# zhm1205/Multimodal_TTA

Hardware: AMD Instinct MI355X
Metric: adapted volumes/sec (higher is better)
Workload: dtype bf16

## Files before the change

include/mmtta.h:

```cpp
#ifndef MMTTA_H
#define MMTTA_H

#include <stdint.h>

#ifdef __cplusplus
extern "C" {
#endif

#define MMTTA_ABI_VERSION 2

typedef enum {
  MMTTA_OK = 0,
  MMTTA_ERR_INVALID = -1,
  MMTTA_ERR_UNSUPPORTED = -2,
  MMTTA_ERR_LAUNCH = -3,
  MMTTA_ERR_WORKSPACE = -4
} mmtta_status;

typedef enum { MMTTA_F32 = 0, MMTTA_BF16 = 1 } mmtta_dtype;

typedef struct {
  void* ptr;
  int32_t n, c, d, h, w;
  int64_t sn, sc, sd, sh, sw;
  int32_t dtype;
  int32_t flags;
} mmtta_tensor;

#define MMTTA_TENSOR_OWNS_PAD 1

#define MMTTA_ACT_NONE 0
#define MMTTA_ACT_RELU 1
#define MMTTA_ACT_LEAKY_RELU 2
typedef struct {
  const float* mean;
  const float* rstd;
  const float* gamma;
  const float* beta;
  int32_t relu;
  int32_t per_item;
  const float* scale;
  const float* shift;
  float negative_slope;
  int32_t _pad2;
} mmtta_norm_on_load;

const char* mmtta_last_error(void);
int mmtta_abi_version(void);

#define MMTTA_OPT_PROFILE_MAIN_KERNEL_ONLY 1
#define MMTTA_OPT_SPLITK_BELOW 2
#define MMTTA_OPT_SPLITK_TARGET 3
#define MMTTA_OPT_WGRAD_WORKGROUPS 4
#define MMTTA_OPT_WGRAD_THIN_SLABS 5
#define MMTTA_OPT_IGEMM_PIPELINE 6
#define MMTTA_OPT_EPILOGUE_VEC16 9
#define MMTTA_OPT_IGEMM_LEAN 10
#define MMTTA_OPT_WGRAD_VECTOR_STAGING 11
#define MMTTA_OPT_CLASS_FUSED_MIN_WORKGROUPS 12
#define MMTTA_OPT_THIN_MFMA 13
#define MMTTA_OPT_IGEMM_FRAGMENT_REUSE 14
#define MMTTA_OPT_LAME_TILED 15
#define MMTTA_OPT_RAW_STAGING 16
#define MMTTA_OPT_HEAD_LOSS_PAIR 17
#define MMTTA_OPT_THIN_LEAN 18
#define MMTTA_OPT_WGRAD_EPILOGUE_UPDATE 19
#define MMTTA_OPT_CLS8_PIPELINE 20
#define MMTTA_OPT_CLS8_LEAN_EPILOGUE 21
int mmtta_set_option(int key, int value);

int mmtta_copy_strided(const mmtta_tensor* src, const mmtta_tensor* dst, void* stream);

typedef enum {
  MMTTA_CONV_FWD = 0,
  MMTTA_CONV_DGRAD = 1,
  MMTTA_CONVT_FWD = 2,
  MMTTA_CONVT_DGRAD = 3
} mmtta_conv_op;

typedef struct {
  int32_t op;
  int32_t ksize;
  int32_t stride;
  int32_t cin;
  int32_t cout;
  int32_t dtype;
} mmtta_conv_desc;

int64_t mmtta_conv_packed_bytes(const mmtta_conv_desc* desc);

int mmtta_conv_pack_weights(const mmtta_conv_desc* desc, const float* w_master, void* packed, void* stream);

typedef struct {
  mmtta_conv_desc desc;
  const float* w_master;
  void* packed;
} mmtta_pack_item;
int64_t mmtta_conv_pack_table_bytes(int count);
int mmtta_conv_pack_table_build(const mmtta_pack_item* items, int count, void* table_host, int64_t* total);
int mmtta_conv_pack_batched(const void* table_dev, int count, int64_t total, void* stream);

typedef struct {
  int32_t tiles;
  int32_t launches;
  int32_t ksplit;
  int32_t stats_rows;
  int32_t config;
  int32_t _pad;
  int64_t workspace_bytes;
} mmtta_conv_plan_t;

int mmtta_conv_plan(const mmtta_conv_desc* desc, const mmtta_tensor* x, const mmtta_tensor* y,
                    mmtta_conv_plan_t* plan);

typedef struct {
  const mmtta_tensor* add;
  mmtta_norm_on_load add_norm;
} mmtta_conv_epilogue;

int mmtta_conv_run(const mmtta_conv_desc* desc, const mmtta_tensor* x, const mmtta_norm_on_load* x_norm,
                   const void* packed, const float* bias, const mmtta_conv_epilogue* epi,
                   const mmtta_tensor* y, int accumulate, float* stats, void* workspace,
                   int64_t workspace_bytes, void* stream);

int mmtta_conv_route(const mmtta_conv_desc* desc, const mmtta_tensor* x, const mmtta_norm_on_load* x_norm,
                     const mmtta_conv_epilogue* epi, const mmtta_tensor* y, int accumulate, const float* stats);

int mmtta_conv_stages_raw(const mmtta_conv_desc* desc, const mmtta_tensor* x, const mmtta_norm_on_load* x_norm,
                          const mmtta_conv_epilogue* epi, const mmtta_tensor* y, int accumulate, const float* stats);

int mmtta_conv_cls8_pipelined(const mmtta_conv_desc* desc, const mmtta_tensor* x, const mmtta_norm_on_load* x_norm,
                              const mmtta_conv_epilogue* epi, const mmtta_tensor* y, int accumulate, const float* stats);

int mmtta_conv_cls8_lean_epilogue(const mmtta_conv_desc* desc, const mmtta_tensor* x, const mmtta_norm_on_load* x_norm,
                                  const mmtta_conv_epilogue* epi, const mmtta_tensor* y, int accumulate, const float* stats);

int mmtta_conv_thin_lean(const mmtta_conv_desc* desc, const mmtta_tensor* x, const mmtta_norm_on_load* x_norm,
                         const mmtta_conv_epilogue* epi, const mmtta_tensor* y, int accumulate, const float* stats);

int mmtta_conv_thin_kernel(const mmtta_conv_desc* desc, const mmtta_tensor* x, const mmtta_norm_on_load* x_norm,
                           const mmtta_conv_epilogue* epi, const mmtta_tensor* y, int accumulate, const float* stats);

typedef struct {
  int32_t items_per_set;
  int32_t inner;
  int64_t packed_outer, packed_inner;
  int64_t weight_outer, weight_inner;
  int64_t bias_outer, bias_inner;
} mmtta_param_sets;

int mmtta_conv_run_sets(const mmtta_conv_desc* desc, const mmtta_tensor* x, const mmtta_norm_on_load* x_norm,
                        const void* packed, const float* bias, const mmtta_conv_epilogue* epi,
                        const mmtta_tensor* y, int accumulate, float* stats, void* workspace,
                        int64_t workspace_bytes, const mmtta_param_sets* sets, void* stream);

int mmtta_conv_head_loss_eligible(const mmtta_conv_desc* desc, const mmtta_tensor* x, const mmtta_norm_on_load* x_norm,
                                  const mmtta_conv_epilogue* epi, const mmtta_tensor* y, const mmtta_tensor* dlogits,
                                  int softmax, int per_item);
int64_t mmtta_conv_head_loss_partials(const mmtta_conv_desc* desc, const mmtta_tensor* x, const mmtta_tensor* y);
int mmtta_conv_head_loss_run_sets(const mmtta_conv_desc* desc, const mmtta_tensor* x, const mmtta_norm_on_load* x_norm,
                                  const void* packed, const float* bias, const mmtta_conv_epilogue* epi,
                                  const mmtta_tensor* y, const mmtta_tensor* dlogits, int softmax, int per_item,
                                  double* partial, float* loss, const mmtta_param_sets* sets, void* stream);

int64_t mmtta_conv_wgrad_workspace_bytes(const mmtta_conv_desc* desc, const mmtta_tensor* x,
                                         const mmtta_tensor* dy);
int mmtta_conv_wgrad_kernel(const mmtta_conv_desc* desc, const mmtta_tensor* x, const mmtta_tensor* dy);
int mmtta_conv_wgrad_stages_raw(const mmtta_conv_desc* desc, const mmtta_tensor* x, const mmtta_norm_on_load* x_norm,
                                const mmtta_tensor* dy);
int mmtta_conv_wgrad(const mmtta_conv_desc* desc, const mmtta_tensor* x, const mmtta_norm_on_load* x_norm,
                     const mmtta_tensor* dy, float* dw, float* db, int accumulate, void* workspace,
                     int64_t workspace_bytes, void* stream);

int64_t mmtta_conv_wgrad_workspace_bytes_sets(const mmtta_conv_desc* desc, const mmtta_tensor* x, const mmtta_tensor* dy,
                                              const mmtta_param_sets* sets);
int mmtta_conv_wgrad_sets(const mmtta_conv_desc* desc, const mmtta_tensor* x, const mmtta_norm_on_load* x_norm,
                          const mmtta_tensor* dy, float* dw, float* db, int accumulate, void* workspace,
                          int64_t workspace_bytes, const mmtta_param_sets* sets, void* stream);
int mmtta_conv_wgrad_plan_sets(const mmtta_conv_desc* desc, const mmtta_tensor* x, const mmtta_tensor* dy,
                               const mmtta_param_sets* sets, int32_t plan[4]);

typedef struct {
  int32_t clip, zscore, masked, min_count;
  float lo, hi, mask_gt, eps;
  float mean, std;
  int32_t legacy, _pad;
} mmtta_intensity_rule;
int64_t mmtta_intensity_scratch_bytes(int channels);
int mmtta_intensity_normalize(const mmtta_tensor* x, const mmtta_intensity_rule* rules, const mmtta_tensor* y,
                              void* scratch, void* stream);

typedef enum {
  MMTTA_NORM_INSTANCE = 0,
  MMTTA_NORM_BATCH = 1,
  MMTTA_NORM_GROUP = 2
} mmtta_norm_kind;

int mmtta_norm_stats_finalize(int kind, int groups, const float* part, int rows_per_n, int n, int c,
                              int64_t count, float eps, int training, float* running_mean,
                              float* running_var, float momentum, float* mean, float* rstd,
                              const float* gamma, const float* beta, float* scale, float* shift,
                              double* scratch, void* stream);

typedef struct {
  int32_t items_per_set;
  int32_t _pad;
  int64_t affine_stride;
  int64_t stats_stride;
} mmtta_norm_sets;

int mmtta_norm_stats_finalize_sets(int kind, int groups, const float* part, int rows_per_n, int n, int c,
                                   int64_t count, float eps, int training, float* running_mean,
                                   float* running_var, float momentum, float* mean, float* rstd,
                                   const float* gamma, const float* beta, float* scale, float* shift,
                                   float* gamma_items, float* beta_items, double* scratch,
                                   const mmtta_norm_sets* sets, void* stream);

int mmtta_reduce_rows_per_n(const mmtta_tensor* t);

int mmtta_channel_stats(const mmtta_tensor* x, float* part, void* stream);

int mmtta_combine(const mmtta_tensor* a, const mmtta_norm_on_load* ta, const mmtta_tensor* b,
                  const mmtta_norm_on_load* tb, const mmtta_tensor* out, void* stream);

int mmtta_norm_bwd_reduce(const mmtta_tensor* dout, const mmtta_tensor* y, const mmtta_norm_on_load* t,
                          float* part, void* stream);

int mmtta_norm_bwd_finalize(int kind, int groups, const float* part, int rows_per_n, int n, int c, int64_t count,
                            const float* gamma, int training, float* m1, float* m2, float* dgamma,
                            float* dbeta, int accumulate, double* scratch , void* stream);

int mmtta_norm_bwd_finalize_sets(int kind, int groups, const float* part, int rows_per_n, int n, int c, int64_t count,
                                 const float* gamma, int training, float* m1, float* m2, float* dgamma,
                                 float* dbeta, int accumulate, double* scratch ,
                                 const mmtta_norm_sets* sets, void* stream);

int mmtta_norm_bwd_apply(const mmtta_tensor* dout, const mmtta_tensor* y, const mmtta_norm_on_load* t,
                         const float* m1, const float* m2, const mmtta_tensor* dy, void* stream);

int mmtta_norm_bwd_small_ok(const mmtta_tensor* dout, const mmtta_tensor* y, const mmtta_norm_on_load* t,
                            const mmtta_tensor* dy);
int mmtta_norm_bwd_small(const mmtta_tensor* dout, const mmtta_tensor* y, const mmtta_norm_on_load* t, int64_t count,
                         const mmtta_tensor* dy, void* stream);

int mmtta_upsample2x_fwd(const mmtta_tensor* x, const mmtta_tensor* y, void* stream);
int mmtta_upsample2x_bwd(const mmtta_tensor* dy, const mmtta_tensor* dx, int accumulate, void* stream);

int mmtta_lincomb(int count, const mmtta_tensor* const* in, const float* w, const mmtta_tensor* out,
                  int accumulate, void* stream);

#define MMTTA_PW_OP_CHANNEL_STATS 0
#define MMTTA_PW_OP_NORM_BWD_REDUCE 1
#define MMTTA_PW_OP_NORM_BWD_APPLY 2
#define MMTTA_PW_OP_NORM_BWD_SMALL 3
#define MMTTA_PW_OP_COMBINE 4
#define MMTTA_PW_OP_LINCOMB 5
#define MMTTA_PW_OP_UPSAMPLE_FWD 6
#define MMTTA_PW_OP_UPSAMPLE_BWD 7
#define MMTTA_PW_REDUCE 0
#define MMTTA_PW_REDUCE_STREAM 1
#define MMTTA_PW_ELEMENTWISE 2
#define MMTTA_PW_COMBINE8 3
#define MMTTA_PW_NORM_BWD_APPLY8 4
#define MMTTA_PW_NORM_BWD_SMALL 5
#define MMTTA_PW_LINCOMB 6
#define MMTTA_PW_UPSAMPLE_FWD 7
#define MMTTA_PW_UPSAMPLE_BWD 8
typedef struct {
  int64_t vox_per_row;
  int64_t work_items;
  int64_t grid_x;
  int32_t grid_y;
  int32_t family;
  int32_t mode;
  int32_t vec;
  int32_t it;
  int32_t count;
  int32_t bf16_a;
  int32_t bf16_b;
  int32_t bf16_o;
  int32_t has_b;
  int32_t rows_per_n;
  int32_t rows_per_block;
  int32_t cpl, nvl;
  int32_t trips;
  int32_t cb_passes;
  int32_t second_trip;
  int32_t leaky;
// ... 225 lines not shown
```

multimodal_tta_amd/_lib.py:

```python
from __future__ import annotations

import ctypes as C
import os
from typing import Optional, Sequence

import torch

_HERE = os.path.dirname(os.path.abspath(__file__))
LIB_PATH = os.path.join(_HERE, "csrc", "libmmtta.so")

F32, BF16 = 0, 1
CONV_FWD, CONV_DGRAD, CONVT_FWD, CONVT_DGRAD = 0, 1, 2, 3
NORM_INSTANCE, NORM_BATCH, NORM_GROUP = 0, 1, 2


class MmttaError(RuntimeError):
    pass


class Tensor(C.Structure):
    _fields_ = [
        ("ptr", C.c_void_p),
        ("n", C.c_int32), ("c", C.c_int32), ("d", C.c_int32), ("h", C.c_int32), ("w", C.c_int32),
        ("sn", C.c_int64), ("sc", C.c_int64), ("sd", C.c_int64), ("sh", C.c_int64), ("sw", C.c_int64),
        ("dtype", C.c_int32), ("flags", C.c_int32),
    ]


class NormOnLoad(C.Structure):
    _fields_ = [
        ("mean", C.c_void_p), ("rstd", C.c_void_p), ("gamma", C.c_void_p), ("beta", C.c_void_p),
        ("relu", C.c_int32), ("per_item", C.c_int32), ("scale", C.c_void_p), ("shift", C.c_void_p),
    ]


class NormOnLoadAct(NormOnLoad):
    _fields_ = [("negative_slope", C.c_float), ("_pad2", C.c_int32)]


class NormSets(C.Structure):
    _fields_ = [("items_per_set", C.c_int32), ("_pad", C.c_int32), ("affine_stride", C.c_int64), ("stats_stride", C.c_int64)]


class ConvDesc(C.Structure):
    _fields_ = [
        ("op", C.c_int32), ("ksize", C.c_int32), ("stride", C.c_int32), ("cin", C.c_int32), ("cout", C.c_int32),
        ("dtype", C.c_int32),
    ]


class PackItem(C.Structure):
    _fields_ = [("desc", ConvDesc), ("w_master", C.c_void_p), ("packed", C.c_void_p)]


class ParamSets(C.Structure):
    _fields_ = [("items_per_set", C.c_int32), ("inner", C.c_int32), ("packed_outer", C.c_int64), ("packed_inner", C.c_int64),
                ("weight_outer", C.c_int64), ("weight_inner", C.c_int64), ("bias_outer", C.c_int64), ("bias_inner", C.c_int64)]


class ConvPlan(C.Structure):
    _fields_ = [
        ("tiles", C.c_int32), ("launches", C.c_int32), ("ksplit", C.c_int32), ("stats_rows", C.c_int32),
        ("config", C.c_int32), ("_pad", C.c_int32), ("workspace_bytes", C.c_int64),
    ]


class PointwiseRoute(C.Structure):
    _fields_ = [("vox_per_row", C.c_int64), ("work_items", C.c_int64), ("grid_x", C.c_int64), ("grid_y", C.c_int32),
                ("family", C.c_int32), ("mode", C.c_int32), ("vec", C.c_int32), ("it", C.c_int32), ("count", C.c_int32),
                ("bf16_a", C.c_int32), ("bf16_b", C.c_int32), ("bf16_o", C.c_int32), ("has_b", C.c_int32),
                ("rows_per_n", C.c_int32), ("rows_per_block", C.c_int32), ("cpl", C.c_int32), ("nvl", C.c_int32),
                ("trips", C.c_int32), ("cb_passes", C.c_int32), ("second_trip", C.c_int32), ("leaky", C.c_int32)]


PW_OPS = ("channel_stats", "norm_bwd_reduce", "norm_bwd_apply", "norm_bwd_small", "combine", "lincomb", "upsample_fwd",
          "upsample_bwd")
PW_FAMILIES = ("reduce", "reduce_stream", "elementwise", "combine8", "norm_bwd_apply8", "norm_bwd_small", "lincomb",
               "upsample_fwd", "upsample_bwd")


class OptimDesc(C.Structure):
    _fields_ = [("kind", C.c_int32), ("lr", C.c_float), ("beta1", C.c_float), ("beta2", C.c_float), ("eps", C.c_float),
                ("weight_decay", C.c_float), ("momentum", C.c_float), ("dampening", C.c_float), ("nesterov", C.c_int32)]


class UpdateTarget(C.Structure):
    _fields_ = [("optim", OptimDesc), ("w_p", C.c_void_p), ("w_m", C.c_void_p), ("w_v", C.c_void_p), ("b_p", C.c_void_p),
                ("b_m", C.c_void_p), ("b_v", C.c_void_p), ("b_grad", C.c_void_p), ("image", C.c_void_p * 2),
                ("image_outer", C.c_int64 * 2), ("image_inner", C.c_int64 * 2), ("step", C.c_void_p),
                ("w_decay", C.c_int32), ("b_decay", C.c_int32)]


OPTIM_ADAM, OPTIM_ADAMW, OPTIM_SGD = 0, 1, 2


class ConvEpilogue(C.Structure):
    _fields_ = [("add", C.POINTER(Tensor)), ("add_norm", NormOnLoadAct)]


class IntensityRule(C.Structure):
    _fields_ = [("clip", C.c_int32), ("zscore", C.c_int32), ("masked", C.c_int32), ("min_count", C.c_int32),
                ("lo", C.c_float), ("hi", C.c_float), ("mask_gt", C.c_float), ("eps", C.c_float),
                ("mean", C.c_float), ("std", C.c_float), ("legacy", C.c_int32), ("_pad", C.c_int32)]


class InputNormBranch(C.Structure):
    _fields_ = [("dy", C.POINTER(Tensor)), ("weight", C.c_void_p), ("set_stride", C.c_int64), ("ksize", C.c_int32),
                ("stride", C.c_int32)]


class WindowGrid(C.Structure):
    _fields_ = [("extent", C.c_int32 * 3), ("count", C.c_int32 * 3)]


_P = C.POINTER
_SIGNATURES = {
    "mmtta_last_error": (C.c_char_p, []),
    "mmtta_abi_version": (C.c_int, []),
    "mmtta_set_option": (C.c_int, [C.c_int, C.c_int]),
    "mmtta_intensity_scratch_bytes": (C.c_int64, [C.c_int]),
    "mmtta_intensity_normalize": (C.c_int, [_P(Tensor), _P(IntensityRule), _P(Tensor), C.c_void_p, C.c_void_p]),
    "mmtta_copy_strided": (C.c_int, [_P(Tensor), _P(Tensor), C.c_void_p]),
    "mmtta_conv_packed_bytes": (C.c_int64, [_P(ConvDesc)]),
    "mmtta_conv_pack_weights": (C.c_int, [_P(ConvDesc), C.c_void_p, C.c_void_p, C.c_void_p]),
    "mmtta_conv_pack_table_bytes": (C.c_int64, [C.c_int]),
    "mmtta_conv_pack_table_build": (C.c_int, [_P(PackItem), C.c_int, C.c_void_p, _P(C.c_int64)]),
    "mmtta_conv_pack_batched": (C.c_int, [C.c_void_p, C.c_int, C.c_int64, C.c_void_p]),
    "mmtta_conv_plan": (C.c_int, [_P(ConvDesc), _P(Tensor), _P(Tensor), _P(ConvPlan)]),
    "mmtta_conv_run": (C.c_int, [_P(ConvDesc), _P(Tensor), _P(NormOnLoad), C.c_void_p, C.c_void_p, _P(ConvEpilogue),
                                 _P(Tensor), C.c_int, C.c_void_p, C.c_void_p, C.c_int64, C.c_void_p]),
    "mmtta_conv_run_sets": (C.c_int, [_P(ConvDesc), _P(Tensor), _P(NormOnLoad), C.c_void_p, C.c_void_p, _P(ConvEpilogue),
                                      _P(Tensor), C.c_int, C.c_void_p, C.c_void_p, C.c_int64, _P(ParamSets), C.c_void_p]),
    "mmtta_conv_route": (C.c_int, [_P(ConvDesc), _P(Tensor), _P(NormOnLoad), _P(ConvEpilogue), _P(Tensor), C.c_int, C.c_void_p]),
    "mmtta_conv_stages_raw": (C.c_int, [_P(ConvDesc), _P(Tensor), _P(NormOnLoad), _P(ConvEpilogue), _P(Tensor), C.c_int, C.c_void_p]),
    "mmtta_conv_cls8_pipelined": (C.c_int, [_P(ConvDesc), _P(Tensor), _P(NormOnLoad), _P(ConvEpilogue), _P(Tensor), C.c_int, C.c_void_p]),
    "mmtta_conv_cls8_lean_epilogue": (C.c_int, [_P(ConvDesc), _P(Tensor), _P(NormOnLoad), _P(ConvEpilogue), _P(Tensor), C.c_int, C.c_void_p]),
    "mmtta_conv_thin_lean": (C.c_int, [_P(ConvDesc), _P(Tensor), _P(NormOnLoad), _P(ConvEpilogue), _P(Tensor), C.c_int, C.c_void_p]),
    "mmtta_conv_thin_kernel": (C.c_int, [_P(ConvDesc), _P(Tensor), _P(NormOnLoad), _P(ConvEpilogue), _P(Tensor), C.c_int, C.c_void_p]),
    "mmtta_conv_head_loss_eligible": (C.c_int, [_P(ConvDesc), _P(Tensor), _P(NormOnLoad), _P(ConvEpilogue), _P(Tensor), _P(Tensor),
                                                C.c_int, C.c_int]),
    "mmtta_conv_head_loss_partials": (C.c_int64, [_P(ConvDesc), _P(Tensor), _P(Tensor)]),
    "mmtta_conv_head_loss_run_sets": (C.c_int, [_P(ConvDesc), _P(Tensor), _P(NormOnLoad), C.c_void_p, C.c_void_p, _P(ConvEpilogue),
                                                _P(Tensor), _P(Tensor), C.c_int, C.c_int, C.c_void_p, C.c_void_p, _P(ParamSets),
                                                C.c_void_p]),
    "mmtta_conv_wgrad_workspace_bytes": (C.c_int64, [_P(ConvDesc), _P(Tensor), _P(Tensor)]),
    "mmtta_conv_wgrad_workspace_bytes_sets": (C.c_int64, [_P(ConvDesc), _P(Tensor), _P(Tensor), _P(ParamSets)]),
    "mmtta_conv_wgrad_plan_sets": (C.c_int, [_P(ConvDesc), _P(Tensor), _P(Tensor), _P(ParamSets), _P(C.c_int32)]),
    "mmtta_conv_wgrad_sets": (C.c_int, [_P(ConvDesc), _P(Tensor), _P(NormOnLoad), _P(Tensor), C.c_void_p, C.c_void_p,
                                        C.c_int, C.c_void_p, C.c_int64, _P(ParamSets), C.c_void_p]),
    "mmtta_conv_wgrad_kernel": (C.c_int, [_P(ConvDesc), _P(Tensor), _P(Tensor)]),
    "mmtta_conv_wgrad_stages_raw": (C.c_int, [_P(ConvDesc), _P(Tensor), _P(NormOnLoad), _P(Tensor)]),
    "mmtta_conv_wgrad": (C.c_int, [_P(ConvDesc), _P(Tensor), _P(NormOnLoad), _P(Tensor), C.c_void_p, C.c_void_p,
                                   C.c_int, C.c_void_p, C.c_int64, C.c_void_p]),
    "mmtta_norm_stats_finalize": (C.c_int, [C.c_int, C.c_int, C.c_void_p, C.c_int, C.c_int, C.c_int, C.c_int64,
                                            C.c_float, C.c_int, C.c_void_p, C.c_void_p, C.c_float, C.c_void_p,
                                            C.c_void_p, C.c_void_p, C.c_void_p, C.c_void_p, C.c_void_p, C.c_void_p,
                                            C.c_void_p]),
    "mmtta_norm_stats_finalize_sets": (C.c_int, [C.c_int, C.c_int, C.c_void_p, C.c_int, C.c_int, C.c_int, C.c_int64,
                                                 C.c_float, C.c_int, C.c_void_p, C.c_void_p, C.c_float, C.c_void_p,
                                                 C.c_void_p, C.c_void_p, C.c_void_p, C.c_void_p, C.c_void_p, C.c_void_p,
                                                 C.c_void_p, C.c_void_p, _P(NormSets), C.c_void_p]),
    "mmtta_reduce_rows_per_n": (C.c_int, [_P(Tensor)]),
    "mmtta_channel_stats": (C.c_int, [_P(Tensor), C.c_void_p, C.c_void_p]),
    "mmtta_combine": (C.c_int, [_P(Tensor), _P(NormOnLoad), _P(Tensor), _P(NormOnLoad), _P(Tensor), C.c_void_p]),
    "mmtta_norm_bwd_reduce": (C.c_int, [_P(Tensor), _P(Tensor), _P(NormOnLoad), C.c_void_p, C.c_void_p]),
    "mmtta_norm_bwd_finalize": (C.c_int, [C.c_int, C.c_int, C.c_void_p, C.c_int, C.c_int, C.c_int, C.c_int64,
                                          C.c_void_p, C.c_int, C.c_void_p, C.c_void_p, C.c_void_p, C.c_void_p,
                                          C.c_int, C.c_void_p, C.c_void_p]),
    "mmtta_norm_bwd_finalize_sets": (C.c_int, [C.c_int, C.c_int, C.c_void_p, C.c_int, C.c_int, C.c_int, C.c_int64,
                                               C.c_void_p, C.c_int, C.c_void_p, C.c_void_p, C.c_void_p, C.c_void_p,
                                               C.c_int, C.c_void_p, _P(NormSets), C.c_void_p]),
    "mmtta_norm_bwd_apply": (C.c_int, [_P(Tensor), _P(Tensor), _P(NormOnLoad), C.c_void_p, C.c_void_p, _P(Tensor),
                                       C.c_void_p]),
    "mmtta_norm_bwd_small_ok": (C.c_int, [_P(Tensor), _P(Tensor), _P(NormOnLoad), _P(Tensor)]),
    "mmtta_norm_bwd_small": (C.c_int, [_P(Tensor), _P(Tensor), _P(NormOnLoad), C.c_int64, _P(Tensor), C.c_void_p]),
    "mmtta_upsample2x_fwd": (C.c_int, [_P(Tensor), _P(Tensor), C.c_void_p]),
    "mmtta_upsample2x_bwd": (C.c_int, [_P(Tensor), _P(Tensor), C.c_int, C.c_void_p]),
    "mmtta_lincomb": (C.c_int, [C.c_int, _P(_P(Tensor)), _P(C.c_float), _P(Tensor), C.c_int, C.c_void_p]),
    "mmtta_pointwise_route": (C.c_int, [C.c_int, _P(_P(Tensor)), C.c_int, _P(NormOnLoad), _P(NormOnLoad), C.c_void_p, C.c_void_p,
                                        _P(PointwiseRoute)]),
    "mmtta_entropy_partials": (C.c_int64, [_P(Tensor)]),
    "mmtta_entropy_loss": (C.c_int, [_P(Tensor), C.c_int, _P(Tensor), C.c_void_p, C.c_void_p, C.c_void_p]),
    "mmtta_entropy_partials_items": (C.c_int64, [_P(Tensor)]),
    "mmtta_entropy_loss_items": (C.c_int, [_P(Tensor), C.c_int, _P(Tensor), C.c_void_p, C.c_void_p, C.c_void_p]),
    "mmtta_entropy_filtered_partials": (C.c_int64, [_P(Tensor)]),
    "mmtta_entropy_filtered_items": (C.c_int, [_P(Tensor), C.c_int, C.c_float, C.c_void_p, C.c_void_p, _P(Tensor), C.c_void_p,
                                               C.c_void_p, C.c_void_p, C.c_void_p]),
    "mmtta_mirror_views": (C.c_int, [_P(Tensor), _P(Tensor), C.c_int, _P(C.c_int32), C.c_void_p]),
    "mmtta_memo_partials": (C.c_int64, [_P(Tensor), C.c_int]),
    "mmtta_memo_loss_items": (C.c_int, [_P(Tensor), C.c_int, C.c_int, _P(C.c_int32), _P(Tensor), C.c_void_p, C.c_void_p,
                                        C.c_void_p]),
    "mmtta_memo_ensemble": (C.c_int, [_P(Tensor), C.c_int, C.c_int, _P(C.c_int32), _P(Tensor), C.c_void_p]),
    "mmtta_affine_views": (C.c_int, [_P(Tensor), _P(Tensor), C.c_int, C.c_int, C.c_int, C.c_void_p, C.c_void_p, C.c_void_p]),
    "mmtta_affine_ensemble": (C.c_int, [_P(Tensor), C.c_int, C.c_int, _P(C.c_int32), C.c_int, C.c_int, C.c_void_p, C.c_void_p,
                                        _P(Tensor), C.c_void_p]),
    "mmtta_consistency_partials": (C.c_int64, [_P(Tensor)]),
    "mmtta_consistency_loss_items": (C.c_int, [_P(Tensor), _P(Tensor), C.c_int, _P(Tensor), C.c_void_p, C.c_void_p, C.c_void_p]),
    "mmtta_cotta_update_partials": (C.c_int64, [C.c_int64, C.c_int]),
    "mmtta_cotta_update_sets": (C.c_int, [C.c_void_p, C.c_void_p, C.c_void_p, C.c_int64, C.c_int, C.c_int64, C.c_int64,
                                          C.c_double, C.c_float, C.c_uint64, C.c_void_p, C.c_void_p, C.c_void_p, C.c_void_p,
                                          C.c_void_p]),
    "mmtta_magnitude_select_class": (C.c_int, [C.c_int64]),
    "mmtta_magnitude_select_chunks": (C.c_int64, [C.c_int64]),
    "mmtta_magnitude_select_scratch_bytes": (C.c_int64, [C.c_int, C.c_int]),
    "mmtta_magnitude_select_sets": (C.c_int, [C.c_void_p, C.c_void_p, C.c_void_p, C.c_int, C.c_int, C.c_int64, C.c_void_p,
                                              C.c_void_p, C.c_void_p]),
    "mmtta_petal_update_partials": (C.c_int64, [C.c_int64, C.c_int]),
    "mmtta_petal_update_sets": (C.c_int, [C.c_void_p, C.c_void_p, C.c_void_p, C.c_void_p, C.c_void_p, C.c_void_p, C.c_void_p,
                                          C.c_int, C.c_int64, C.c_int, C.c_int64, C.c_int64, C.c_int64, C.c_double, C.c_void_p,
                                          C.c_void_p, C.c_void_p]),
    "mmtta_intensity_range_partials": (C.c_int64, [_P(Tensor)]),
    "mmtta_intensity_range": (C.c_int, [_P(Tensor), C.c_void_p, C.c_void_p, C.c_void_p]),
    "mmtta_augment_views": (C.c_int, [_P(Tensor), _P(Tensor), C.c_int, _P(C.c_int32), C.c_void_p, C.c_void_p, C.c_void_p,
                                      C.c_uint64, C.c_void_p, C.c_void_p]),
    "mmtta_entropy_weighted_partials": (C.c_int64, [_P(Tensor)]),
    "mmtta_entropy_weighted_items": (C.c_int, [_P(Tensor), C.c_int, C.c_float, C.c_void_p, _P(Tensor), C.c_void_p, C.c_void_p,
                                               C.c_void_p, C.c_void_p]),
    "mmtta_pseudo_label_partials": (C.c_int64, [_P(Tensor)]),
    "mmtta_pseudo_label_loss_items": (C.c_int, [_P(Tensor), C.c_int, _P(Tensor), C.c_void_p, C.c_void_p, C.c_void_p]),
    "mmtta_fisher_accumulate_sets": (C.c_int, [C.c_void_p, C.c_void_p, C.c_int64, C.c_int, C.c_int64, C.c_void_p]),
    "mmtta_fisher_scale": (C.c_int, [C.c_void_p, C.c_int64, C.c_float, C.c_void_p]),
    "mmtta_fisher_penalty_partials": (C.c_int64, [C.c_int64, C.c_int]),
    "mmtta_fisher_penalty_sets": (C.c_int, [C.c_void_p, C.c_void_p, C.c_void_p, C.c_void_p, C.c_int64, C.c_int, C.c_int,
                                            C.c_int64, C.c_float, C.c_void_p, C.c_void_p, C.c_void_p]),
    "mmtta_patch_shuffle": (C.c_int, [_P(Tensor), _P(Tensor), _P(C.c_int32), C.c_void_p, C.c_void_p]),
    "mmtta_deyo_partials": (C.c_int64, [_P(Tensor)]),
    "mmtta_deyo_loss_items": (C.c_int, [_P(Tensor), _P(Tensor), _P(C.c_int32), C.c_void_p, C.c_int, C.c_float, C.c_float,
                                        C.c_float, C.c_void_p, _P(Tensor), C.c_void_p, C.c_void_p, C.c_void_p, C.c_void_p,
                                        C.c_void_p]),
    "mmtta_lame_refine": (C.c_int, [_P(Tensor), _P(Tensor), C.c_uint32, C.c_int, C.c_int, C.c_float, C.c_float, C.c_int,
                                    _P(Tensor), _P(Tensor), C.c_void_p, C.c_void_p]),
    "mmtta_crf_partials": (C.c_int64, [_P(Tensor)]),
    "mmtta_crf_entropy_items": (C.c_int, [_P(Tensor), _P(Tensor), C.c_uint32, C.c_int, C.c_int, C.c_int, C.c_float, C.c_float,
                                          _P(Tensor), C.c_void_p, C.c_void_p, C.c_void_p, C.c_void_p, C.c_void_p]),
    "mmtta_nuclear_scratch": (C.c_int64, [_P(Tensor), C.c_int, C.c_int, C.c_int, C.c_int]),
    "mmtta_nuclear_entropy_items": (C.c_int, [_P(Tensor), C.c_int, C.c_int, C.c_int, C.c_int, C.c_float, C.c_float, C.c_float,
                                              _P(Tensor), C.c_void_p, C.c_void_p, C.c_void_p, C.c_void_p, C.c_void_p]),
    "mmtta_input_norm_apply": (C.c_int, [_P(Tensor), _P(Tensor), C.c_void_p, C.c_void_p, C.c_uint32, C.c_int, C.c_void_p]),
    "mmtta_input_norm_grad_partials": (C.c_int64, [_P(Tensor)]),
    "mmtta_input_norm_grad": (C.c_int, [_P(Tensor), _P(InputNormBranch), C.c_int, C.c_void_p, C.c_void_p, C.c_uint32, C.c_int,
                                        C.c_void_p, C.c_void_p, C.c_void_p, C.c_void_p, C.c_void_p, C.c_double, C.c_double,
                                        C.c_double, C.c_double, C.c_void_p]),
    "mmtta_bias_field_apply": (C.c_int, [_P(Tensor), _P(Tensor), C.c_void_p, C.c_void_p, C.c_void_p, C.c_void_p, C.c_void_p, C.c_int,
                                         C.c_int, C.c_uint32, C.c_void_p]),
    "mmtta_bias_field_grad_partials": (C.c_int64, [_P(Tensor), C.c_int]),
    "mmtta_bias_field_grad": (C.c_int, [_P(Tensor), _P(InputNormBranch), C.c_int, C.c_void_p, C.c_void_p, C.c_void_p, C.c_void_p,
                                        C.c_void_p, C.c_int, C.c_int, C.c_uint32, C.c_void_p, C.c_void_p, C.c_void_p, C.c_void_p,
                                        C.c_void_p, C.c_double, C.c_double, C.c_double, C.c_double, C.c_void_p]),
    "mmtta_modality_views": (C.c_int, [_P(Tensor), _P(Tensor), C.c_int, _P(C.c_uint32), C.c_void_p]),
    "mmtta_modcons_partials": (C.c_int64, [_P(Tensor), C.c_int]),
    "mmtta_modcons_loss_items": (C.c_int, [_P(Tensor), C.c_int, C.c_int, C.c_float, C.c_float, C.c_int, _P(Tensor), C.c_void_p,
                                           C.c_void_p, C.c_void_p, C.c_void_p, C.c_void_p, C.c_void_p, C.c_void_p]),
    "mmtta_window_views": (C.c_int, [_P(Tensor), _P(Tensor), _P(WindowGrid), _P(C.c_int32), C.c_void_p, C.c_float, C.c_void_p]),
    "mmtta_window_partials": (C.c_int64, [_P(Tensor)]),
    "mmtta_window_entropy_items": (C.c_int, [_P(Tensor), C.c_int, _P(WindowGrid), C.c_void_p, _P(Tensor), C.c_void_p, C.c_void_p,
                                             C.c_void_p]),
    "mmtta_window_blend": (C.c_int, [_P(Tensor), _P(Tensor), _P(WindowGrid), C.c_void_p, C.c_void_p, C.c_void_p]),
    "mmtta_adam_step": (C.c_int, [C.c_void_p, C.c_void_p, C.c_void_p, C.c_void_p, C.c_int64, C.c_int64, C.c_float,
                                  C.c_float, C.c_float, C.c_float, C.c_float, C.c_void_p, C.c_void_p]),
    "mmtta_optim_step": (C.c_int, [_P(OptimDesc), C.c_void_p, C.c_void_p, C.c_void_p, C.c_void_p, C.c_int64, C.c_int64,
                                   C.c_void_p, C.c_void_p]),
    "mmtta_optim_step_sets": (C.c_int, [_P(OptimDesc), C.c_void_p, C.c_void_p, C.c_void_p, C.c_void_p, C.c_int64, C.c_int64,
                                        C.c_int, C.c_int64, C.c_void_p, C.c_void_p]),
    "mmtta_optim_step_segments": (C.c_int, [_P(OptimDesc), C.c_void_p, C.c_void_p, C.c_void_p, C.c_void_p, C.c_void_p, C.c_int,
                                            C.c_int64, C.c_int, C.c_int64, C.c_void_p, C.c_void_p]),
    "mmtta_fused_update_enabled": (C.c_int, []),
    "mmtta_conv_wgrad_update_sets": (C.c_int, [_P(ConvDesc), _P(Tensor), _P(NormOnLoad), _P(Tensor), _P(UpdateTarget),
                                               C.c_void_p, C.c_int64, _P(ParamSets), C.c_void_p]),
    "mmtta_conv_wgrad_updates_in_epilogue": (C.c_int, [_P(ConvDesc), _P(Tensor), _P(NormOnLoad), _P(Tensor), _P(ParamSets)]),
    "mmtta_sam_ascent_partials": (C.c_int64, [C.c_int64, C.c_int]),
    "mmtta_sam_ascent_sets": (C.c_int, [C.c_void_p, C.c_void_p, C.c_void_p, C.c_int64, C.c_void_p, C.c_int64, C.c_int, C.c_int,
                                        C.c_int64, C.c_float, C.c_void_p]),
    "mmtta_mask_dice_counts": (C.c_int, [_P(Tensor), _P(Tensor), C.c_float, C.c_void_p, C.c_void_p, C.c_void_p]),
    "mmtta_dice_ce_scratch_bytes": (C.c_int64, [_P(Tensor)]),
    "mmtta_dice_ce_sums": (C.c_int, [_P(Tensor), _P(Tensor), C.c_void_p, C.c_int, C.c_int, C.c_void_p, C.c_void_p, C.c_void_p]),
    "mmtta_dice_ce_grad": (C.c_int, [_P(Tensor), _P(Tensor), C.c_void_p, C.c_int, C.c_int, C.c_int, C.c_int, C.c_float, C.c_float,
                                     C.c_float, C.c_float, C.c_void_p, _P(Tensor), C.c_void_p]),
    "mmtta_calibration_scratch_bytes": (C.c_int64, [_P(Tensor), C.c_int]),
    "mmtta_calibration_bins": (C.c_int, [_P(Tensor), _P(Tensor), C.c_int, C.c_int, C.c_int, C.c_void_p, C.c_void_p, C.c_void_p]),
    "mmtta_components_scratch_bytes": (C.c_int64, [C.c_int64, C.c_int64, C.c_int64, C.c_int64]),
    "mmtta_components_filter": (C.c_int, [C.c_void_p, C.c_void_p, _P(Tensor), C.c_int, C.c_int, C.c_int, C.c_int, C.c_int, C.c_int,
                                          _P(C.c_int64), _P(C.c_int32), C.c_void_p, C.c_void_p, C.c_void_p, C.c_void_p, C.c_void_p]),
    "mmtta_lesionwise_scratch_bytes": (C.c_int64, [C.c_int64, C.c_int64, C.c_int64, C.c_int64]),
    "mmtta_lesionwise_scores": (C.c_int, [C.c_void_p, _P(Tensor), C.c_int, C.c_int, C.c_int, C.c_int, C.c_int, C.c_int, C.c_int,
                                          _P(C.c_int64), C.c_void_p, C.c_void_p, C.c_void_p, C.c_void_p]),
    "mmtta_lesionwise_hd95_scratch_bytes": (C.c_int64, [C.c_int64, C.c_int64, C.c_int64, C.c_int64]),
    "mmtta_lesionwise_hd95": (C.c_int, [C.c_void_p, _P(Tensor), C.c_int, C.c_int, C.c_int, C.c_int, C.c_int, _P(C.c_double), C.c_double,
                                        _P(C.c_int64), C.c_void_p, C.c_void_p, C.c_void_p, C.c_void_p, C.c_void_p]),
    "mmtta_mask_fill_nest_scratch_bytes": (C.c_int64, [C.c_int64, C.c_int64, C.c_int64, C.c_int64]),
    "mmtta_mask_fill_nest": (C.c_int, [C.c_void_p, _P(Tensor), C.c_int, C.c_int, C.c_int, C.c_int, C.c_int, C.c_int, _P(C.c_int32),
                                       _P(C.c_int64), _P(C.c_int32), C.c_int, C.c_int, C.c_void_p, C.c_void_p, C.c_void_p, C.c_void_p]),
    "mmtta_surface_scratch_bytes": (C.c_int64, [C.c_int64, C.c_int64, C.c_int64, C.c_int64]),
    "mmtta_surface_distances": (C.c_int, [C.c_void_p, _P(Tensor), _P(C.c_double), C.c_double, C.c_int, C.c_void_p,
                                          C.c_void_p, C.c_void_p, C.c_void_p]),
    "mmtta_surface_dice_scratch_bytes": (C.c_int64, [C.c_int64, C.c_int64, C.c_int64, C.c_int64]),
    "mmtta_surface_dice": (C.c_int, [C.c_void_p, _P(Tensor), _P(C.c_double), _P(C.c_double), C.c_int, C.c_void_p, C.c_void_p,
                                     C.c_void_p]),
    "mmtta_lesionwise_nsd_list_slots": (C.c_int, []),
    "mmtta_lesionwise_nsd_scratch_bytes": (C.c_int64, [C.c_int64, C.c_int64, C.c_int64, C.c_int64]),
    "mmtta_lesionwise_nsd": (C.c_int, [C.c_void_p, C.c_int, C.c_int, C.c_int, C.c_int, C.c_int, _P(C.c_double), _P(C.c_double),
                                       C.c_int, _P(C.c_int64), C.c_void_p, C.c_void_p, C.c_void_p, C.c_void_p, C.c_void_p]),
}

_lib = None


def load() -> C.CDLL:
    global _lib
    if _lib is not None:
        return _lib
    if not os.path.exists(LIB_PATH):
        raise MmttaError(
            f"{LIB_PATH} is missing: build it with `python -m multimodal_tta_amd.build` (hipcc, gfx950). "
            "There is no CPU or PyTorch fallback for the adaptation path."
        )
    lib = C.CDLL(LIB_PATH)
    for name, (res, args) in _SIGNATURES.items():
        fn = getattr(lib, name)
        fn.restype = res
        fn.argtypes = args
    if lib.mmtta_abi_version() != 2:
        raise MmttaError("libmmtta.so ABI version mismatch")
    if os.environ.get("MMTTA_NO_PIPE", "0") == "1":
        lib.mmtta_set_option(6, 0)
    if os.environ.get("MMTTA_NO_EPIVEC", "0") == "1":
        lib.mmtta_set_option(9, 0)
    if "MMTTA_WGVEC" in os.environ:
        lib.mmtta_set_option(11, int(os.environ["MMTTA_WGVEC"]))
    if "MMTTA_THINMFMA" in os.environ:
        lib.mmtta_set_option(13, int(os.environ["MMTTA_THINMFMA"]))
    if "MMTTA_CLSFUSE" in os.environ:
        lib.mmtta_set_option(12, int(os.environ["MMTTA_CLSFUSE"]))
    if "MMTTA_LEAN" in os.environ:
        lib.mmtta_set_option(10, int(os.environ["MMTTA_LEAN"]))
    if "MMTTA_RAWSTAGE" in os.environ:
        lib.mmtta_set_option(16, int(os.environ["MMTTA_RAWSTAGE"]))
    if "MMTTA_HEADLOSS" in os.environ:
        lib.mmtta_set_option(17, int(os.environ["MMTTA_HEADLOSS"]))
    if "MMTTA_THINLEAN" in os.environ:
        lib.mmtta_set_option(18, int(os.environ["MMTTA_THINLEAN"]))
    if "MMTTA_EPIUPDATE" in os.environ:
        lib.mmtta_set_option(19, int(os.environ["MMTTA_EPIUPDATE"]))
    if "MMTTA_CLS8PIPE" in os.environ:
        lib.mmtta_set_option(20, int(os.environ["MMTTA_CLS8PIPE"]))
    if "MMTTA_CLS8LEAN" in os.environ:
        lib.mmtta_set_option(21, int(os.environ["MMTTA_CLS8LEAN"]))
    _lib = lib
    return lib


def exported_names() -> Sequence[str]:
    return list(_SIGNATURES)


def check(status: int, what: str = "") -> None:
    if status != 0:
        msg = load().mmtta_last_error().decode("utf-8", "replace")
        raise MmttaError(f"{what or 'libmmtta'} failed with status {status}: {msg}")


def stream_ptr() -> int:
    return int(torch.cuda.current_stream().cuda_stream)


def ptr(t: Optional[torch.Tensor]) -> Optional[int]:
    return None if t is None else int(t.data_ptr())


TENSOR_OWNS_PAD = 1


def desc_cl(t: torch.Tensor) -> Tensor:
    if t.dim() != 5 or t.dtype not in (torch.float32, torch.bfloat16) or not t.is_cuda:
        raise MmttaError(f"expected a CUDA float32 / bfloat16 [N,D,H,W,C] view, got {tuple(t.shape)} {t.dtype} {t.device}")
    n, d, h, w, c = t.shape
    sn, sd, sh, sw, sc = t.stride()
    if sc != 1 and c != 1:
        raise MmttaError("activation views must have unit stride along C")
    flags = TENSOR_OWNS_PAD if getattr(t, "_mmtta_owns_pad", False) else 0
    return Tensor(t.data_ptr(), n, c, d, h, w, sn, 1, sd, sh, sw, BF16 if t.dtype == torch.bfloat16 else F32, flags)


def desc_ncdhw(t: torch.Tensor) -> Tensor:
    if t.dim() != 5 or t.dtype != torch.float32 or not t.is_cuda:
        raise MmttaError(f"expected a CUDA float32 [N,C,D,H,W] tensor, got {tuple(t.shape)} {t.dtype} {t.device}")
    n, c, d, h, w = t.shape
    sn, sc, sd, sh, sw = t.stride()
    return Tensor(t.data_ptr(), n, c, d, h, w, sn, sc, sd, sh, sw, F32, 0)


ACT_NONE, ACT_RELU, ACT_LEAKY_RELU = 0, 1, 2


def norm_on_load(mean=None, rstd=None, gamma=None, beta=None, relu=False, scale=None, shift=None,
                 per_item=False, act=None, negative_slope=0.0) -> NormOnLoadAct:
    code = (ACT_RELU if relu else ACT_NONE) if act is None else int(act)
    return NormOnLoadAct(ptr(mean), ptr(rstd), ptr(gamma), ptr(beta), code, 1 if per_item else 0, ptr(scale),
                      ptr(shift), float(negative_slope) if code == ACT_LEAKY_RELU else 0.0, 0)
```

multimodal_tta_amd/csrc/api.hip:

```cpp
#include "common.h"
#include <string.h>

namespace mmtta {
static thread_local char g_err[512] = "";
void set_error(const char* fmt, ...) {
  va_list ap;
  va_start(ap, fmt);
  vsnprintf(g_err, sizeof(g_err), fmt, ap);
  va_end(ap);
}
int g_profile_main_only = 0;
int g_igemm_pipeline = 1;
int g_epilogue_vec = 1;
int g_igemm_lean = 1;
int g_igemm_reuse = 1;
int g_cls_fused_min = 128;
int g_thin_mfma = 2;
int g_wgrad_vec = 1;
int g_lame_tiled = 1;
int g_raw_staging = 3;
int g_head_loss_pair = 3;
int g_thin_lean = 3;
int g_wgrad_epilogue_update = 1;
int g_cls8_pipeline = 1;
int g_cls8_lean_epilogue = 1;
int g_tune[4] = {96, 128, 128, 256};
}

extern "C" int mmtta_set_option(int key, int value) {
  if (key == MMTTA_OPT_PROFILE_MAIN_KERNEL_ONLY) {
    const int prev = mmtta::g_profile_main_only;
    mmtta::g_profile_main_only = value;
    return prev;
  }
  if (key == MMTTA_OPT_WGRAD_VECTOR_STAGING) {
    const int prev = mmtta::g_wgrad_vec;
    mmtta::g_wgrad_vec = value ? 1 : 0;
    return prev;
  }
  if (key == MMTTA_OPT_THIN_MFMA) {
    const int prev = mmtta::g_thin_mfma;
    mmtta::g_thin_mfma = value < 0 ? 0 : (value > 3 ? 3 : value);
    return prev;
  }
  if (key == MMTTA_OPT_CLASS_FUSED_MIN_WORKGROUPS) {
    const int prev = mmtta::g_cls_fused_min;
    mmtta::g_cls_fused_min = value < 0 ? 0 : value;
    return prev;
  }
  if (key == MMTTA_OPT_IGEMM_LEAN) {
    const int prev = mmtta::g_igemm_lean;
    mmtta::g_igemm_lean = value ? 1 : 0;
    return prev;
  }
  if (key == MMTTA_OPT_IGEMM_FRAGMENT_REUSE) {
    const int prev = mmtta::g_igemm_reuse;
    mmtta::g_igemm_reuse = value ? 1 : 0;
    return prev;
  }
  if (key == MMTTA_OPT_EPILOGUE_VEC16) {
    const int prev = mmtta::g_epilogue_vec;
    mmtta::g_epilogue_vec = value ? 1 : 0;
    return prev;
  }
  if (key == MMTTA_OPT_LAME_TILED) {
    const int prev = mmtta::g_lame_tiled;
    mmtta::g_lame_tiled = value ? 1 : 0;
    return prev;
  }
  if (key == MMTTA_OPT_RAW_STAGING) {
    const int prev = mmtta::g_raw_staging;
    mmtta::g_raw_staging = value & 3;
    return prev;
  }
  if (key == MMTTA_OPT_HEAD_LOSS_PAIR) {
    const int prev = mmtta::g_head_loss_pair;
    mmtta::g_head_loss_pair = value & 3;
    return prev;
  }
  if (key == MMTTA_OPT_THIN_LEAN) {
    const int prev = mmtta::g_thin_lean;
    mmtta::g_thin_lean = value & 3;
    return prev;
  }
  if (key == MMTTA_OPT_WGRAD_EPILOGUE_UPDATE) {
    const int prev = mmtta::g_wgrad_epilogue_update;
    mmtta::g_wgrad_epilogue_update = value ? 1 : 0;
    return prev;
  }
  if (key == MMTTA_OPT_CLS8_PIPELINE) {
    const int prev = mmtta::g_cls8_pipeline;
    mmtta::g_cls8_pipeline = value ? 1 : 0;
    return prev;
  }
  if (key == MMTTA_OPT_CLS8_LEAN_EPILOGUE) {
    const int prev = mmtta::g_cls8_lean_epilogue;
    mmtta::g_cls8_lean_epilogue = value & 1;
    return prev;
  }
  if (key == MMTTA_OPT_IGEMM_PIPELINE) {
    const int prev = mmtta::g_igemm_pipeline;
    mmtta::g_igemm_pipeline = value ? 1 : 0;
    return prev;
  }
  if (key >= MMTTA_OPT_SPLITK_BELOW && key <= MMTTA_OPT_WGRAD_THIN_SLABS) {
    if (value < 1) return MMTTA_ERR_INVALID;
    const int prev = mmtta::g_tune[key - MMTTA_OPT_SPLITK_BELOW];
    mmtta::g_tune[key - MMTTA_OPT_SPLITK_BELOW] = value;
    return prev;
  }
  return MMTTA_ERR_INVALID;
}

extern "C" const char* mmtta_last_error(void) { return mmtta::g_err; }
extern "C" int mmtta_abi_version(void) { return MMTTA_ABI_VERSION; }
```

multimodal_tta_amd/csrc/common.h:

```cpp
#pragma once
#include <hip/hip_runtime.h>
#include <type_traits>
#include <stdint.h>
#include <stdio.h>
#include <stdarg.h>
#include "../../include/mmtta.h"

namespace mmtta {

constexpr int WAVE = 64;

void set_error(const char* fmt, ...);

#define MMTTA_CHECK(cond, code, ...)      \
  do {                                    \
    if (!(cond)) {                        \
      ::mmtta::set_error(__VA_ARGS__);    \
      return (code);                      \
    }                                     \
  } while (0)

inline int launch_status(const char* what) {
  hipError_t e = hipGetLastError();
  if (e != hipSuccess) {
    set_error("%s: %s", what, hipGetErrorString(e));
    return MMTTA_ERR_LAUNCH;
  }
  return MMTTA_OK;
}

extern int g_profile_main_only;
extern int g_igemm_pipeline;
extern int g_wgrad_vec;
extern int g_igemm_lean;
extern int g_igemm_reuse;
extern int g_cls_fused_min;
extern int g_lame_tiled;
extern int g_thin_mfma;
extern int g_epilogue_vec;
extern int g_raw_staging;
extern int g_head_loss_pair;
extern int g_thin_lean;
extern int g_wgrad_epilogue_update;
extern int g_cls8_pipeline;
extern int g_cls8_lean_epilogue;
extern int g_tune[4];

inline bool nl_leaky(const mmtta_norm_on_load* t) { return t != nullptr && t->relu == MMTTA_ACT_LEAKY_RELU; }
inline int nl_act_check(const mmtta_norm_on_load* t, const char* what) {
  MMTTA_CHECK(t == nullptr || (t->relu >= MMTTA_ACT_NONE && t->relu <= MMTTA_ACT_LEAKY_RELU), MMTTA_ERR_INVALID,
              "%s: activation code %d (MMTTA_ACT_NONE, _RELU or _LEAKY_RELU)", what, t ? t->relu : 0);
  MMTTA_CHECK(t == nullptr || t->relu != MMTTA_ACT_LEAKY_RELU || __builtin_isfinite(t->negative_slope), MMTTA_ERR_INVALID,
              "%s: LeakyReLU negative_slope must be finite", what);
  return MMTTA_OK;
}

struct PackImageGeo {
  int A, B, T, Kp, Np, kn_is_ba, plain_bf16;
};
int pack_image_geometry(const mmtta_conv_desc* d, PackImageGeo& g);

#define MMTTA_ACT_BODIES                                                                                                    \
  int conv_run_body(const mmtta_conv_desc* d, const mmtta_tensor* x, const mmtta_norm_on_load* x_norm, const void* packed,  \
                    const float* bias, const mmtta_conv_epilogue* epi, const mmtta_tensor* y, int accumulate, float* stats, \
                    void* workspace, int64_t workspace_bytes, const mmtta_param_sets* sets, void* stream);                \
  int conv_wgrad_body(const mmtta_conv_desc* d, const mmtta_tensor* x, const mmtta_norm_on_load* x_norm,                    \
                      const mmtta_tensor* dy, float* dw, float* db, int accumulate, void* workspace,                        \
                      int64_t workspace_bytes, const mmtta_param_sets* sets, void* stream,                                  \
                      const mmtta_update_target* upd);                                                                      \
  int combine_body(const mmtta_tensor* a, const mmtta_norm_on_load* ta, const mmtta_tensor* b,                              \
                   const mmtta_norm_on_load* tb, const mmtta_tensor* out, void* stream);                                    \
  int norm_bwd_reduce_body(const mmtta_tensor* dout, const mmtta_tensor* y, const mmtta_norm_on_load* t, float* part,      \
                           void* stream);                                                                                   \
  int norm_bwd_apply_body(const mmtta_tensor* dout, const mmtta_tensor* y, const mmtta_norm_on_load* t, const float* m1,   \
                          const float* m2, const mmtta_tensor* dy, void* stream);                                           \
  int norm_bwd_small_body(const mmtta_tensor* dout, const mmtta_tensor* y, const mmtta_norm_on_load* t, int64_t count,     \
                          const mmtta_tensor* dy, void* stream);
namespace leaky { MMTTA_ACT_BODIES }

#ifdef MMTTA_ACT_LEAKY_TU
#define MMTTA_ACT_NS_OPEN namespace leaky {
#define MMTTA_ACT_NS_CLOSE }
#else
#define MMTTA_ACT_NS_OPEN
#define MMTTA_ACT_NS_CLOSE
#endif

MMTTA_ACT_NS_OPEN
MMTTA_ACT_BODIES

inline bool is_cl(const mmtta_tensor* t) { return t->sc == 1 || t->c == 1; }

inline bool is_f32(const mmtta_tensor* t) { return t->dtype == MMTTA_F32; }
inline bool is_bf16(const mmtta_tensor* t) { return t->dtype == MMTTA_BF16; }

inline bool quad_aligned(const mmtta_tensor* t, int base_bytes, int elems = 4) {
  return ((uintptr_t)t->ptr) % base_bytes == 0 && t->sw % elems == 0 && t->sh % elems == 0 && t->sd % elems == 0 &&
         t->sn % elems == 0;
}
inline int quad_bytes(const mmtta_tensor* t) { return is_bf16(t) ? 8 : 16; }
inline bool item_fits_31(const mmtta_tensor* t, int64_t pad) {
  const int64_t last = (int64_t)(t->d - 1) * t->sd + (int64_t)(t->h - 1) * t->sh + (int64_t)(t->w - 1) * t->sw + pad;
  return last < ((int64_t)1 << 31);
}
inline bool strides_fit_24(const mmtta_tensor* t) { return t->sw < (1 << 24) && t->sh < (1 << 24) && t->sd < (1 << 24); }
inline bool voxel_dense(const mmtta_tensor* t) { return t->sc == 1 && t->sh == (int64_t)t->w * t->sw && t->sd == (int64_t)t->h * t->sh; }
inline bool dense_rows16(const mmtta_tensor* t) {
  const int q = is_bf16(t) ? 8 : 4;
  return voxel_dense(t) && ((uintptr_t)t->ptr) % 16 == 0 && t->sw % q == 0 && t->sn % q == 0 &&
         (int64_t)t->d * t->h * t->w * t->sw < ((int64_t)1 << 31);
}
inline bool same_shape(const mmtta_tensor* a, const mmtta_tensor* b) {
  return a->n == b->n && a->c == b->c && a->d == b->d && a->h == b->h && a->w == b->w;
}

__device__ __forceinline__ float bf16_bits_to_f32(unsigned int h) { return __uint_as_float(h << 16); }
__device__ __forceinline__ unsigned int f32x2_to_bf16x2(float lo, float hi) {
  typedef __bf16 bf2 __attribute__((ext_vector_type(2)));
  bf2 v;
  v[0] = (__bf16)lo;
  v[1] = (__bf16)hi;
  return __builtin_bit_cast(unsigned int, v);
}
__device__ __forceinline__ unsigned short f32_to_bf16_bits(float v) { return __builtin_bit_cast(unsigned short, (__bf16)v); }
__device__ __forceinline__ uint4 bf16x8_pack(const unsigned short* h) {
  uint4 q;
  q.x = h[0] | ((unsigned)h[1] << 16); q.y = h[2] | ((unsigned)h[3] << 16);
  q.z = h[4] | ((unsigned)h[5] << 16); q.w = h[6] | ((unsigned)h[7] << 16);
  return q;
}
__device__ __forceinline__ float4 ld4_any(const float* base, long long eoff, int bf) {
  if (bf) {
    const uint2 u = *reinterpret_cast<const uint2*>(reinterpret_cast<const unsigned short*>(base) + eoff);
    return make_float4(bf16_bits_to_f32(u.x & 0xffffu), bf16_bits_to_f32(u.x >> 16), bf16_bits_to_f32(u.y & 0xffffu),
                       bf16_bits_to_f32(u.y >> 16));
  }
  return *reinterpret_cast<const float4*>(base + eoff);
}
__device__ __forceinline__ void st4_any(float* base, long long eoff, float4 v, int bf) {
  if (bf) {
    uint2 u;
    u.x = f32x2_to_bf16x2(v.x, v.y);
    u.y = f32x2_to_bf16x2(v.z, v.w);
    *reinterpret_cast<uint2*>(reinterpret_cast<unsigned short*>(base) + eoff) = u;
  } else {
    *reinterpret_cast<float4*>(base + eoff) = v;
  }
}
__device__ __forceinline__ float ld1_any(const float* base, long long eoff, int bf) {
  if (bf) return bf16_bits_to_f32(reinterpret_cast<const unsigned short*>(base)[eoff]);
  return base[eoff];
}
__device__ __forceinline__ void st1_any(float* base, long long eoff, float v, int bf) {
  if (bf) reinterpret_cast<unsigned short*>(base)[eoff] = (unsigned short)(f32x2_to_bf16x2(v, 0.f) & 0xffffu);
  else base[eoff] = v;
}
__device__ __forceinline__ void ld8_any(const float* base, long long eoff, int bf, float4& lo, float4& hi) {
  if (bf) {
    const uint4 u = *reinterpret_cast<const uint4*>(reinterpret_cast<const unsigned short*>(base) + eoff);
    lo = make_float4(bf16_bits_to_f32(u.x & 0xffffu), bf16_bits_to_f32(u.x >> 16), bf16_bits_to_f32(u.y & 0xffffu),
                     bf16_bits_to_f32(u.y >> 16));
    hi = make_float4(bf16_bits_to_f32(u.z & 0xffffu), bf16_bits_to_f32(u.z >> 16), bf16_bits_to_f32(u.w & 0xffffu),
                     bf16_bits_to_f32(u.w >> 16));
  } else {
    lo = *reinterpret_cast<const float4*>(base + eoff);
    hi = *reinterpret_cast<const float4*>(base + eoff + 4);
  }
}

template <bool BF> struct Oct8 { float4 lo, hi; };
template <> struct Oct8<true> { uint4 q; };
template <bool BF>
__device__ __forceinline__ Oct8<BF> oct8_ld(const float* base, unsigned eoff_lo, unsigned eoff_hi) {
  Oct8<BF> o;
  if constexpr (BF) {
    o.q = *reinterpret_cast<const uint4*>(reinterpret_cast<const unsigned short*>(base) + eoff_lo);
  } else {
    o.lo = *reinterpret_cast<const float4*>(base + eoff_lo);
    o.hi = *reinterpret_cast<const float4*>(base + eoff_hi);
  }
  return o;
}
__device__ __forceinline__ void oct8_f8(const Oct8<false>& o, float (&v)[8]) {
  v[0] = o.lo.x; v[1] = o.lo.y; v[2] = o.lo.z; v[3] = o.lo.w; v[4] = o.hi.x; v[5] = o.hi.y; v[6] = o.hi.z; v[7] = o.hi.w;
}
__device__ __forceinline__ void oct8_f8(const Oct8<true>& o, float (&v)[8]) {
  v[0] = bf16_bits_to_f32(o.q.x & 0xffffu); v[1] = __uint_as_float(o.q.x & 0xffff0000u);
  v[2] = bf16_bits_to_f32(o.q.y & 0xffffu); v[3] = __uint_as_float(o.q.y & 0xffff0000u);
  v[4] = bf16_bits_to_f32(o.q.z & 0xffffu); v[5] = __uint_as_float(o.q.z & 0xffff0000u);
  v[6] = bf16_bits_to_f32(o.q.w & 0xffffu); v[7] = __uint_as_float(o.q.w & 0xffff0000u);
}


template <bool BF>
__device__ __forceinline__ void oct8_st(float* base, unsigned eoff, const float (&v)[8]) {
  if constexpr (BF) {
    uint4 q;
    q.x = f32x2_to_bf16x2(v[0], v[1]); q.y = f32x2_to_bf16x2(v[2], v[3]);
// ... 348 lines not shown
```

multimodal_tta_amd/csrc/conv_igemm.hip:

```cpp
#include "common.h"

namespace mmtta {
MMTTA_ACT_NS_OPEN

typedef float f32x16 __attribute__((ext_vector_type(16)));
typedef __bf16 bf16x8 __attribute__((ext_vector_type(8)));
typedef __bf16 bf16x2 __attribute__((ext_vector_type(2)));

__device__ __forceinline__ unsigned int pack_bf16x2(float lo, float hi) {
  bf16x2 v;
  v[0] = (__bf16)lo;
  v[1] = (__bf16)hi;
  return __builtin_bit_cast(unsigned int, v);
}

struct Taps {
  int n;
  int slab[27];
  signed char dz[27], dy[27], dx[27];
  int zmin, ymin, xmin;
  int zext, yext, xext;
};

struct ClassInfo {
  int tap0, ntaps;
  int oz, oy, ox;
  int zmin, ymin, xmin;
  int zext, yext, xext;
  int Dg, Hg, Wg;
  int BX, BXY;
  unsigned mBX, mBXY;
};

struct GArgs {
  const float* in; long long isn, isd, ish, isw; int Ci, Di, Hi, Wi;
  NL tin;
  float* out; long long osn, osd, osh, osw; int Co, Do, Ho, Wo;
  int so;
  int si;
  const float* wp; int Kp, Np;
  const float* bias;
  PSets ps;
  const float* add; long long asn, asd, ash, asw; NL tadd;
  int accumulate;
  float* stats; int stats_rows_per_n;
  float* ws; int ksplit, stages_per_split, nstages;
  int tz, ty, tx;
  int in_bf, out_bf, add_bf;
  int vec4;
  int ovec;
  int coef_off;
  int rowload;
  int flip27;
  int ncls;
  ClassInfo cls[8];
  int toff[27];
  int slab[27];
};

__device__ __forceinline__ void class_of_tile(const GArgs& a, int tile, int& cidx, int& t) {
  if (a.ncls == 8) { cidx = 7 - (tile & 7); t = tile >> 3; }
  else { cidx = 0; t = tile; }
}

template <int TZ, int TY, int TX, bool PERM>
__device__ __forceinline__ void row_to_local(int v, int& zl, int& yl, int& xl) {
  if (PERM) {
    static_assert(TX == 8 && TY % 4 == 0, "the permutation assumes 4 x 8 row blocks");
    const int r = v & 31, q = r >> 2;
    const int y = (0xEB14 >> (2 * q)) & 3;
    const int xh = (q >> 1) & 1;
    v = (v & ~31) + y * 8 + xh * 4 + (r & 3);
  }
  xl = v % TX;
  yl = (v / TX) % TY;
  zl = v / (TX * TY);
}

constexpr int LDS_PITCH_BF16 = 12;

__host__ __device__ constexpr int tap27_off(int t, int rby) { return ((t / 9) * rby + (t / 3) % 3) * LDS_PITCH_BF16 + t % 3; }

__host__ __device__ constexpr int reuse_xslot(int bx) { return (bx & 1) * 5 + (bx >> 1); }
__host__ __device__ constexpr int reuse_row(int i, int b) {
  const int yl = i >> 2, x = 2 * (i & 3) + b, xh = x >> 2;
  int q = 0;
  for (int c = 0; c < 8; ++c)
    if (((0xEB14 >> (2 * c)) & 3) == yl && ((c >> 1) & 1) == xh) q = c;
  return q * 4 + (x & 3);
}

template <int TZ, int TY, int TX, int MB, bool PERM, bool ABF, bool XPAR = false>
__device__ __forceinline__ void epilogue_vec16(const GArgs& a, const float* biasp, const ClassInfo& ci, f32x16 (&acc)[MB], float* tr,
                                               int lane, int rowblock0, int colbase, bool colact, int n, int gz0, int gy0, int gx0,
                                               float (&ssum)[4], float (&ssq)[4]) {
  int osd = (int)a.osd, osh = (int)a.osh, osw = (int)a.osw, asd = (int)a.asd, ash_ = (int)a.ash, asw = (int)a.asw;
  int so = a.so, Do = a.Do, Ho = a.Ho, Wo = a.Wo, coz = ci.oz, coy = ci.oy, cox = ci.ox, cDg = ci.Dg, cHg = ci.Hg, cWg = ci.Wg;
  asm volatile("" : "+s"(osd), "+s"(osh), "+s"(osw), "+s"(asd), "+s"(ash_), "+s"(asw), "+s"(so), "+s"(Do), "+s"(Ho), "+s"(Wo));
  asm volatile("" : "+s"(coz), "+s"(coy), "+s"(cox), "+s"(cDg), "+s"(cHg), "+s"(cWg));
  const int h = lane >> 5, r = lane & 31;
  const int rsub = lane >> 3, c4 = (lane & 7) * 4;
  const int colv = colbase + c4;
  const bool cvok = colact && colv < a.Co;
  const int colc = min(colv, a.Co - 4);
  float4 bias4 = make_float4(0.f, 0.f, 0.f, 0.f);
  float asc[4] = {1.f, 1.f, 1.f, 1.f}, ash[4] = {0.f, 0.f, 0.f, 0.f};
  if (biasp) bias4 = *reinterpret_cast<const float4*>(biasp + colc);
  if (a.add) nl_coeff_vec<4>(a.tadd, n, a.Co, colc, asc, ash);
#pragma unroll
  for (int j = 0; j < 4; ++j) { ssum[j] = 0.f; ssq[j] = 0.f; }
  const float* addb = a.add;
  float* outb = a.out;
  const long long abase = (long long)n * a.asn + colc, obase = (long long)n * a.osn + colc;
  auto finish = [&](const float4& val, const float4& addq, const float4& oldq, bool okk, int oo) {
    float v[4] = {val.x + bias4.x, val.y + bias4.y, val.z + bias4.z, val.w + bias4.w};
    if (a.add) {
      const float av[4] = {addq.x, addq.y, addq.z, addq.w};
#pragma unroll
      for (int j = 0; j < 4; ++j) v[j] += nl_apply(av[j], asc[j], ash[j], a.tadd.relu);
    }
    if (a.accumulate) { v[0] += oldq.x; v[1] += oldq.y; v[2] += oldq.z; v[3] += oldq.w; }
    if (okk) {
      st4_t<ABF>(outb, obase + oo, make_float4(v[0], v[1], v[2], v[3]));
#pragma unroll
      for (int j = 0; j < 4; ++j) { ssum[j] += v[j]; ssq[j] += v[j] * v[j]; }
    }
  };
  if constexpr (XPAR) {
    static_assert(MB == 2, "two parity blocks");
#pragma unroll
    for (int b = 0; b < 2; ++b)
#pragma unroll
      for (int i = 0; i < 16; ++i) tr[(reuse_row(i, b) + 32 * h) * 36 + r] = acc[b][i];
  }
  const bool interior = PERM && so == 1 && coz == 0 && coy == 0 && cox == 0 && gz0 + TZ <= min(cDg, Do) && gy0 + TY <= min(cHg, Ho) &&
                        gx0 + TX <= min(cWg, Wo);
  if (interior) {
    const bool lb = (rsub >> 2) != 0;
    const int lxo = (rsub & 3) * osw, lxa = (rsub & 3) * asw;
    constexpr int T = 0xEB14;
    auto row_off = [&](int mb, int k, int sd_, int sh_, int sw_, int lx) {
      const int rb = rowblock0 + mb;
      const int zl = TY == 4 ? rb : (rb >> 1), yb = TY == 4 ? 0 : (rb & 1) * 4;
      const int u = (gz0 + zl) * sd_ + (gy0 + yb) * sh_ + (gx0 + 4 * (k & 1)) * sw_;
      const int y0 = (T >> (2 * (2 * k))) & 3, y1 = (T >> (2 * (2 * k + 1))) & 3;
      return (lb ? u + y1 * sh_ : u + y0 * sh_) + lx;
    };
    const bool one_operand = (a.add != nullptr) != (a.accumulate != 0);
    float4 pre[MB][4];
    if (one_operand) {
#pragma unroll
      for (int mb = 0; mb < MB; ++mb)
#pragma unroll
        for (int k = 0; k < 4; ++k)
          pre[mb][k] = a.add ? ld4_t<ABF>(addb, abase + row_off(mb, k, asd, ash_, asw, lxa))
                             : ld4_t<ABF>(outb, obase + row_off(mb, k, osd, osh, osw, lxo));
    }
#pragma unroll
    for (int mb = 0; mb < MB; ++mb) {
      if constexpr (!XPAR) {
#pragma unroll
        for (int i = 0; i < 16; ++i) tr[((i & 3) + 8 * (i >> 2) + 4 * h) * 36 + r] = acc[mb][i];
      }
      const float* trb = tr + (XPAR ? mb * 32 * 36 : 0);
      float4 val[4], addv[4], oldv[4];
#pragma unroll
      for (int k = 0; k < 4; ++k) val[k] = *reinterpret_cast<const float4*>(trb + (rsub + 8 * k) * 36 + c4);
      if (!one_operand) {
        if (a.add) {
#pragma unroll
          for (int k = 0; k < 4; ++k) addv[k] = ld4_t<ABF>(addb, abase + row_off(mb, k, asd, ash_, asw, lxa));
        }
        if (a.accumulate) {
#pragma unroll
          for (int k = 0; k < 4; ++k) oldv[k] = ld4_t<ABF>(outb, obase + row_off(mb, k, osd, osh, osw, lxo));
        }
      }
#pragma unroll
      for (int k = 0; k < 4; ++k) {
        const int oo = row_off(mb, k, osd, osh, osw, lxo);
        if (one_operand) finish(val[k], pre[mb][k], pre[mb][k], cvok, oo);
        else finish(val[k], addv[k], oldv[k], cvok, oo);
      }
    }
  } else {
#pragma unroll
  for (int mb = 0; mb < MB; ++mb) {
    if constexpr (!XPAR) {
#pragma unroll
      for (int i = 0; i < 16; ++i) tr[((i & 3) + 8 * (i >> 2) + 4 * h) * 36 + r] = acc[mb][i];
    }
    const float* trb = tr + (XPAR ? mb * 32 * 36 : 0);
    int ooff[4], aoff[4];
    bool ok[4];
    float4 val[4];
#pragma unroll
    for (int k = 0; k < 4; ++k) {
      const int row = rsub + 8 * k;
      val[k] = *reinterpret_cast<const float4*>(trb + row * 36 + c4);
      int zl, yl, xl;
      row_to_local<TZ, TY, TX, PERM>((rowblock0 + mb) * 32 + row, zl, yl, xl);
      const int gz = gz0 + zl, gy = gy0 + yl, gx = gx0 + xl;
      const int oz = gz * so + coz, oy = gy * so + coy, ox = gx * so + cox;
      ok[k] = cvok && gz < cDg && gy < cHg && gx < cWg && oz < Do && oy < Ho && ox < Wo;
      const int cz = min(oz, Do - 1), cy = min(oy, Ho - 1), cx = min(ox, Wo - 1);
      ooff[k] = cz * osd + cy * osh + cx * osw;
      aoff[k] = cz * asd + cy * ash_ + cx * asw;
    }
    float4 addv[4], oldv[4];
    if (a.add) {
#pragma unroll
      for (int k = 0; k < 4; ++k) addv[k] = ld4_t<ABF>(addb, abase + aoff[k]);
    }
    if (a.accumulate) {
#pragma unroll
      for (int k = 0; k < 4; ++k) oldv[k] = ld4_t<ABF>(outb, obase + ooff[k]);
    }
#pragma unroll
    for (int k = 0; k < 4; ++k) finish(val[k], addv[k], oldv[k], ok[k], ooff[k]);
  }
  }
#pragma unroll
  for (int j = 0; j < 4; ++j) {
#pragma unroll
    for (int o = 8; o < 64; o <<= 1) { ssum[j] += __shfl_xor(ssum[j], o, 64); ssq[j] += __shfl_xor(ssq[j], o, 64); }
  }
}

constexpr int EPI_TILE_FLOATS = 32 * 36;

template <int NB, int MB, int TZ, int TY, int TX, int KCI, bool BF, int OCC = 2, bool ABF = false>
__global__ __launch_bounds__(256, OCC) void igemm_kernel(GArgs a) {
  constexpr bool REUSE = false, RAW = false;
#include "conv_igemm_body.h"
}

template <bool ABF>
__global__ __launch_bounds__(256, 3) void igemm_reuse_kernel(GArgs a) {
  constexpr int NB = 1, MB = 2, TZ = 4, TY = 8, TX = 8, KCI = 16, OCC = 3;
  constexpr bool BF = true, REUSE = true, RAW = false;
#include "conv_igemm_body.h"
}

template <int NB, int MB, int TZ, int TY, int TX, int KCI, int OCC>
__global__ __launch_bounds__(256, OCC) void igemm_raw_kernel(GArgs a) {
  constexpr bool BF = true, ABF = true, REUSE = false, RAW = true;
#include "conv_igemm_body.h"
}

template <bool ABF>
__global__ __launch_bounds__(256, 3) void igemm_reuse_raw_kernel(GArgs a) {
  constexpr int NB = 1, MB = 2, TZ = 4, TY = 8, TX = 8, KCI = 16, OCC = 3;
  constexpr bool BF = true, REUSE = true, RAW = true;
#include "conv_igemm_body.h"
}

struct ClsTap { int cls, d, slab; };
__host__ __device__ constexpr ClsTap cls_tap(int f) {
  int idx = 0;
  for (int cls = 0; cls < 8; ++cls) {
    const int pz = (cls >> 2) & 1, py = (cls >> 1) & 1, px = cls & 1;
    for (int a = 0; a <= pz; ++a)
      for (int b = 0; b <= py; ++b)
        for (int c = 0; c <= px; ++c) {
          const int kz = pz ? (a == 0 ? 0 : 2) : 1, dz = pz ? (a == 0 ? 1 : 0) : 0;
          const int ky = py ? (b == 0 ? 0 : 2) : 1, dy = py ? (b == 0 ? 1 : 0) : 0;
          const int kx = px ? (c == 0 ? 0 : 2) : 1, dx = px ? (c == 0 ? 1 : 0) : 0;
          if (idx == f) return ClsTap{cls, (dz * 2 + dy) * 2 + dx, (kz * 3 + ky) * 3 + kx};
          ++idx;
        }
  }
  return ClsTap{0, 0, 0};
}

typedef unsigned cls8_u32x4 __attribute__((ext_vector_type(4)));
template <bool TYPED>
__device__ __forceinline__ uint4 cls8_lds_q(const void* p) {
  if constexpr (TYPED) {
    const cls8_u32x4 v = *reinterpret_cast<const cls8_u32x4*>(p);
    return make_uint4(v.x, v.y, v.z, v.w);
  } else {
    return *reinterpret_cast<const uint4*>(p);
  }
}

template <bool ADD, bool ACC>
__device__ __forceinline__ void epilogue_cls8_lean_t(const GArgs& a, const float* biasp, f32x16 (&acc)[8], float* tr, int lane, int wave,
                                                     int colbase, bool colact, int n, int gz0, int gy0, int gx0, float (&tsum)[4],
                                                     float (&tsq)[4]) {
  constexpr int AHEAD = (ADD && ACC) ? 1 : 3;
  const int osd = (int)a.osd, osh = (int)a.osh, osw = (int)a.osw, asd = (int)a.asd, ash_ = (int)a.ash, asw = (int)a.asw;
  const int h = lane >> 5, r = lane & 31;
  const int rsub = lane >> 3, c4 = (lane & 7) * 4;
  const int colv = colbase + c4;
  const bool cvok = colact && colv < a.Co;
  const int colc = min(colv, a.Co - 4);
  float4 bias4 = make_float4(0.f, 0.f, 0.f, 0.f);
  float asc[4] = {1.f, 1.f, 1.f, 1.f}, ash[4] = {0.f, 0.f, 0.f, 0.f};
  if (biasp) bias4 = *reinterpret_cast<const float4*>(biasp + colc);
  if constexpr (ADD) nl_coeff_vec<4>(a.tadd, n, a.Co, colc, asc, ash);
  const bool lb = (rsub >> 2) != 0, odd = (lane & 1) != 0;
  constexpr int T = 0xEB14;
  unsigned lo[4], la[4];
#pragma unroll
  for (int k = 0; k < 4; ++k) {
    const int y0 = (T >> (2 * (2 * k))) & 3, y1 = (T >> (2 * (2 * k + 1))) & 3, x2 = 2 * (4 * (k & 1) + (rsub & 3));
    lo[k] = (unsigned)((lb ? 2 * y1 : 2 * y0) * osh + x2 * osw + colc) * 2u;
    la[k] = (unsigned)((lb ? 2 * y1 : 2 * y0) * ash_ + x2 * asw + colc) * 2u;
  }
  const unsigned lst[2] = {odd ? lo[1] - 8u : lo[0], odd ? lo[3] - 8u : lo[2]};
  char* const outh = reinterpret_cast<char*>(reinterpret_cast<unsigned short*>(a.out) + ((long long)n * a.osn + (long long)(2 * (gz0 + wave)) * osd +
                                                                               (long long)(2 * gy0) * osh + (long long)(2 * gx0) * osw));
  const char* const addh = reinterpret_cast<const char*>(reinterpret_cast<const unsigned short*>(a.add) + ((long long)n * a.asn + (long long)(2 * (gz0 + wave)) * asd +
                                                                                           (long long)(2 * gy0) * ash_ + (long long)(2 * gx0) * asw));
  uint2 qa[AHEAD + 1][4], qo[AHEAD + 1][4];
  auto request = [&](auto cc) {
    constexpr int c = decltype(cc)::value, s = c % (AHEAD + 1), pz = (c >> 2) & 1, py = (c >> 1) & 1, px = c & 1;
    if constexpr (ADD) {
      const char* const p = addh + 2 * (pz * asd + py * ash_ + px * asw);
#pragma unroll
      for (int k = 0; k < 4; ++k) qa[s][k] = *reinterpret_cast<const uint2*>(p + la[k]);
    }
    if constexpr (ACC) {
      const char* const p = outh + 2 * (pz * osd + py * osh + px * osw);
#pragma unroll
      for (int k = 0; k < 4; ++k) qo[s][k] = *reinterpret_cast<const uint2*>(p + lo[k]);
    }
  };
  static_for<0, AHEAD>([&](auto cc) { request(cc); });
  static_for<0, 8>([&](auto cc) {
    constexpr int c = decltype(cc)::value, s = c % (AHEAD + 1), pz = (c >> 2) & 1, py = (c >> 1) & 1, px = c & 1;
    if constexpr (c + AHEAD < 8) request(std::integral_constant<int, c + AHEAD>{});
#pragma unroll
    for (int i = 0; i < 16; ++i) tr[((i & 3) + 8 * (i >> 2) + 4 * h) * 36 + r] = acc[c][i];
    float v[4][4];
#pragma unroll
    for (int k = 0; k < 4; ++k) {
      const float4 val = *reinterpret_cast<const float4*>(tr + (rsub + 8 * k) * 36 + c4);
      v[k][0] = val.x + bias4.x; v[k][1] = val.y + bias4.y; v[k][2] = val.z + bias4.z; v[k][3] = val.w + bias4.w;
    }
    unsigned pk[4][2];
#pragma unroll
    for (int k = 0; k < 4; ++k) {
      if constexpr (ADD) {
        const uint2 u = qa[s][k];
        const float av[4] = {bf16_bits_to_f32(u.x & 0xffffu), bf16_bits_to_f32(u.x >> 16), bf16_bits_to_f32(u.y & 0xffffu),
                             bf16_bits_to_f32(u.y >> 16)};
#pragma unroll
        for (int j = 0; j < 4; ++j) v[k][j] += nl_apply(av[j], asc[j], ash[j], a.tadd.relu);
      }
      if constexpr (ACC) {
        const uint2 u = qo[s][k];
        v[k][0] += bf16_bits_to_f32(u.x & 0xffffu); v[k][1] += bf16_bits_to_f32(u.x >> 16);
        v[k][2] += bf16_bits_to_f32(u.y & 0xffffu); v[k][3] += bf16_bits_to_f32(u.y >> 16);
      }
      pk[k][0] = f32x2_to_bf16x2(v[k][0], v[k][1]);
      pk[k][1] = f32x2_to_bf16x2(v[k][2], v[k][3]);
    }
    char* const po = outh + 2 * (pz * osd + py * osh + px * osw);
    uint4 q[2];
#pragma unroll
    for (int p = 0; p < 2; ++p) {
      const unsigned s0 = odd ? pk[2 * p][0] : pk[2 * p + 1][0], s1 = odd ? pk[2 * p][1] : pk[2 * p + 1][1];
      const unsigned n0 = (unsigned)__builtin_amdgcn_update_dpp(0, (int)s0, 0xb1, 0xf, 0xf, true);
      const unsigned n1 = (unsigned)__builtin_amdgcn_update_dpp(0, (int)s1, 0xb1, 0xf, 0xf, true);
      q[p] = odd ? make_uint4(n0, n1, pk[2 * p + 1][0], pk[2 * p + 1][1]) : make_uint4(pk[2 * p][0], pk[2 * p][1], n0, n1);
    }
    if (cvok) {
      *reinterpret_cast<uint4*>(po + lst[0]) = q[0];
      *reinterpret_cast<uint4*>(po + lst[1]) = q[1];
    }
    if (a.stats != nullptr) {
#pragma clang fp contract(off)
      float ssum[4] = {0.f, 0.f, 0.f, 0.f}, ssq[4] = {0.f, 0.f, 0.f, 0.f};
      if (cvok) {
#pragma unroll
        for (int k = 0; k < 4; ++k)
#pragma unroll
          for (int j = 0; j < 4; ++j) { ssum[j] += v[k][j]; ssq[j] = fmaf(v[k][j], v[k][j], ssq[j]); }
      }
#pragma unroll
      for (int j = 0; j < 4; ++j) {
#pragma unroll
        for (int o = 8; o < 64; o <<= 1) { ssum[j] += __shfl_xor(ssum[j], o, 64); ssq[j] += __shfl_xor(ssq[j], o, 64); }
      }
#pragma unroll
      for (int j = 0; j < 4; ++j) { tsum[j] += ssum[j]; tsq[j] += ssq[j]; }
    }
  });
}

template <bool ABF>
__device__ __forceinline__ void epilogue_cls8_lean(const GArgs& a, const float* biasp, f32x16 (&acc)[8], float* tr, int lane, int wave,
                                                   int colbase, bool colact, int n, int gz0, int gy0, int gx0, float (&tsum)[4],
                                                   float (&tsq)[4]) {
  static_assert(ABF, "bf16 rows: a lane pair holds 16 bytes of one");
  if (a.add != nullptr) {
    if (a.accumulate) epilogue_cls8_lean_t<true, true>(a, biasp, acc, tr, lane, wave, colbase, colact, n, gz0, gy0, gx0, tsum, tsq);
    else epilogue_cls8_lean_t<true, false>(a, biasp, acc, tr, lane, wave, colbase, colact, n, gz0, gy0, gx0, tsum, tsq);
  } else {
    if (a.accumulate) epilogue_cls8_lean_t<false, true>(a, biasp, acc, tr, lane, wave, colbase, colact, n, gz0, gy0, gx0, tsum, tsq);
    else epilogue_cls8_lean_t<false, false>(a, biasp, acc, tr, lane, wave, colbase, colact, n, gz0, gy0, gx0, tsum, tsq);
  }
}

template <int KCI, bool ABF>
// ... 469 lines not shown
    __builtin_amdgcn_fence(__ATOMIC_RELEASE, "wavefront");
    __builtin_amdgcn_wave_barrier();
  }
}

template <int KB, bool BF>
static void launch_pointwise_mfma_nb(const PWArgs& a, int nb, dim3 grid, hipStream_t s) {
  if (nb == 1) hipLaunchKernelGGL((pointwise_mfma_kernel<KB, 1, BF>), grid, dim3(256), 0, s, a);
  else hipLaunchKernelGGL((pointwise_mfma_kernel<KB, 2, BF>), grid, dim3(256), 0, s, a);
}
template <bool BF>
static void launch_pointwise_mfma(const PWArgs& a, int kb, int nb, dim3 grid, hipStream_t s) {
  switch (kb) {
    case 1: launch_pointwise_mfma_nb<1, BF>(a, nb, grid, s); break;
    case 2: launch_pointwise_mfma_nb<2, BF>(a, nb, grid, s); break;
    case 3: launch_pointwise_mfma_nb<3, BF>(a, nb, grid, s); break;
    case 4: launch_pointwise_mfma_nb<4, BF>(a, nb, grid, s); break;
    case 6: launch_pointwise_mfma_nb<6, BF>(a, nb, grid, s); break;
    default: launch_pointwise_mfma_nb<8, BF>(a, nb, grid, s); break;
  }
}

struct Config { int NB, MB, TZ, TY, TX, KCI; bool bf; };

static inline int roundup(int v, int m) { return (v + m - 1) / m * m; }

static void op_dims(const mmtta_conv_desc* d, int& K, int& N, int& si, bool& classes) {
  switch (d->op) {
    case MMTTA_CONV_FWD: K = d->cin; N = d->cout; si = d->stride; classes = false; break;
    case MMTTA_CONV_DGRAD: K = d->cout; N = d->cin; si = 1; classes = d->stride == 2; break;
    case MMTTA_CONVT_FWD: K = d->cin; N = d->cout; si = 1; classes = true; break;
    default: K = d->cout; N = d->cin; si = 2; classes = false; break;
  }
}

static Config pick_config(int Np, int si, long long voxels, int K, bool bf) {
  if (si == 1) {
    if (Np == 32 && bf && g_igemm_lean) return {1, 2, 4, 8, 8, 16, bf};
    if (Np == 32) return {1, 4, 8, 8, 8, bf ? 16 : 8, bf};
    if (Np == 64) return {2, 4, 4, 8, 8, bf ? 32 : 16, bf};
    const long long tiles = (voxels + 127) / 128, colgroups = (Np + 127) / 128;
    if (tiles * colgroups * ((K + 31) / 32) < 384) return {4, 4, 4, 4, 8, bf ? 16 : 8, bf};
    return {4, 4, 4, 4, 8, 32, bf};
  }
  if (Np == 32) return {1, 1, 4, 4, 8, bf ? 16 : 8, bf};
  if (Np == 64) return {2, 2, 4, 4, 8, bf ? 16 : 8, bf};
  return {4, 4, 4, 4, 8, bf ? 16 : 8, bf};
}

static bool use_bf16(const mmtta_conv_desc* d, int K) {
  return d->dtype == MMTTA_BF16 && K >= 16 && !direct_applicable(d);
}

static int validate_desc(const mmtta_conv_desc* d) {
  MMTTA_CHECK(d != nullptr, MMTTA_ERR_INVALID, "conv: null desc");
  MMTTA_CHECK(d->op >= 0 && d->op <= 3, MMTTA_ERR_INVALID, "conv: bad op %d", d->op);
  MMTTA_CHECK(d->ksize == 1 || d->ksize == 3, MMTTA_ERR_UNSUPPORTED, "conv: ksize %d (1 or 3)", d->ksize);
  MMTTA_CHECK(d->stride == 1 || d->stride == 2, MMTTA_ERR_UNSUPPORTED, "conv: stride %d (1 or 2)", d->stride);
  MMTTA_CHECK(!(d->ksize == 1 && d->stride != 1), MMTTA_ERR_UNSUPPORTED, "conv: 1x1x1 with stride 2");
  MMTTA_CHECK(d->cin > 0 && d->cout > 0, MMTTA_ERR_INVALID, "conv: channels must be positive");
  MMTTA_CHECK(d->dtype == MMTTA_F32 || d->dtype == MMTTA_BF16, MMTTA_ERR_UNSUPPORTED, "conv: dtype %d", d->dtype);
  if (d->op == MMTTA_CONVT_FWD || d->op == MMTTA_CONVT_DGRAD)
    MMTTA_CHECK(d->ksize == 3 && d->stride == 2, MMTTA_ERR_UNSUPPORTED,
                "conv_transpose: only k3 s2 p1 op1 (the monai UNet up layer)");
  return MMTTA_OK;
}

static int config_id(const Config& c) {
  int id;
  if (c.bf && c.NB == 1 && c.MB == 2) return 14;
  if (c.NB == 1) id = c.MB == 4 ? 0 : 3;
  else if (c.NB == 2) id = c.MB == 4 ? 1 : 4;
  else id = c.KCI == 32 ? 2 : 5;
  return c.bf ? id + 7 : id;
}

enum CRoute : int {
  C_DIRECT = 6,
  C_THIN = 13,
  C_CLS_FUSED = 15,
  C_PW_SMALL = 16,
  C_PW_MFMA = 17,
  C_IGEMM_REUSE = 18,
};

struct RunFacts {
  const float* stats; const mmtta_tensor* add; const mmtta_norm_on_load* x_norm;
  int accumulate;
  const float* bias;
};

#ifdef MMTTA_ACT_LEAKY_TU
constexpr bool RAW_KERNELS = false;
#else
constexpr bool RAW_KERNELS = true;
#endif
static bool raw_operand(const mmtta_tensor* x, const mmtta_norm_on_load* x_norm) {
  return is_bf16(x) && x->c % 8 == 0 && quad_aligned(x, 16, 8) &&
         (x_norm == nullptr || (x_norm->mean == nullptr && x_norm->scale == nullptr && x_norm->relu == MMTTA_ACT_NONE));
}
static bool raw_staging(int route, bool bf_tile, const mmtta_tensor* x, const mmtta_norm_on_load* x_norm, const mmtta_tensor* y,
                        const mmtta_tensor* add) {
  const bool igemm = route != 6 && route != 13 && route != 16 && route != 17;
  return RAW_KERNELS && (g_raw_staging & 1) && igemm && bf_tile && raw_operand(x, x_norm) && is_bf16(y) && (add == nullptr || is_bf16(add));
}

static bool cls8_pipelined(int route, bool bf_tile, const mmtta_tensor* x, const mmtta_norm_on_load* x_norm, const mmtta_tensor* y,
                           const mmtta_tensor* add) {
  return g_cls8_pipeline && route == 15  && raw_staging(route, bf_tile, x, x_norm, y, add);
}

static bool cls8_lean(int route, bool bf_tile, const mmtta_tensor* x, const mmtta_norm_on_load* x_norm, const mmtta_tensor* y,
                      const mmtta_tensor* add) {
  return (g_cls8_lean_epilogue & 1) && cls8_pipelined(route, bf_tile, x, x_norm, y, add) && y->c % 8 == 0 &&
         (add == nullptr || add->c % 8 == 0);
}

struct Geometry {
  int route;
  int K, N, Kp, Np, si;
  bool classes;
  Config cfg;
  int tz, ty, tx, tiles_per_n, tiles, ncls;
  int nstages, ksplit, sps;
  int stats_rows;
  int64_t workspace_bytes;
};

static int expected_out_dim(const mmtta_conv_desc* d, int in) {
  switch (d->op) {
    case MMTTA_CONV_FWD: return d->stride == 1 ? in : (in + 1) / 2;
    case MMTTA_CONVT_FWD: return in * 2;
    case MMTTA_CONVT_DGRAD: return in / 2;
    default: return -1;
  }
}

static bool pointwise_mfma_applicable(const mmtta_conv_desc* d, const mmtta_tensor* x, const mmtta_tensor* y, const Geometry& g,
                                      const RunFacts& rt) {
  static const bool pw_on = !(getenv("MMTTA_POINTWISE_MFMA") && atoi(getenv("MMTTA_POINTWISE_MFMA")) == 0);
  const int kb = (g.K + 15) / 16;
  auto rows_ok = [&](const mmtta_tensor* t) { return dense_rows16(t) && is_bf16(t) == is_bf16(x); };
  return pw_on && d->ksize == 1 && (d->op == MMTTA_CONV_FWD || d->op == MMTTA_CONV_DGRAD) && use_bf16(d, g.K) &&
         (kb <= 4 || kb == 6 || kb == 8) && g.Np <= 64 && rt.stats == nullptr && !(rt.x_norm && (rt.x_norm->mean || rt.x_norm->scale)) &&
         (long long)y->d * y->h * y->w >= 4096 && rows_ok(x) && rows_ok(y) && (rt.add == nullptr || (rows_ok(rt.add) && same_shape(rt.add, y)));
}

static bool rowload_operand(const mmtta_tensor* x) {
  const int64_t lim24 = (int64_t)1 << 24;
  return quad_aligned(x, 16, is_bf16(x) ? 8 : 4) && strides_fit_24(x) && x->d < lim24 && x->h < lim24 && x->w < lim24 &&
         item_fits_31(x, x->c + 16);
}

static bool igemm_reuse_applicable(const mmtta_conv_desc* d, const mmtta_tensor* x, const mmtta_tensor* y, const Geometry& g,
                                   const RunFacts& rt) {
  const mmtta_tensor* ad = rt.add;
  return g_igemm_reuse && g_igemm_pipeline && g_epilogue_vec && g.route == 14 && !g.classes && d->ksize == 3 && g.si == 1 &&
         g.K == 32 && g.N == 32 && g.ksplit == 1 && rowload_operand(x) && quad_aligned(y, quad_bytes(y)) && (!ad || quad_aligned(ad, quad_bytes(ad))) &&
         is_bf16(x) == is_bf16(y) && (!ad || is_bf16(ad) == is_bf16(y)) && ((uintptr_t)rt.bias) % 16 == 0;
}

static bool cls_fused_operand(const mmtta_tensor* t) {
  return quad_aligned(t, 16, is_bf16(t) ? 8 : 4) && strides_fit_24(t) && item_fits_31(t, t->c + 16);
}

static int stats_rows_per_tile(const Geometry& g) {
  if (g.route == C_CLS_FUSED) return 1;
  return g.ksplit > 1 ? g.cfg.TZ * g.cfg.TY * g.cfg.TX / 32 : 1;
}

static int geometry(const mmtta_conv_desc* d, const mmtta_tensor* x, const mmtta_tensor* y, const RunFacts* rt, Geometry& g) {
  int st = validate_desc(d);
  if (st) return st;
  MMTTA_CHECK(x && y && x->ptr && y->ptr, MMTTA_ERR_INVALID, "conv: null tensor");
  MMTTA_CHECK(is_cl(x) && is_cl(y), MMTTA_ERR_UNSUPPORTED, "conv: tensors must be channels-last (sc == 1)");
  op_dims(d, g.K, g.N, g.si, g.classes);
  MMTTA_CHECK(x->c == g.K && y->c == g.N, MMTTA_ERR_INVALID, "conv: channel mismatch (x.c=%d want %d, y.c=%d want %d)",
              x->c, g.K, y->c, g.N);
  MMTTA_CHECK(x->n == y->n, MMTTA_ERR_INVALID, "conv: batch mismatch");
  const int xd[3] = {x->d, x->h, x->w}, yd[3] = {y->d, y->h, y->w};
  for (int i = 0; i < 3; ++i) {
    int e = expected_out_dim(d, xd[i]);
    if (e >= 0) {
      MMTTA_CHECK(yd[i] == e, MMTTA_ERR_INVALID, "conv: spatial mismatch axis %d: in %d -> out %d, expected %d", i, xd[i],
                  yd[i], e);
      if (d->op == MMTTA_CONVT_DGRAD)
        MMTTA_CHECK(xd[i] % 2 == 0, MMTTA_ERR_INVALID, "conv_transpose dgrad: dy extent must be even");
    } else {
      int want = d->stride == 1 ? yd[i] : (yd[i] + 1) / 2;
      MMTTA_CHECK(xd[i] == want, MMTTA_ERR_INVALID, "conv dgrad: dy extent %d does not match dx extent %d", xd[i], yd[i]);
    }
  }
  g.Kp = roundup(g.K, 32);
  g.Np = roundup(g.N, 32);
  int Dg = y->d, Hg = y->h, Wg = y->w;
  if (g.classes) { Dg = (y->d + 1) / 2; Hg = (y->h + 1) / 2; Wg = (y->w + 1) / 2; }
  g.cfg = pick_config(g.Np, g.si, (long long)Dg * Hg * Wg * (g.classes ? 8 : 1), g.K, use_bf16(d, g.K));
  g.tz = (Dg + g.cfg.TZ - 1) / g.cfg.TZ;
  g.ty = (Hg + g.cfg.TY - 1) / g.cfg.TY;
  g.tx = (Wg + g.cfg.TX - 1) / g.cfg.TX;
  g.tiles_per_n = g.tz * g.ty * g.tx;
  g.ncls = g.classes ? 8 : 1;
  g.tiles = g.tiles_per_n * x->n * g.ncls;
  g.nstages = (g.K + g.cfg.KCI - 1) / g.cfg.KCI;
  const int ncolgroups = (g.Np + 32 * g.cfg.NB - 1) / (32 * g.cfg.NB);
  const int wgs = g.tiles_per_n * g.ncls * ncolgroups;
  g.ksplit = 1;
  g.sps = g.nstages;
  if (wgs < g_tune[0] && g.nstages > 1) {
    int want = (g_tune[1] + wgs - 1) / wgs;
    if (want > g.nstages) want = g.nstages;
    g.sps = (g.nstages + want - 1) / want;
    g.ksplit = (g.nstages + g.sps - 1) / g.sps;
  }
  g.route = config_id(g.cfg);
  if (g.classes && g.cfg.bf && g_cls_fused_min > 0) {
    const int ftz = (Dg + 3) / 4, fty = (Hg + 3) / 4, ftx = (Wg + 7) / 8;
    const long long fw = (long long)ftz * fty * ftx * (g.Np / 32);
    if (fw >= g_cls_fused_min && cls_fused_operand(x) && cls_fused_operand(y) && y->c % 4 == 0 && is_bf16(x) == is_bf16(y) &&
        g_epilogue_vec) {
      g.route = C_CLS_FUSED;
      g.tz = ftz; g.ty = fty; g.tx = ftx;
      g.tiles_per_n = ftz * fty * ftx;
      g.ncls = 1;
      g.tiles = g.tiles_per_n * x->n;
      g.nstages = (g.K + 15) / 16;
      g.ksplit = 1; g.sps = g.nstages;
    }
  }
  const bool f32_operands = !use_bf16(d, g.K);
  if (direct_applicable(d)) {
    g.route = C_DIRECT; g.ksplit = 1;
    g.tiles = direct_blocks_per_n(d, x, y) * y->n;
  } else if (rt && f32_operands && is_f32(x) && pointwise_small_applicable(d, x, y, rt->stats, rt->add, rt->x_norm)) {
    g.route = C_PW_SMALL;
  } else if (f32_operands && chan_applicable(d, x, y)) {
    g.route = C_THIN; g.ksplit = 1;
    g.tiles = chan_tiles_per_n(y) * y->n;
  } else if (rt && pointwise_mfma_applicable(d, x, y, g, *rt)) {
    g.route = C_PW_MFMA;
  } else if (rt && igemm_reuse_applicable(d, x, y, g, *rt)) {
    g.route = C_IGEMM_REUSE;
  }
  g.stats_rows = g.tiles * stats_rows_per_tile(g);
  g.workspace_bytes = g.ksplit > 1 ? (int64_t)g.ksplit * g.tiles * g.cfg.TZ * g.cfg.TY * g.cfg.TX * g.Np * (int64_t)sizeof(float) : 0;
  return MMTTA_OK;
}

static void build_taps(const mmtta_conv_desc* d, int pz, int py, int px, Taps& t) {
  int n = 0;
  const bool classes = (d->op == MMTTA_CONVT_FWD) || (d->op == MMTTA_CONV_DGRAD && d->stride == 2);
  if (d->ksize == 1) {
    t.dz[0] = t.dy[0] = t.dx[0] = 0; t.slab[0] = 0; n = 1;
  } else if (!classes) {
    const int sgn = (d->op == MMTTA_CONV_DGRAD) ? -1 : 1;
    for (int m = 0; m < 27; ++m) {
      const int q = sgn < 0 ? 26 - m : m, kz = q / 9, ky = q / 3 % 3, kx = q % 3;
      t.dz[n] = (signed char)(sgn * (kz - 1)); t.dy[n] = (signed char)(sgn * (ky - 1));
      t.dx[n] = (signed char)(sgn * (kx - 1)); t.slab[n] = q; ++n;
    }
  } else {
    int kzs[2], dzs[2], nz, kys[2], dys[2], ny, kxs[2], dxs[2], nx;
    auto axis = [](int p, int* ks, int* ds) { if (p == 0) { ks[0] = 1; ds[0] = 0; return 1; }
                                              ks[0] = 0; ds[0] = 1; ks[1] = 2; ds[1] = 0; return 2; };
    nz = axis(pz, kzs, dzs); ny = axis(py, kys, dys); nx = axis(px, kxs, dxs);
    for (int a = 0; a < nz; ++a) for (int b = 0; b < ny; ++b) for (int c = 0; c < nx; ++c) {
      t.dz[n] = (signed char)dzs[a]; t.dy[n] = (signed char)dys[b]; t.dx[n] = (signed char)dxs[c];
      t.slab[n] = (kzs[a] * 3 + kys[b]) * 3 + kxs[c]; ++n;
    }
  }
  t.n = n;
  int zmn = 9, zmx = -9, ymn = 9, ymx = -9, xmn = 9, xmx = -9;
  for (int i = 0; i < n; ++i) {
    zmn = t.dz[i] < zmn ? t.dz[i] : zmn; zmx = t.dz[i] > zmx ? t.dz[i] : zmx;
    ymn = t.dy[i] < ymn ? t.dy[i] : ymn; ymx = t.dy[i] > ymx ? t.dy[i] : ymx;
    xmn = t.dx[i] < xmn ? t.dx[i] : xmn; xmx = t.dx[i] > xmx ? t.dx[i] : xmx;
  }
  t.zmin = zmn; t.ymin = ymn; t.xmin = xmn;
  t.zext = zmx - zmn; t.yext = ymx - ymn; t.xext = xmx - xmn;
}

template <int NB, int MB, int TZ, int TY, int TX, int KCI, bool BF, int OCC, bool ABF, bool REUSE = false, bool RAW = false>
static int launch_cfg_t(const GArgs& a_in, const Taps* ht, int tiles, hipStream_t s) {
  GArgs a = a_in;
  size_t lds = 0;
  for (int c = 0; c < a.ncls; ++c) {
    const Taps& tp = ht[c];
    const int BZ = (TZ - 1) * a.si + tp.zext + 1, BY = (TY - 1) * a.si + tp.yext + 1, BX = (TX - 1) * a.si + tp.xext + 1;
    const int LP = (BF && a.si == 1) ? LDS_PITCH_BF16 : BX;
    for (int t = 0; t < tp.n; ++t) {
      a.toff[a.cls[c].tap0 + t] = ((tp.dz[t] - tp.zmin) * BY + (tp.dy[t] - tp.ymin)) * LP + (tp.dx[t] - tp.xmin);
      a.slab[a.cls[c].tap0 + t] = tp.slab[t];
    }
    a.cls[c].BX = BX; a.cls[c].BXY = BX * BY;
    a.cls[c].mBX = (unsigned)(((1ULL << 32) + BX - 1) / BX);
    a.cls[c].mBXY = (unsigned)(((1ULL << 32) + (unsigned long long)BX * BY - 1) / ((unsigned long long)BX * BY));
    const size_t need = BF ? (size_t)BZ * BY * LP * (KCI + 8) * 2 : (size_t)BZ * BY * BX * (KCI + 1) * sizeof(float);
    if (need > lds) lds = need;
  }
  if (BF && a.rowload && a.si == 1 && a.ncls == 1 && a.cls[0].ntaps == 27) {
    a.flip27 = a.slab[0] == 26 ? 1 : 0;
    for (int t = 0; t < 27; ++t)
      if (a.toff[t] != tap27_off(t, TY + 2) || a.slab[t] != (a.flip27 ? 26 - t : t)) a.rowload = 0;
  }
  constexpr size_t epi = (4 * (REUSE ? 2 : 1) * EPI_TILE_FLOATS + 4 * 2 * 32) * sizeof(float);
  if (lds < epi) lds = epi;
  if constexpr (REUSE) {
    if (!(a.rowload && a.ovec && a.ksplit == 1 && a.Ci == KCI * a.nstages))
      return launch_cfg_t<NB, MB, TZ, TY, TX, KCI, BF, OCC, ABF, false, RAW>(a_in, ht, tiles, s);
  }
  lds = (lds + 15) / 16 * 16;
  a.coef_off = (int)(lds / sizeof(float));
  if (BF && !RAW) lds += (size_t)2 * a.stages_per_split * KCI * sizeof(float);
  MMTTA_CHECK(lds <= 160 * 1024, MMTTA_ERR_UNSUPPORTED, "conv: LDS box of %zu bytes exceeds 160 KiB", lds);
  int st;
  void (*kern)(GArgs);
  if constexpr (RAW) {
    static_assert(BF && ABF, "raw staging copies bf16-stored items");
    if constexpr (REUSE) kern = igemm_reuse_raw_kernel<ABF>;
    else kern = igemm_raw_kernel<NB, MB, TZ, TY, TX, KCI, OCC>;
  } else if constexpr (REUSE) {
    kern = igemm_reuse_kernel<ABF>;
  } else {
    kern = igemm_kernel<NB, MB, TZ, TY, TX, KCI, BF, OCC, ABF>;
  }
  static bool attr_set = false;
  if (!attr_set) {
    (void)hipFuncSetAttribute((const void*)kern, hipFuncAttributeMaxDynamicSharedMemorySize, 160 * 1024);
    attr_set = true;
  }
  dim3 grid(tiles, (a.Np + 32 * NB - 1) / (32 * NB), a.ksplit);
  hipLaunchKernelGGL(kern, grid, dim3(256), lds, s, a);
  st = launch_status("conv igemm");
  if (st) return st;
  if (a.ksplit > 1 && !g_profile_main_only) {
    dim3 g2(tiles * (TZ * TY * TX / 32), (a.Np + 31) / 32);
    hipLaunchKernelGGL((splitk_finalize_kernel<TZ, TY, TX, BF, ABF>), g2, dim3(256), 0, s, a, tiles);
    st = launch_status("conv split-K finalize");
  }
  return st;
}

template <int NB, int MB, int TZ, int TY, int TX, int KCI, bool BF, int OCC = 2, bool REUSE = false>
static int launch_cfg(const GArgs& a, const Taps* ht, int tiles, bool raw, hipStream_t s) {
  if constexpr (BF) {
    if (a.in_bf || a.out_bf || a.add_bf) {
      MMTTA_CHECK(a.in_bf && a.out_bf && (a.add == nullptr || a.add_bf), MMTTA_ERR_UNSUPPORTED,
                  "conv: input, output and fused add must share one storage type (in %d out %d add %d)", a.in_bf, a.out_bf,
                  a.add_bf);
      if constexpr (RAW_KERNELS) {
        if (raw) return launch_cfg_t<NB, MB, TZ, TY, TX, KCI, BF, OCC, true, REUSE, true>(a, ht, tiles, s);
      }
      return launch_cfg_t<NB, MB, TZ, TY, TX, KCI, BF, OCC, true, REUSE>(a, ht, tiles, s);
    }
  }
  return launch_cfg_t<NB, MB, TZ, TY, TX, KCI, BF, OCC, false, REUSE>(a, ht, tiles, s);
}

static int launch_any(int route, const GArgs& a, const Taps* ht, int tiles, bool raw, hipStream_t s) {
  switch (route) {
    case 0: return launch_cfg<1, 4, 8, 8, 8, 8, false>(a, ht, tiles, raw, s);
    case 1: return launch_cfg<2, 4, 4, 8, 8, 16, false>(a, ht, tiles, raw, s);
    case 2: return launch_cfg<4, 4, 4, 4, 8, 32, false>(a, ht, tiles, raw, s);
    case 3: return launch_cfg<1, 1, 4, 4, 8, 8, false>(a, ht, tiles, raw, s);
    case 4: return launch_cfg<2, 2, 4, 4, 8, 8, false>(a, ht, tiles, raw, s);
    case 5: return launch_cfg<4, 4, 4, 4, 8, 8, false>(a, ht, tiles, raw, s);
    case 14: return launch_cfg<1, 2, 4, 8, 8, 16, true, 3>(a, ht, tiles, raw, s);
    case C_IGEMM_REUSE: return launch_cfg<1, 2, 4, 8, 8, 16, true, 3, true>(a, ht, tiles, raw, s);
    case 7: return launch_cfg<1, 4, 8, 8, 8, 16, true>(a, ht, tiles, raw, s);
    case 8: return launch_cfg<2, 4, 4, 8, 8, 32, true>(a, ht, tiles, raw, s);
    case 9: return launch_cfg<4, 4, 4, 4, 8, 32, true>(a, ht, tiles, raw, s);
    case 10: return launch_cfg<1, 1, 4, 4, 8, 16, true>(a, ht, tiles, raw, s);
    case 11: return launch_cfg<2, 2, 4, 4, 8, 16, true>(a, ht, tiles, raw, s);
    default: return launch_cfg<4, 4, 4, 4, 8, 16, true>(a, ht, tiles, raw, s);
  }
}

struct ConvCall {
  const mmtta_conv_desc* d; const mmtta_tensor* x; const mmtta_norm_on_load* x_norm; const void* packed; const float* bias;
  const mmtta_conv_epilogue* epi; const mmtta_tensor* y; int accumulate; float* stats; void* workspace; int64_t workspace_bytes;
  PSets ps; hipStream_t stream;
};

static int fill_gargs(const ConvCall& c, const Geometry& g, GArgs& a, Taps* ht) {
  const mmtta_tensor *x = c.x, *y = c.y, *ad = (c.epi && c.epi->add) ? c.epi->add : nullptr;
  a.in = (const float*)x->ptr; a.isn = x->sn; a.isd = x->sd; a.ish = x->sh; a.isw = x->sw;
  a.Ci = x->c; a.Di = x->d; a.Hi = x->h; a.Wi = x->w; a.tin = nl(c.x_norm);
  a.out = (float*)y->ptr; a.osn = y->sn; a.osd = y->sd; a.osh = y->sh; a.osw = y->sw;
  a.Co = y->c; a.Do = y->d; a.Ho = y->h; a.Wo = y->w;
  a.si = g.si; a.bias = c.bias; a.ps = c.ps; a.accumulate = c.accumulate;
  a.wp = (const float*)c.packed; a.Kp = g.Kp; a.Np = g.Np;
  const int st = epilogue_add(c.epi, y, a);
  if (st) return st;
  a.in_bf = is_bf16(x) ? 1 : 0; a.out_bf = is_bf16(y) ? 1 : 0; a.add_bf = (ad && is_bf16(ad)) ? 1 : 0;
  const bool oal = quad_aligned(y, quad_bytes(y)) && y->c % 4 == 0 &&
                   (!ad || quad_aligned(ad, quad_bytes(ad))) && (c.bias == nullptr || ((uintptr_t)c.bias) % 16 == 0);
  a.ovec = (oal && g_epilogue_vec) ? 1 : 0;
  a.stats = c.stats; a.stats_rows_per_n = g.ncls * g.tiles_per_n * stats_rows_per_tile(g);
  a.ws = (float*)c.workspace; a.ksplit = g.ksplit; a.stages_per_split = g.sps; a.nstages = g.nstages;
  a.tz = g.tz; a.ty = g.ty; a.tx = g.tx;
  MMTTA_CHECK(g.cfg.bf || (!a.in_bf && !a.out_bf && !a.add_bf), MMTTA_ERR_UNSUPPORTED,
              "conv: bf16-stored tensors need a bf16-operand layer (K >= 16 in bf16 precision)");
  const bool al = quad_aligned(x, 16, a.in_bf ? 8 : 4);
  a.vec4 = al ? 1 : 0; a.flip27 = 0;
  a.rowload = (rowload_operand(x) && g_igemm_pipeline) ? 1 : 0;
  a.ncls = g.classes ? 8 : 1; a.so = g.classes ? 2 : 1;
  int tap0 = 0;
  for (int cls = 0; cls < a.ncls; ++cls) {
    const int pz = (cls >> 2) & 1, py = (cls >> 1) & 1, px = cls & 1;
    build_taps(c.d, pz, py, px, ht[cls]);
    ClassInfo& ci = a.cls[cls];
    ci.tap0 = tap0; ci.ntaps = ht[cls].n; tap0 += ht[cls].n;
    ci.zmin = ht[cls].zmin; ci.ymin = ht[cls].ymin; ci.xmin = ht[cls].xmin;
    ci.zext = ht[cls].zext; ci.yext = ht[cls].yext; ci.xext = ht[cls].xext;
    if (g.classes) {
      ci.oz = pz; ci.oy = py; ci.ox = px;
      ci.Dg = (y->d - pz + 1) / 2; ci.Hg = (y->h - py + 1) / 2; ci.Wg = (y->w - px + 1) / 2;
    } else {
      ci.oz = ci.oy = ci.ox = 0;
      ci.Dg = y->d; ci.Hg = y->h; ci.Wg = y->w;
    }
  }
  return MMTTA_OK;
}

static int igemm_run(const ConvCall& c, const Geometry& g) {
  MMTTA_CHECK(g.workspace_bytes == 0 || (c.workspace != nullptr && c.workspace_bytes >= g.workspace_bytes), MMTTA_ERR_WORKSPACE,
              "conv: workspace %lld bytes, need %lld", (long long)c.workspace_bytes, (long long)g.workspace_bytes);
  GArgs a; Taps ht[8];
  const int st = fill_gargs(c, g, a, ht);
  if (st) return st;
  const bool raw = raw_staging(g.route, g.cfg.bf, c.x, c.x_norm, c.y, (c.epi && c.epi->add) ? c.epi->add : nullptr);
  return launch_any(g.route, a, ht, g.tiles, raw, c.stream);
}

static int cls_fused_run(const ConvCall& c, const Geometry& g) {
  GArgs a; Taps ht[8];
  const int st = fill_gargs(c, g, a, ht);
  if (st) return st;
  MMTTA_CHECK(a.ovec && a.vec4, MMTTA_ERR_UNSUPPORTED,
              "conv (class-fused stride-2 form): the epilogue operands must admit 16-byte accesses");
  MMTTA_CHECK(a.in_bf == a.out_bf && (a.add == nullptr || a.add_bf == a.out_bf), MMTTA_ERR_UNSUPPORTED,
              "conv: input, output and fused add must share one storage type (in %d out %d add %d)", a.in_bf, a.out_bf, a.add_bf);
  if constexpr (RAW_KERNELS) {
    const mmtta_tensor* ad = (c.epi && c.epi->add) ? c.epi->add : nullptr;
    if (cls8_lean(g.route, g.cfg.bf, c.x, c.x_norm, c.y, ad)) return launch_cls8_t<16, true, true, true, true>(a, g.tiles, c.stream);
    if (cls8_pipelined(g.route, g.cfg.bf, c.x, c.x_norm, c.y, ad)) return launch_cls8_t<16, true, true, true>(a, g.tiles, c.stream);
    if (raw_staging(g.route, g.cfg.bf, c.x, c.x_norm, c.y, ad)) return launch_cls8_t<16, true, true>(a, g.tiles, c.stream);
  }
  return a.in_bf ? launch_cls8_t<16, true>(a, g.tiles, c.stream) : launch_cls8_t<16, false>(a, g.tiles, c.stream);
}

static int pointwise_mfma_run(const ConvCall& c, const Geometry& g) {
  const mmtta_tensor *x = c.x, *y = c.y, *ad = (c.epi && c.epi->add) ? c.epi->add : nullptr;
  PWArgs q;
  q.in = (const float*)x->ptr; q.isn = x->sn; q.isw = (unsigned)x->sw; q.Ci = x->c;
  q.out = (float*)y->ptr; q.osn = y->sn; q.osw = (unsigned)y->sw; q.Co = y->c;
  q.add = ad ? (const float*)ad->ptr : nullptr; q.asn = ad ? ad->sn : 0; q.asw = ad ? (unsigned)ad->sw : 0u;
  q.tadd = ad ? nl(&c.epi->add_norm) : nl(nullptr);
  q.wp = (const float*)c.packed; q.bias = c.bias; q.Np = g.Np; q.ps = c.ps; q.accumulate = c.accumulate;
  q.dhw = (long long)y->d * y->h * y->w;
  long long blocks = (q.dhw + 127) / 128;
  if (blocks > 2048) blocks = 2048;
  const dim3 grid((unsigned)blocks, y->n);
  if (is_bf16(x)) launch_pointwise_mfma<true>(q, (g.K + 15) / 16, g.Np / 32, grid, c.stream);
  else launch_pointwise_mfma<false>(q, (g.K + 15) / 16, g.Np / 32, grid, c.stream);
  return launch_status("1x1 conv (streaming MFMA)");
}

static int plan_run(const mmtta_conv_desc* d, const mmtta_tensor* x, const mmtta_norm_on_load* x_norm, const mmtta_conv_epilogue* epi,
                    const mmtta_tensor* y, int accumulate, const float* stats, const float* bias, Geometry& g) {
  const RunFacts rt{stats, epi ? epi->add : nullptr, x_norm, accumulate, bias};
  return geometry(d, x, y, &rt, g);
}

int conv_run_body(const mmtta_conv_desc* d, const mmtta_tensor* x, const mmtta_norm_on_load* x_norm, const void* packed,
                  const float* bias, const mmtta_conv_epilogue* epi, const mmtta_tensor* y, int accumulate, float* stats,
                  void* workspace, int64_t workspace_bytes, const mmtta_param_sets* sets, void* stream) {
  Geometry g;
  int st = plan_run(d, x, x_norm, epi, y, accumulate, stats, bias, g);
  if (st) return st;
  MMTTA_CHECK(packed != nullptr, MMTTA_ERR_INVALID, "conv: null packed weights");
  st = psets_validate(sets, x->n);
  if (st) return st;
  const ConvCall c{d, x, x_norm, packed, bias, epi, y, accumulate, stats, workspace, workspace_bytes, psets(sets), (hipStream_t)stream};
  switch (g.route) {
    case C_DIRECT: return direct_conv_run(d, x, x_norm, packed, bias, epi, y, accumulate, stats, c.ps, c.stream);
    case C_PW_SMALL: return pointwise_small_run(x, packed, g.Kp, g.Np, bias, y, accumulate, c.ps, c.stream);
    case C_THIN: return chan_conv_run(d, x, x_norm, packed, g.Kp, g.Np, bias, epi, y, accumulate, stats, c.ps, c.stream);
    case C_PW_MFMA: return pointwise_mfma_run(c, g);
    case C_CLS_FUSED: return cls_fused_run(c, g);
    default: return igemm_run(c, g);
  }
}

MMTTA_ACT_NS_CLOSE
}

#ifndef MMTTA_ACT_LEAKY_TU
using namespace mmtta;

static int pack_entry_geometry(const mmtta_conv_desc* d, PackEntry& e, bool& up8, bool& chfr) {
  int st = validate_desc(d);
  if (st) return st;
  int K, N, si; bool cl;
  op_dims(d, K, N, si, cl);
  const bool convt = d->op == MMTTA_CONVT_FWD || d->op == MMTTA_CONVT_DGRAD;
  const bool direct = direct_applicable(d);
  e.w = nullptr; e.p = nullptr; e.up8 = nullptr; e.chfr = nullptr;
  e.A = convt ? d->cin : d->cout; e.B = convt ? d->cout : d->cin;
  e.T = d->ksize * d->ksize * d->ksize;
  e.Kp = direct ? K : roundup(K, 32); e.Np = direct ? 4 : roundup(N, 32);
  e.kn_is_ba = (d->op == MMTTA_CONV_FWD || d->op == MMTTA_CONVT_DGRAD) ? 1 : 0;
  e.bf16 = use_bf16(d, K) ? 1 : 0; e.direct = direct ? 1 : 0;
  up8 = direct && upconv8_image_bytes(d) > 0;
  chfr = !direct && chan_frag_bytes(d) > 0;
  e.KI = K; e.NO = N;
  MMTTA_CHECK(e.T == 1 || e.T == 27, MMTTA_ERR_UNSUPPORTED, "pack: ksize %d", d->ksize);
  e.start = 0;
  return MMTTA_OK;
}

static int fill_pack_entry(const mmtta_conv_desc* d, const float* w, void* packed, PackEntry& e) {
  bool up8, chfr;
  int st = pack_entry_geometry(d, e, up8, chfr);
  if (st) return st;
  MMTTA_CHECK(w && packed, MMTTA_ERR_INVALID, "pack: null pointer");
  e.w = w; e.p = packed;
  e.up8 = up8 ? (unsigned short*)((char*)packed + (size_t)e.T * e.Kp * e.Np * 4) : nullptr;
  e.chfr = chfr ? (uint4*)((char*)packed + (size_t)e.T * e.Kp * e.Np * 4) : nullptr;
  return MMTTA_OK;
}

extern "C" int64_t mmtta_conv_packed_bytes(const mmtta_conv_desc* d) {
  PackEntry e;
  bool up8, chfr;
  if (pack_entry_geometry(d, e, up8, chfr)) return -1;
  return (int64_t)e.T * e.Kp * e.Np * (int64_t)(e.bf16 ? 2 : sizeof(float)) + (e.direct ? upconv8_image_bytes(d) : chan_frag_bytes(d));
}

extern "C" int mmtta_conv_pack_weights(const mmtta_conv_desc* d, const float* w, void* packed, void* stream) {
  PackEntry e;
  int st = fill_pack_entry(d, w, packed, e);
  if (st) return st;
  const long long total = (long long)e.T * e.Kp * e.Np;
  int blocks = (int)((total + 255) / 256);
  if (blocks > 4096) blocks = 4096;
  if (e.bf16)
    hipLaunchKernelGGL(pack_weights_bf16_kernel, dim3(blocks), dim3(256), 0, (hipStream_t)stream, w, (unsigned short*)packed,
                       e.A, e.B, e.T, e.Kp, e.Np, e.kn_is_ba);
  else
    hipLaunchKernelGGL(pack_weights_kernel, dim3(blocks), dim3(256), 0, (hipStream_t)stream, w, (float*)packed, e.A, e.B, e.T,
                       e.Kp, e.Np, e.kn_is_ba);
  if (e.up8)
    hipLaunchKernelGGL(pack_upconv8_kernel, dim3((e.KI * 4 + 255) / 256), dim3(256), 0, (hipStream_t)stream, w, e.up8, e.KI, e.NO);
  if (e.chfr)
    hipLaunchKernelGGL(pack_chan_frags_kernel, dim3(1), dim3(256), 0, (hipStream_t)stream, (const float*)packed, e.chfr, e.Kp,
                       e.Np, e.KI, e.NO);
  return launch_status("pack weights");
}

namespace mmtta {
int pack_image_geometry(const mmtta_conv_desc* d, PackImageGeo& g) {
  PackEntry e;
  bool up8, chfr;
  const int st = pack_entry_geometry(d, e, up8, chfr);
  if (st) return st;
  g.A = e.A; g.B = e.B; g.T = e.T; g.Kp = e.Kp; g.Np = e.Np; g.kn_is_ba = e.kn_is_ba;
  g.plain_bf16 = (e.bf16 && !e.direct && !up8 && !chfr) ? 1 : 0;
  return MMTTA_OK;
}
}

extern "C" int64_t mmtta_conv_pack_table_bytes(int count) { return count < 0 ? -1 : (int64_t)count * (int64_t)sizeof(PackEntry); }

extern "C" int mmtta_conv_pack_table_build(const mmtta_pack_item* items, int count, void* table_host, int64_t* total) {
  MMTTA_CHECK(items && table_host && total && count > 0, MMTTA_ERR_INVALID, "pack table: bad argument");
  PackEntry* tab = (PackEntry*)table_host;
  long long run = 0;
  for (int i = 0; i < count; ++i) {
    int st = fill_pack_entry(&items[i].desc, items[i].w_master, items[i].packed, tab[i]);
    if (st) return st;
    tab[i].start = run;
    run += tab[i].direct ? ((long long)tab[i].Kp * tab[i].Np + 255) / 256
                         : (long long)(tab[i].Kp / PK) * (tab[i].Np / PN);
  }
  *total = run;
  return MMTTA_OK;
}

extern "C" int mmtta_conv_pack_batched(const void* table_dev, int count, int64_t total, void* stream) {
  MMTTA_CHECK(table_dev && count > 0 && total > 0, MMTTA_ERR_INVALID, "pack batched: bad argument");
  MMTTA_CHECK(total < (1LL << 31), MMTTA_ERR_UNSUPPORTED, "pack batched: %lld workgroups", (long long)total);
  hipLaunchKernelGGL(pack_batched_kernel, dim3((unsigned)total), dim3(256), 0, (hipStream_t)stream, (const PackEntry*)table_dev,
                     count);
  int st = launch_status("pack batched");
  if (st) return st;
  hipLaunchKernelGGL(pack_chan_frags_batched_kernel, dim3((unsigned)count), dim3(256), 0, (hipStream_t)stream, (const PackEntry*)table_dev);
  return launch_status("pack batched (thin-K fragments)");
}

extern "C" int mmtta_conv_plan(const mmtta_conv_desc* d, const mmtta_tensor* x, const mmtta_tensor* y,
                               mmtta_conv_plan_t* plan) {
  MMTTA_CHECK(plan != nullptr, MMTTA_ERR_INVALID, "conv plan: null plan");
  Geometry g;
  int st = geometry(d, x, y, nullptr, g);
  if (st) return st;
  *plan = mmtta_conv_plan_t{g.tiles,  1, g.ksplit, g.stats_rows, g.route, 0, g.workspace_bytes};
  return MMTTA_OK;
}

extern "C" int mmtta_conv_route(const mmtta_conv_desc* d, const mmtta_tensor* x, const mmtta_norm_on_load* x_norm,
                                const mmtta_conv_epilogue* epi, const mmtta_tensor* y, int accumulate, const float* stats) {
  Geometry g;
  const int st = plan_run(d, x, x_norm, epi, y, accumulate, stats, nullptr, g);
  if (st) return st < 0 ? st : -st;
  return g.route;
}

extern "C" int mmtta_conv_stages_raw(const mmtta_conv_desc* d, const mmtta_tensor* x, const mmtta_norm_on_load* x_norm,
                                     const mmtta_conv_epilogue* epi, const mmtta_tensor* y, int accumulate, const float* stats) {
  Geometry g;
  const int st = plan_run(d, x, x_norm, epi, y, accumulate, stats, nullptr, g);
  if (st) return st < 0 ? st : -st;
  const mmtta_tensor* add = (epi && epi->add) ? epi->add : nullptr;
  return (raw_staging(g.route, g.cfg.bf, x, x_norm, y, add) && !(add && nl_leaky(&epi->add_norm))) ? 1 : 0;
}

extern "C" int mmtta_conv_cls8_pipelined(const mmtta_conv_desc* d, const mmtta_tensor* x, const mmtta_norm_on_load* x_norm,
                                         const mmtta_conv_epilogue* epi, const mmtta_tensor* y, int accumulate, const float* stats) {
  Geometry g;
  const int st = plan_run(d, x, x_norm, epi, y, accumulate, stats, nullptr, g);
  if (st) return st < 0 ? st : -st;
  const mmtta_tensor* add = (epi && epi->add) ? epi->add : nullptr;
  return (cls8_pipelined(g.route, g.cfg.bf, x, x_norm, y, add) && !(add && nl_leaky(&epi->add_norm))) ? 1 : 0;
}

extern "C" int mmtta_conv_cls8_lean_epilogue(const mmtta_conv_desc* d, const mmtta_tensor* x, const mmtta_norm_on_load* x_norm,
                                             const mmtta_conv_epilogue* epi, const mmtta_tensor* y, int accumulate, const float* stats) {
  Geometry g;
  const int st = plan_run(d, x, x_norm, epi, y, accumulate, stats, nullptr, g);
  if (st) return st < 0 ? st : -st;
  const mmtta_tensor* add = (epi && epi->add) ? epi->add : nullptr;
  return (cls8_lean(g.route, g.cfg.bf, x, x_norm, y, add) && !(add && nl_leaky(&epi->add_norm))) ? 1 : 0;
}

extern "C" int mmtta_conv_thin_lean(const mmtta_conv_desc* d, const mmtta_tensor* x, const mmtta_norm_on_load* x_norm,
                                    const mmtta_conv_epilogue* epi, const mmtta_tensor* y, int accumulate, const float* stats) {
  Geometry g;
  const int st = plan_run(d, x, x_norm, epi, y, accumulate, stats, nullptr, g);
  if (st) return st < 0 ? st : -st;
  if (g.route == C_THIN) return chan_lean_applicable(d, x, x_norm, epi, y, accumulate) ? 1 : 0;
  if (g.route == C_DIRECT) return direct_upconv8_lean(d, x, x_norm, epi, y) ? 2 : 0;
  return 0;
}

extern "C" int mmtta_conv_thin_kernel(const mmtta_conv_desc* d, const mmtta_tensor* x, const mmtta_norm_on_load* x_norm,
                                      const mmtta_conv_epilogue* epi, const mmtta_tensor* y, int accumulate, const float* stats) {
  Geometry g;
  const int st = plan_run(d, x, x_norm, epi, y, accumulate, stats, nullptr, g);
  if (st) return st < 0 ? st : -st;
  if (g.route == C_THIN) return chan_kernel(d, x, x_norm, epi, y, accumulate);
  if (g.route == C_DIRECT) return direct_kernel(d, x, x_norm, epi, y, accumulate, stats);
  return 0;
}

static int head_loss_plan(const mmtta_conv_desc* d, const mmtta_tensor* x, const mmtta_norm_on_load* x_norm,
                          const mmtta_conv_epilogue* epi, const mmtta_tensor* y, const mmtta_tensor* dz, int softmax, int per_item,
                          bool& eligible) {
  Geometry g;
  const int st = plan_run(d, x, x_norm, epi, y, 0, nullptr, nullptr, g);
  if (st) return st;
  eligible = g.route == C_DIRECT && direct_head_loss_eligible(d, x, x_norm, epi, y, dz, softmax, per_item);
  return MMTTA_OK;
}

extern "C" int mmtta_conv_head_loss_eligible(const mmtta_conv_desc* d, const mmtta_tensor* x, const mmtta_norm_on_load* x_norm,
                                             const mmtta_conv_epilogue* epi, const mmtta_tensor* y, const mmtta_tensor* dlogits,
                                             int softmax, int per_item) {
  bool ok = false;
  const int st = head_loss_plan(d, x, x_norm, epi, y, dlogits, softmax, per_item, ok);
  if (st) return st < 0 ? st : -st;
  return ok ? 1 : 0;
}

extern "C" int64_t mmtta_conv_head_loss_partials(const mmtta_conv_desc* d, const mmtta_tensor* x, const mmtta_tensor* y) {
  Geometry g;
  if (geometry(d, x, y, nullptr, g) || g.route != C_DIRECT) return -1;
  return (int64_t)direct_blocks_per_n(d, x, y) * y->n;
}

extern "C" int mmtta_conv_head_loss_run_sets(const mmtta_conv_desc* d, const mmtta_tensor* x, const mmtta_norm_on_load* x_norm,
                                             const void* packed, const float* bias, const mmtta_conv_epilogue* epi,
                                             const mmtta_tensor* y, const mmtta_tensor* dlogits, int softmax, int per_item,
                                             double* partial, float* loss, const mmtta_param_sets* sets, void* stream) {
  int st = nl_act_check(x_norm, "conv_head_loss_run (x_norm)");
  if (st) return st;
  st = nl_act_check((epi && epi->add) ? &epi->add_norm : nullptr, "conv_head_loss_run (epilogue add_norm)");
  if (st) return st;
  st = nl_per_item_check(x_norm, "conv_head_loss_run (x_norm)");
  if (st) return st;
  st = nl_per_item_check(epi ? &epi->add_norm : nullptr, "conv_head_loss_run (epilogue add_norm)");
  if (st) return st;
  bool ok = false;
  st = head_loss_plan(d, x, x_norm, epi, y, dlogits, softmax, per_item, ok);
  if (st) return st;
  MMTTA_CHECK(ok, MMTTA_ERR_UNSUPPORTED,
              "conv_head_loss_run: not a sigmoid head on the 4x4x4 matrix tiles with a dense 4-lane `dlogits` (ask "
              "mmtta_conv_head_loss_eligible; run mmtta_conv_run and mmtta_entropy_loss_items instead)");
  MMTTA_CHECK(packed != nullptr && partial != nullptr && loss != nullptr, MMTTA_ERR_INVALID, "conv_head_loss_run: null argument");
  st = psets_validate(sets, x->n);
  if (st) return st;
  return direct_head_loss_run(d, x, x_norm, packed, bias, epi, y, dlogits, partial, loss, psets(sets), (hipStream_t)stream);
}

extern "C" int mmtta_conv_run(const mmtta_conv_desc* d, const mmtta_tensor* x, const mmtta_norm_on_load* x_norm,
                              const void* packed, const float* bias, const mmtta_conv_epilogue* epi,
                              const mmtta_tensor* y, int accumulate, float* stats, void* workspace,
                              int64_t workspace_bytes, void* stream) {
  return mmtta_conv_run_sets(d, x, x_norm, packed, bias, epi, y, accumulate, stats, workspace, workspace_bytes, nullptr, stream);
}

extern "C" int mmtta_conv_run_sets(const mmtta_conv_desc* d, const mmtta_tensor* x, const mmtta_norm_on_load* x_norm,
                                   const void* packed, const float* bias, const mmtta_conv_epilogue* epi,
                                   const mmtta_tensor* y, int accumulate, float* stats, void* workspace,
                                   int64_t workspace_bytes, const mmtta_param_sets* sets, void* stream) {
  const mmtta_norm_on_load* add_norm = (epi && epi->add) ? &epi->add_norm : nullptr;
  {
    int st = nl_act_check(x_norm, "conv_run (x_norm)");
    if (st) return st;
    st = nl_act_check(add_norm, "conv_run (epilogue add_norm)");
    if (st) return st;
    st = nl_per_item_check(x_norm, "conv_run (x_norm)");
    if (st) return st;
    st = nl_per_item_check(epi ? &epi->add_norm : nullptr, "conv_run (epilogue add_norm)");
    if (st) return st;
  }
  if (nl_leaky(x_norm) || nl_leaky(add_norm))
    return leaky::conv_run_body(d, x, x_norm, packed, bias, epi, y, accumulate, stats, workspace, workspace_bytes, sets, stream);
  return conv_run_body(d, x, x_norm, packed, bias, epi, y, accumulate, stats, workspace, workspace_bytes, sets, stream);
}
#endif
```

multimodal_tta_amd/csrc/conv_igemm_body.h:

```cpp
  extern __shared__ float lds[];
  static_assert(!REUSE || (NB == 1 && MB == 2 && TZ == 4 && TY == 8 && TX == 8 && KCI == 16 && BF && OCC > 2),
                "fragment reuse is built for the lean tile");
  static_assert(!RAW || (BF && ABF), "raw staging copies bf16-stored items");
  constexpr int VS = BF ? (KCI + 8) : (KCI + 1);
  static_assert(!BF || KCI % 16 == 0, "bf16 stages are multiples of the MFMA K=16");
  constexpr int MT = TZ * TY * TX;
  constexpr int MG = 4 / NB;
  static_assert(MT == 32 * MB * MG, "tile rows must equal 32*MB*(4/NB)");

  const int tid = threadIdx.x, lane = tid & 63, wave = tid >> 6;
  const int cb = wave % NB, mg = wave / NB;
  const int h = lane >> 5, r = lane & 31;

  const unsigned lflat = xcd_contiguous_id(blockIdx.x + gridDim.x * (blockIdx.y + gridDim.y * blockIdx.z),
                                           gridDim.x * gridDim.y * gridDim.z);
  const int bx = (int)(lflat % gridDim.x);
  const int lby = (int)((lflat / gridDim.x) % gridDim.y), lbz = (int)(lflat / (gridDim.x * gridDim.y));
  int cidx, t;
  class_of_tile(a, bx, cidx, t);
  const ClassInfo ci = a.cls[cidx];
  const int tile_in_n = t % (a.tz * a.ty * a.tx);
  const int txi = t % a.tx; t /= a.tx;
  const int tyi = t % a.ty; t /= a.ty;
  const int tzi = t % a.tz;
  const int n = t / a.tz;
  const float* wpn = pset_packed(a.ps, a.wp, n);
  const float* biasn = pset_bias(a.ps, a.bias, n);
  const int gz0 = tzi * TZ, gy0 = tyi * TY, gx0 = txi * TX;
  const int BZ = (TZ - 1) * a.si + ci.zext + 1;
  const int BY = (TY - 1) * a.si + ci.yext + 1;
  const int BX = (TX - 1) * a.si + ci.xext + 1;
  const int boxvox = BZ * BY * BX;
  const int LP = (BF && a.si == 1) ? LDS_PITCH_BF16 : BX;
  const int iz0 = gz0 * a.si + ci.zmin, iy0 = gy0 * a.si + ci.ymin, ix0 = gx0 * a.si + ci.xmin;

  const int colbase = (lby * NB + cb) * 32;
  const bool colact = REUSE || colbase < a.Np;

  int rowaddr[MB];
#pragma unroll
  for (int mb = 0; mb < MB; ++mb) {
    int zl, yl, xl;
    row_to_local<TZ, TY, TX, BF>((mg * MB + mb) * 32 + r, zl, yl, xl);
    rowaddr[mb] = (((zl * a.si) * BY + yl * a.si) * LP + xl * a.si) * VS + (BF ? 8 * h : h);
    if constexpr (REUSE) rowaddr[mb] = ((mg * (TY + 2) + (r >> 3) + 4 * ((r >> 2) & 1)) * LDS_PITCH_BF16 + (r & 3)) * VS + 8 * h;
  }

  f32x16 acc[MB];
#pragma unroll
  for (int mb = 0; mb < MB; ++mb)
#pragma unroll
    for (int i = 0; i < 16; ++i) acc[mb][i] = 0.f;

  const int ks0 = lbz * a.stages_per_split;
  const int ks1 = min(a.nstages, ks0 + a.stages_per_split);
  const float* inb = a.in;
  const long long inoff = (long long)n * a.isn;

  constexpr int RCV8 = BF ? KCI / 8 : 1;
  constexpr int RBY = TY + 2, RBZ = TZ + 2, RBX = TX + 2;
  constexpr int RIPR = RBX * RCV8;
  constexpr int RRPP = 256 / RIPR;
  constexpr int RNROW = RBZ * RBY;
  constexpr int RGP = (RNROW + RRPP - 1) / RRPP;
  constexpr int RPG = !BF ? 0 : (OCC > 2 ? 0 : (KCI == 16 ? (ABF ? 4 : 2) : 0));
  constexpr int RGPA = BF ? RGP : 1;
  const bool fast = REUSE || (BF && a.rowload && ci.ntaps == 27 && a.si == 1);
  const bool pipe = fast && RPG > 0;
  Oct8<ABF> gv[RGPA];
  unsigned voff[RGPA];
  unsigned pok = 0u;
  constexpr bool RHOIST = KCI == 16;
  const int rrsub = min(tid / RIPR, RRPP - 1), rrem = tid % RIPR, rbx = rrem / RCV8, rcv = rrem % RCV8;
  auto geometry = [&]() {
    int rs = rrsub;
    if constexpr (!RHOIST) asm volatile("" : "+v"(rs));
    const int ix = ix0 + rbx;
    const bool xok = (unsigned)ix < (unsigned)a.Wi;
    const unsigned xoff = __umul24((unsigned)min(max(ix, 0), a.Wi - 1), (unsigned)a.isw) + rcv * 8;
    pok = 0u;
    static_for<0, RGP>([&](auto pc) {
      constexpr int P = decltype(pc)::value;
      const int row = min(RRPP * P + rs, RNROW - 1);
      const int bz = row / RBY, by = row - bz * RBY;
      const int iz = iz0 + bz, iy = iy0 + by;
      const bool ok = xok && (unsigned)iz < (unsigned)a.Di && (unsigned)iy < (unsigned)a.Hi;
      pok |= (ok ? 1u : 0u) << P;
      voff[P] = __umul24((unsigned)min(max(iz, 0), a.Di - 1), (unsigned)a.isd) + __umul24((unsigned)min(max(iy, 0), a.Hi - 1), (unsigned)a.ish) + xoff;
    });
  };
  unsigned short* lh0 = reinterpret_cast<unsigned short*>(lds);
  unsigned short* rst = lh0 + (rrsub * LDS_PITCH_BF16 + (REUSE ? reuse_xslot(rbx) : rbx)) * VS + rcv * 8;
  float* coef = lds + a.coef_off;
  const int cbase = ks0 * KCI, nch = (ks1 - ks0) * KCI;
  if (fast) {
    if constexpr (!RAW) {
      for (int cch = tid; cch < nch; cch += 256) {
        float sc1 = 0.f, sh1 = 0.f;
        if (cbase + cch < a.Ci) nl_coeff(a.tin, n, a.Ci, cbase + cch, sc1, sh1);
        coef[cch] = sc1;
        coef[nch + cch] = sh1;
      }
    }
    if constexpr (RHOIST) geometry();
  }
  auto stage_base = [&](int ks) {
    return reinterpret_cast<const float*>(reinterpret_cast<const char*>(a.in) + ((long long)n * a.isn + (long long)ks * KCI) * (ABF ? 2 : 4));
  };
  const int cmax8 = ABF ? ((a.Ci - 1) & ~7) : ((a.Ci - 1) & ~3);
  auto load_item = [&](auto pc, const float* sb, int c0) {
    constexpr int P = decltype(pc)::value;
    const int over = max(c0 + rcv * 8 - cmax8, 0), over_hi = max(c0 + rcv * 8 + 4 - cmax8, 0);
    gv[P] = oct8_ld<ABF>(sb, voff[P] - over, voff[P] + 4 - over_hi);
  };
  auto issue = [&](int ks) {
    const float* sb = stage_base(ks);
    static_for<0, RPG>([&](auto pc) { load_item(pc, sb, ks * KCI); });
  };
  if (fast && ks0 < ks1) {
    if (pipe) issue(ks0);
    if constexpr (!RAW) __syncthreads();
  }

  constexpr bool CANON_CFG = BF && OCC > 2;
  const long long wslab16 = (long long)(a.Kp / 8) * a.Np * 16;
  const char* const wuni = reinterpret_cast<const char*>(wpn) + (a.flip27 ? 26 * wslab16 : 0);
  const long long wstep16 = a.flip27 ? -wslab16 : wslab16;
  const unsigned wlane16 = (unsigned)(h * a.Np + colbase + r) * 16u;
  auto wfrag27 = [&](int c0, int t, int k2) {
    const char* ub = wuni + ((long long)(c0 / 8) * a.Np + (long long)k2 * 2 * a.Np) * 16 + t * wstep16;
    return *reinterpret_cast<const uint4*>(ub + wlane16);
  };

  for (int ks = ks0; ks < ks1; ++ks) {
    const int stage = ks;
    const int c0 = ks * KCI;
    constexpr int WG0 = BF ? (OCC > 2 ? 3 : (KCI == 16 ? 9 : 5)) : 1;
    constexpr int WKS = BF ? KCI / 16 : 1;
    uint4 wfirst[WG0][WKS];
    bool wfirst_ok = false;
    if constexpr (BF) {
      if (REUSE || (colact && ci.ntaps == 27 && ((min(KCI, a.Ci - c0) + 15) >> 4) == WKS)) {
        wfirst_ok = true;
        const long long slabsz8 = (long long)(a.Kp / 8) * a.Np;
        if (CANON_CFG && fast) {
#pragma unroll
          for (int t = 0; t < WG0; ++t)
#pragma unroll
            for (int k2 = 0; k2 < WKS; ++k2) wfirst[t][k2] = wfrag27(c0, t, k2);
        } else {
          const uint4* wq0 = reinterpret_cast<const uint4*>(wpn) + (long long)(c0 / 8 + h) * a.Np + colbase + r;
#pragma unroll
          for (int t = 0; t < WG0; ++t)
#pragma unroll
            for (int k2 = 0; k2 < WKS; ++k2) wfirst[t][k2] = wq0[(a.slab + ci.tap0)[t] * slabsz8 + k2 * 2 * a.Np];
        }
      }
    }
    if constexpr (BF) {
      unsigned short* lh = reinterpret_cast<unsigned short*>(lds);
      if (fast) {
        const float* sb = stage_base(ks);
        constexpr int RB = ABF ? 6 : 4;
        constexpr int R1 = RPG + RB < RGP ? RPG + RB : RGP;
        if constexpr (!RHOIST) geometry();
        static_for<RPG, R1>([&](auto pc) { load_item(pc, sb, c0); });
        float sc[8], sh[8];
        if constexpr (!RAW) {
          const float4* cq = reinterpret_cast<const float4*>(coef + (c0 - cbase) + rcv * 8);
          const float4* hq = reinterpret_cast<const float4*>(coef + nch + (c0 - cbase) + rcv * 8);
          const float4 s0 = cq[0], s1 = cq[1], h0 = hq[0], h1 = hq[1];
          sc[0] = s0.x; sc[1] = s0.y; sc[2] = s0.z; sc[3] = s0.w; sc[4] = s1.x; sc[5] = s1.y; sc[6] = s1.z; sc[7] = s1.w;
          sh[0] = h0.x; sh[1] = h0.y; sh[2] = h0.z; sh[3] = h0.w; sh[4] = h1.x; sh[5] = h1.y; sh[6] = h1.z; sh[7] = h1.w;
        }
        const float relu_lo = act_lo(a.tin.relu);
        auto commit_item = [&](auto pc) {
          constexpr int P = decltype(pc)::value;
          uint4 pk;
          if constexpr (RAW) {
            const unsigned okm = (((pok >> P) & 1u) && (REUSE || c0 + rcv * 8 < a.Ci)) ? 0xffffffffu : 0u;
            pk = gv[P].q;
            pk.x &= okm; pk.y &= okm; pk.z &= okm; pk.w &= okm;
          } else {
          float v[8];
          oct8_f8(gv[P], v);
#pragma unroll
          for (int j = 0; j < 8; ++j) v[j] = act_max(fmaf(v[j], sc[j], sh[j]), relu_lo);
          const unsigned okm = ((pok >> P) & 1u) ? 0xffffffffu : 0u;
          pk.x = pack_bf16x2(v[0], v[1]) & okm; pk.y = pack_bf16x2(v[2], v[3]) & okm;
          pk.z = pack_bf16x2(v[4], v[5]) & okm; pk.w = pack_bf16x2(v[6], v[7]) & okm;
          }
          if (RNROW % RRPP == 0 || P + 1 < RGP || RRPP * P + rrsub < RNROW)
            *reinterpret_cast<uint4*>(rst + P * (RRPP * LDS_PITCH_BF16 * VS)) = pk;
        };
        static_for<0, R1>(commit_item);
        static_for_step<R1, RGP, RB>([&](auto r0) {
          constexpr int A = decltype(r0)::value, B = A + RB < RGP ? A + RB : RGP;
          static_for<A, B>([&](auto pc) { load_item(pc, sb, c0); });
          static_for<A, B>(commit_item);
        });
      } else if (RAW || a.vec4) {
        constexpr int CV8 = KCI / 8;
        const int cv = tid % CV8;
        const int c = c0 + cv * 8;
        float sc[8], sh[8];
        constexpr int STEP = 256 / CV8;
        const int first_item = 0;
        if constexpr (!RAW) nl_coeff_vec<8>(a.tin, n, a.Ci, c, sc, sh);
        constexpr int U = OCC > 2 ? 2 : 4;
        const bool tail = (a.Ci & 7) != 0;
        for (int bv0 = tid / CV8 + first_item * STEP; bv0 < boxvox; bv0 += U * STEP) {
          float4 x0[U], x1[U];
          uint4 xq[U];
          bool ok[U];
#pragma unroll
          for (int u = 0; u < U; ++u) {
            const int bv = bv0 + u * STEP;
            const int bz = (int)__umulhi((unsigned)bv, ci.mBXY), brem = bv - bz * ci.BXY;
            const int by = (int)__umulhi((unsigned)brem, ci.mBX), bx = brem - by * ci.BX;
            const int iz = iz0 + bz, iy = iy0 + by, ix = ix0 + bx;
            ok[u] = bv < boxvox && (unsigned)iz < (unsigned)a.Di && (unsigned)iy < (unsigned)a.Hi &&
                    (unsigned)ix < (unsigned)a.Wi && c < a.Ci;
            x0[u] = make_float4(0.f, 0.f, 0.f, 0.f);
            x1[u] = make_float4(0.f, 0.f, 0.f, 0.f);
            if constexpr (RAW) xq[u] = make_uint4(0u, 0u, 0u, 0u);
            if (ok[u]) {
              const long long so = inoff + (long long)iz * a.isd + (long long)iy * a.ish + (long long)ix * a.isw + c;
              if constexpr (RAW) xq[u] = *reinterpret_cast<const uint4*>(reinterpret_cast<const unsigned short*>(inb) + so);
              else if constexpr (ABF) ld8_t<true>(inb, so, x0[u], x1[u]);
              else {
                x0[u] = *reinterpret_cast<const float4*>(inb + so);
                if (c + 4 < a.Ci) x1[u] = *reinterpret_cast<const float4*>(inb + so + 4);
              }
            }
          }
#pragma unroll
          for (int u = 0; u < U; ++u) {
            const int bv = bv0 + u * STEP;
            if (bv < boxvox) {
              uint4 pk = make_uint4(0u, 0u, 0u, 0u);
              if constexpr (RAW) pk = xq[u];
              else if (ok[u]) {
                const float xs[8] = {x0[u].x, x0[u].y, x0[u].z, x0[u].w, x1[u].x, x1[u].y, x1[u].z, x1[u].w};
                float v[8];
#pragma unroll
                for (int j = 0; j < 8; ++j) {
                  v[j] = nl_apply(xs[j], sc[j], sh[j], a.tin.relu);
                  if (tail && c + j >= a.Ci) v[j] = 0.f;
                }
                pk.x = pack_bf16x2(v[0], v[1]); pk.y = pack_bf16x2(v[2], v[3]);
                pk.z = pack_bf16x2(v[4], v[5]); pk.w = pack_bf16x2(v[6], v[7]);
              }
              const int bz = (int)__umulhi((unsigned)bv, ci.mBXY), brem = bv - bz * ci.BXY;
              const int by = (int)__umulhi((unsigned)brem, ci.mBX), bx = brem - by * ci.BX;
              *reinterpret_cast<uint4*>(lh + ((bz * BY + by) * LP + bx) * VS + cv * 8) = pk;
            }
          }
        }
      } else {
        const int cc = tid % KCI;
        const int c = c0 + cc;
        float sc, sh;
        nl_coeff_vec<1>(a.tin, n, a.Ci, c, &sc, &sh);
        for (int bv = tid / KCI; bv < boxvox; bv += 256 / KCI) {
          const int bz = (int)__umulhi((unsigned)bv, ci.mBXY), brem = bv - bz * ci.BXY;
          const int by = (int)__umulhi((unsigned)brem, ci.mBX), bx = brem - by * ci.BX;
          const int iz = iz0 + bz, iy = iy0 + by, ix = ix0 + bx;
          float v = 0.f;
          if ((unsigned)iz < (unsigned)a.Di && (unsigned)iy < (unsigned)a.Hi && (unsigned)ix < (unsigned)a.Wi &&
              c < a.Ci)
            v = nl_apply(ld1_t<ABF>(inb, inoff + (long long)iz * a.isd + (long long)iy * a.ish + (long long)ix * a.isw + c), sc, sh,
                         a.tin.relu);
          lh[((bz * BY + by) * LP + bx) * VS + cc] = __builtin_bit_cast(unsigned short, (__bf16)v);
        }
      }
    } else {
    if (a.vec4) {
      constexpr int CV = KCI / 4;
      const int cv = tid % CV;
      const int c = c0 + cv * 4;
      float sc[4], sh[4];
      nl_coeff_vec<4>(a.tin, n, a.Ci, c, sc, sh);
      constexpr int U = 4, STEP = 256 / CV;
      for (int bv0 = tid / CV; bv0 < boxvox; bv0 += U * STEP) {
        float4 xin[U];
        bool ok[U];
#pragma unroll
        for (int u = 0; u < U; ++u) {
          const int bv = bv0 + u * STEP;
          const int bz = (int)__umulhi((unsigned)bv, ci.mBXY), brem = bv - bz * ci.BXY;
          const int by = (int)__umulhi((unsigned)brem, ci.mBX), bx = brem - by * ci.BX;
          const int iz = iz0 + bz, iy = iy0 + by, ix = ix0 + bx;
          ok[u] = bv < boxvox && (unsigned)iz < (unsigned)a.Di && (unsigned)iy < (unsigned)a.Hi &&
                  (unsigned)ix < (unsigned)a.Wi && c < a.Ci;
          xin[u] = make_float4(0.f, 0.f, 0.f, 0.f);
          if (ok[u]) xin[u] = *reinterpret_cast<const float4*>(inb + inoff + iz * a.isd + iy * a.ish + ix * a.isw + c);
        }
#pragma unroll
        for (int u = 0; u < U; ++u) {
          const int bv = bv0 + u * STEP;
          if (bv < boxvox) {
            float4 v = make_float4(0.f, 0.f, 0.f, 0.f);
            if (ok[u]) {
              v.x = nl_apply(xin[u].x, sc[0], sh[0], a.tin.relu);
              v.y = (c + 1 < a.Ci) ? nl_apply(xin[u].y, sc[1], sh[1], a.tin.relu) : 0.f;
              v.z = (c + 2 < a.Ci) ? nl_apply(xin[u].z, sc[2], sh[2], a.tin.relu) : 0.f;
              v.w = (c + 3 < a.Ci) ? nl_apply(xin[u].w, sc[3], sh[3], a.tin.relu) : 0.f;
            }
            float* d = lds + bv * VS + cv * 4;
            d[0] = v.x; d[1] = v.y; d[2] = v.z; d[3] = v.w;
          }
        }
      }
    } else {
      const int cc = tid % KCI;
      const int c = c0 + cc;
      float sc, sh;
      nl_coeff_vec<1>(a.tin, n, a.Ci, c, &sc, &sh);
      for (int bv = tid / KCI; bv < boxvox; bv += 256 / KCI) {
        const int bx = bv % BX, by = (bv / BX) % BY, bz = bv / (BX * BY);
        const int iz = iz0 + bz, iy = iy0 + by, ix = ix0 + bx;
        float v = 0.f;
        if ((unsigned)iz < (unsigned)a.Di && (unsigned)iy < (unsigned)a.Hi && (unsigned)ix < (unsigned)a.Wi &&
            c < a.Ci)
          v = nl_apply(inb[inoff + iz * a.isd + iy * a.ish + ix * a.isw + c], sc, sh, a.tin.relu);
        lds[bv * VS + cc] = v;
      }
    }
    }
    __syncthreads();

    if constexpr (BF) {
      if (colact) {
        constexpr int KS = KCI / 16;
        const unsigned short* lh = reinterpret_cast<const unsigned short*>(lds);
        const int kreal = min(KCI, a.Ci - c0);
        const int nks = (kreal + 15) >> 4;
        const uint4* wq = reinterpret_cast<const uint4*>(wpn);
        const long long slabsz8 = (long long)(a.Kp / 8) * a.Np;
        const uint4* wcol = wq + (long long)(c0 / 8 + h) * a.Np + colbase + r;
        const int np2 = 2 * a.Np;
        const int ntap = ci.ntaps;
        const int* tslab = a.slab + ci.tap0;
        const int* ttoff = a.toff + ci.tap0;
        if constexpr (REUSE) {
          constexpr int G = 3, NG = 9;
          static_assert(G == WG0 && KS == 1 && WKS == 1, "a weight group is one box row");
          auto rfrag = [&](int j, int m) {
            return *reinterpret_cast<const uint4*>(lh + rowaddr[0] + (((j / 3) * RBY + j % 3) * LDS_PITCH_BF16 + reuse_xslot(m)) * VS);
          };
          uint4 wset[2][G];
#pragma unroll
          for (int t = 0; t < G; ++t) wset[0][t] = wfirst[t][0];
          uint4 f[4], fn[2];
          f[0] = rfrag(0, 0);
          f[1] = rfrag(0, 1);
#pragma unroll
          for (int g = 0; g < NG; ++g) {
            if (g + 1 < NG) {
#pragma unroll
              for (int t = 0; t < G; ++t) wset[(g + 1) & 1][t] = wfrag27(c0, (g + 1) * G + t, 0);
            }
            __builtin_amdgcn_sched_barrier(0);
#pragma unroll
            for (int t = 0; t < G; ++t) {
              const bf16x8 bfr = __builtin_bit_cast(bf16x8, wset[g & 1][t]);
              if (t < 2) f[t + 2] = rfrag(g, t + 2);
              else if (g + 1 < NG) fn[0] = rfrag(g + 1, 0);
              acc[0] = __builtin_amdgcn_mfma_f32_32x32x16_bf16(__builtin_bit_cast(bf16x8, f[t]), bfr, acc[0], 0, 0, 0);
              if (t == 2 && g + 1 < NG) fn[1] = rfrag(g + 1, 1);
              acc[1] = __builtin_amdgcn_mfma_f32_32x32x16_bf16(__builtin_bit_cast(bf16x8, f[t + 1]), bfr, acc[1], 0, 0, 0);
              const bool rd0 = t < 2 || g + 1 < NG, rd1 = t == 2 && g + 1 < NG;
              if (rd0) __builtin_amdgcn_sched_group_barrier(0x100, 1, 0);
              __builtin_amdgcn_sched_group_barrier(0x008, 1, 0);
              if (rd1) __builtin_amdgcn_sched_group_barrier(0x100, 1, 0);
              __builtin_amdgcn_sched_group_barrier(0x008, 1, 0);
            }
            f[0] = fn[0];
            f[1] = fn[1];
            __builtin_amdgcn_sched_barrier(0);
          }
        } else if (nks == KS && ntap == 27) {
          constexpr int G = OCC > 2 ? 3 : (KS == 1 ? 9 : 5);
          constexpr int NG = (27 + G - 1) / G;
          static_assert(G == WG0 && KS == WKS, "first-group prefetch must match the group shape");
          auto stage27 = [&](auto fc) {
          constexpr bool CANON = decltype(fc)::value;
          uint4 wset[2][G][KS];
#pragma unroll
          for (int t = 0; t < G; ++t)
#pragma unroll
            for (int ks = 0; ks < KS; ++ks) wset[0][t][ks] = wfirst[t][ks];
          uint4 avc[MB];
          {
            const int ta0 = CANON ? 0 : ttoff[0] * VS;
#pragma unroll
            for (int mb = 0; mb < MB; ++mb) avc[mb] = *reinterpret_cast<const uint4*>(lh + rowaddr[mb] + ta0);
          }
#pragma unroll
          for (int g = 0; g < NG; ++g) {
            if (g + 1 < NG) {
#pragma unroll
              for (int t = 0; t < G; ++t) {
                if ((g + 1) * G + t < 27) {
#pragma unroll
                  for (int ks = 0; ks < KS; ++ks)
                    wset[(g + 1) & 1][t][ks] = CANON ? wfrag27(c0, (g + 1) * G + t, ks) : wcol[tslab[(g + 1) * G + t] * slabsz8 + ks * np2];
                }
              }
            }
            if (g == NG - 2 && pipe && stage + 1 < ks1) issue(stage + 1);
            __builtin_amdgcn_sched_barrier(0);
#pragma unroll
            for (int t = 0; t < G; ++t) {
              if (g * G + t < 27) {
#pragma unroll
                for (int ks = 0; ks < KS; ++ks) {
                  const bf16x8 bfr = __builtin_bit_cast(bf16x8, wset[g & 1][t][ks]);
                  const int idx = g * G + t;
                  const bool more = !(idx == 26 && ks == KS - 1);
                  const int nidx = ks + 1 < KS ? idx : idx + 1, nks2 = ks + 1 < KS ? ks + 1 : 0;
                  uint4 avn[MB];
                  int tan = 0;
                  if (more) tan = (CANON ? tap27_off(nidx, RBY) : ttoff[nidx]) * VS + nks2 * 16;
#pragma unroll
                  for (int mb = 0; mb < MB; ++mb) {
                    if (more) avn[mb] = *reinterpret_cast<const uint4*>(lh + rowaddr[mb] + tan);
                    acc[mb] = __builtin_amdgcn_mfma_f32_32x32x16_bf16(__builtin_bit_cast(bf16x8, avc[mb]), bfr, acc[mb], 0, 0, 0);
                  }
#pragma unroll
                  for (int mb = 0; mb < MB; ++mb) {
                    if (more) __builtin_amdgcn_sched_group_barrier(0x100, 1, 0);
                    __builtin_amdgcn_sched_group_barrier(0x008, 1, 0);
                  }
                  if (more) {
#pragma unroll
                    for (int mb = 0; mb < MB; ++mb) avc[mb] = avn[mb];
                  }
                }
              }
            }
            __builtin_amdgcn_sched_barrier(0);
          }
          };
          if constexpr (CANON_CFG) {
            if (fast) stage27(std::true_type{});
            else stage27(std::false_type{});
          } else {
            stage27(std::false_type{});
          }
        } else if (nks == KS && ntap >= 4) {
          constexpr int D = 4;
          uint4 ring[D][KS];
#pragma unroll
          for (int d = 0; d < D; ++d) {
            const uint4* wb = wcol + tslab[d] * slabsz8;
#pragma unroll
            for (int ks = 0; ks < KS; ++ks) ring[d][ks] = wb[ks * np2];
          }
          const int ntap_pad = (ntap + D - 1) / D * D;
          for (int tp0 = 0; tp0 < ntap_pad; tp0 += D) {
#pragma unroll
            for (int d = 0; d < D; ++d) {
              const int tp = tp0 + d;
              const bool live = tp < ntap;
              bf16x8 bfrag[KS];
#pragma unroll
              for (int ks = 0; ks < KS; ++ks) {
                uint4 q = ring[d][ks];
                q.x = live ? q.x : 0u; q.y = live ? q.y : 0u; q.z = live ? q.z : 0u; q.w = live ? q.w : 0u;
                bfrag[ks] = __builtin_bit_cast(bf16x8, q);
              }
              const uint4* wb = wcol + tslab[min(tp + D, ntap - 1)] * slabsz8;
#pragma unroll
              for (int ks = 0; ks < KS; ++ks) ring[d][ks] = wb[ks * np2];
              const int ta = ttoff[min(tp, ntap - 1)] * VS;
#pragma unroll
              for (int ks = 0; ks < KS; ++ks) {
#pragma unroll
                for (int mb = 0; mb < MB; ++mb) {
                  const uint4 av = *reinterpret_cast<const uint4*>(lh + rowaddr[mb] + ta + ks * 16);
                  acc[mb] = __builtin_amdgcn_mfma_f32_32x32x16_bf16(__builtin_bit_cast(bf16x8, av), bfrag[ks], acc[mb], 0, 0, 0);
                }
              }
            }
          }
        } else {
          for (int tp = 0; tp < ntap; ++tp) {
            const uint4* wb = wcol + tslab[tp] * slabsz8;
            const int ta = ttoff[tp] * VS;
            for (int ks = 0; ks < nks; ++ks) {
              const bf16x8 bfrag = __builtin_bit_cast(bf16x8, wb[ks * np2]);
#pragma unroll
              for (int mb = 0; mb < MB; ++mb) {
                const uint4 av = *reinterpret_cast<const uint4*>(lh + rowaddr[mb] + ta + ks * 16);
                acc[mb] = __builtin_amdgcn_mfma_f32_32x32x16_bf16(__builtin_bit_cast(bf16x8, av), bfrag, acc[mb], 0, 0, 0);
              }
            }
          }
        }
      } else if (pipe && stage + 1 < ks1) {
        issue(stage + 1);
      }
    } else {
    if (colact) {
      constexpr int KK = KCI / 2;
      const int kreal = min(KCI, a.Ci - c0);
      const float* wcol = wpn + (long long)c0 * a.Np + colbase + r + (long long)h * a.Np;
      const long long slabsz = (long long)a.Kp * a.Np;
      const int np2 = 2 * a.Np;
      const int ntap = ci.ntaps;
      const int* tslab = a.slab + ci.tap0;
      const int* ttoff = a.toff + ci.tap0;
      if (kreal == KCI) {
        float bcur[KK], bnxt[KK];
        {
          const float* wb = wcol + tslab[0] * slabsz;
#pragma unroll
          for (int kk = 0; kk < KK; ++kk) bcur[kk] = wb[kk * np2];
        }
        for (int tp = 0; tp < ntap; ++tp) {
          const int tn = min(tp + 1, ntap - 1);
          const float* wb = wcol + tslab[tn] * slabsz;
#pragma unroll
          for (int kk = 0; kk < KK; ++kk) bnxt[kk] = wb[kk * np2];
          const int ta = ttoff[tp] * VS;
#pragma unroll
          for (int kk = 0; kk < KK; ++kk) {
#pragma unroll
            for (int mb = 0; mb < MB; ++mb) {
              const float av = lds[rowaddr[mb] + ta + 2 * kk];
              acc[mb] = __builtin_amdgcn_mfma_f32_32x32x2f32(av, bcur[kk], acc[mb], 0, 0, 0);
            }
          }
#pragma unroll
          for (int kk = 0; kk < KK; ++kk) bcur[kk] = bnxt[kk];
        }
      } else {
        const int kkn = (kreal + 1) >> 1;
        for (int tp = 0; tp < ntap; ++tp) {
          const float* wb = wcol + tslab[tp] * slabsz;
          const int ta = ttoff[tp] * VS;
          for (int kk = 0; kk < kkn; ++kk) {
            const float b = wb[kk * np2];
#pragma unroll
            for (int mb = 0; mb < MB; ++mb) {
              const float av = lds[rowaddr[mb] + ta + 2 * kk];
              acc[mb] = __builtin_amdgcn_mfma_f32_32x32x2f32(av, b, acc[mb], 0, 0, 0);
            }
          }
        }
      }
    }
    }
    __syncthreads();
  }

  const int col = colbase + r;
  const bool colok = colact && col < a.Co;
  float s_sum = 0.f, s_sq = 0.f;
  if (!REUSE && a.ksplit > 1) {
    if (colact) {
      float* wsb = a.ws + ((long long)lbz * gridDim.x + bx) * MT * a.Np + col;
#pragma unroll
      for (int mb = 0; mb < MB; ++mb)
#pragma unroll
        for (int i = 0; i < 16; ++i) {
          const int row = (i & 3) + 8 * (i >> 2) + 4 * h;
          const int v = (mg * MB + mb) * 32 + row;
          wsb[(long long)v * a.Np] = acc[mb][i];
        }
    }
    return;
  }
  if (REUSE || a.ovec) {
    constexpr int ETF = (REUSE ? 2 : 1) * EPI_TILE_FLOATS;
    float v_sum[4], v_sq[4];
    epilogue_vec16<TZ, TY, TX, MB, BF, ABF, REUSE>(a, biasn, ci, acc, lds + wave * ETF, lane, mg * MB, colbase, colact, n, gz0,
                                                   gy0, gx0, v_sum, v_sq);
    if (a.stats != nullptr) {
      float* red = lds + 4 * ETF;
      if (lane < 8) {
#pragma unroll
        for (int j = 0; j < 4; ++j) {
          red[(wave * 2 + 0) * 32 + lane * 4 + j] = v_sum[j];
          red[(wave * 2 + 1) * 32 + lane * 4 + j] = v_sq[j];
        }
      }
      __syncthreads();
      if (mg == 0 && h == 0 && colok) {
        float ts = 0.f, tq = 0.f;
#pragma unroll
        for (int g = 0; g < MG; ++g) {
          ts += red[((g * NB + cb) * 2 + 0) * 32 + r];
          tq += red[((g * NB + cb) * 2 + 1) * 32 + r];
        }
        const long long row = (long long)n * a.stats_rows_per_n + cidx * (a.tz * a.ty * a.tx) + tile_in_n;
        a.stats[(row * 2 + 0) * a.Co + col] = ts;
        a.stats[(row * 2 + 1) * a.Co + col] = tq;
      }
    }
    return;
  }
  float bias = 0.f, asc = 1.f, ash = 0.f;
  if (colok) {
    if (biasn) bias = biasn[col];
    if (a.add) nl_coeff(a.tadd, n, a.Co, col, asc, ash);
  }
  const int colc = min(col, a.Co - 1);
  const float* addb = a.add;
  float* outb = a.out;
  const long long abase = (long long)n * a.asn + colc, obase = (long long)n * a.osn + colc;
#pragma unroll
  for (int mb = 0; mb < MB; ++mb) {
#pragma unroll
    for (int half = 0; half < 2; ++half) {
      int ooff[8], aoff[8];
      bool ok[8];
#pragma unroll
      for (int j = 0; j < 8; ++j) {
        const int i = half * 8 + j;
        const int row = (i & 3) + 8 * (i >> 2) + 4 * h;
        int zl, yl, xl;
        row_to_local<TZ, TY, TX, BF>((mg * MB + mb) * 32 + row, zl, yl, xl);
        const int gz = gz0 + zl, gy = gy0 + yl, gx = gx0 + xl;
        const int oz = gz * a.so + ci.oz, oy = gy * a.so + ci.oy, ox = gx * a.so + ci.ox;
        ok[j] = colok && gz < ci.Dg && gy < ci.Hg && gx < ci.Wg && oz < a.Do && oy < a.Ho && ox < a.Wo;
        const int cz = min(oz, a.Do - 1), cy = min(oy, a.Ho - 1), cx = min(ox, a.Wo - 1);
        ooff[j] = cz * (int)a.osd + cy * (int)a.osh + cx * (int)a.osw;
        aoff[j] = cz * (int)a.asd + cy * (int)a.ash + cx * (int)a.asw;
      }
      float addv[8], oldv[8];
      if (a.add) {
#pragma unroll
        for (int j = 0; j < 8; ++j) addv[j] = ld1_t<ABF>(addb, abase + aoff[j]);
      }
      if (a.accumulate) {
#pragma unroll
        for (int j = 0; j < 8; ++j) oldv[j] = ld1_t<ABF>(outb, obase + ooff[j]);
      }
#pragma unroll
      for (int j = 0; j < 8; ++j) {
        float v = acc[mb][half * 8 + j] + bias;
        if (a.add) v += nl_apply(addv[j], asc, ash, a.tadd.relu);
        if (a.accumulate) v += oldv[j];
        if (ok[j]) {
          st1_t<ABF>(outb, obase + ooff[j], v);
          s_sum += v;
          s_sq += v * v;
        }
      }
    }
  }
  if (a.stats != nullptr) {
    s_sum += __shfl_xor(s_sum, 32, 64);
// ... 20 lines not shown
```

Before: 122.0.

## Add plane-wise staging loader with prefetch for stride-2 raw bf16 conv

Adds a dedicated stride-2 implicit-GEMM kernel variant for raw bf16 16-channel stages. It loads the input box plane by plane, with 256 items per plane plus a remainder handled by each wave, and lays rows out in LDS with an even/odd x-slot split at pitch 18. The next stage's global loads are prefetched into registers while the MFMA loop runs. It targets the generic stride-2 staging path, which previously had no pipelining or row loads. In exchange it holds more registers for the prefetched planes and adds new layout and tap-offset bookkeeping, which falls back to the old kernel when taps don't match.

```diff
diff --git a/include/mmtta.h b/include/mmtta.h
--- a/include/mmtta.h
+++ b/include/mmtta.h
@@ -67,6 +67,7 @@
 #define MMTTA_OPT_WGRAD_EPILOGUE_UPDATE 19
 #define MMTTA_OPT_CLS8_PIPELINE 20
 #define MMTTA_OPT_CLS8_LEAN_EPILOGUE 21
+#define MMTTA_OPT_S2_PLANE_LOADER 22
 int mmtta_set_option(int key, int value);
 
 int mmtta_copy_strided(const mmtta_tensor* src, const mmtta_tensor* dst, void* stream);
@@ -134,6 +135,9 @@
 
 int mmtta_conv_cls8_lean_epilogue(const mmtta_conv_desc* desc, const mmtta_tensor* x, const mmtta_norm_on_load* x_norm,
                                   const mmtta_conv_epilogue* epi, const mmtta_tensor* y, int accumulate, const float* stats);
+
+int mmtta_conv_s2_plane_loader(const mmtta_conv_desc* desc, const mmtta_tensor* x, const mmtta_norm_on_load* x_norm,
+                               const mmtta_conv_epilogue* epi, const mmtta_tensor* y, int accumulate, const float* stats);
 
 int mmtta_conv_thin_lean(const mmtta_conv_desc* desc, const mmtta_tensor* x, const mmtta_norm_on_load* x_norm,
                          const mmtta_conv_epilogue* epi, const mmtta_tensor* y, int accumulate, const float* stats);
diff --git a/multimodal_tta_amd/_lib.py b/multimodal_tta_amd/_lib.py
--- a/multimodal_tta_amd/_lib.py
+++ b/multimodal_tta_amd/_lib.py
@@ -135,6 +135,7 @@
     "mmtta_conv_stages_raw": (C.c_int, [_P(ConvDesc), _P(Tensor), _P(NormOnLoad), _P(ConvEpilogue), _P(Tensor), C.c_int, C.c_void_p]),
     "mmtta_conv_cls8_pipelined": (C.c_int, [_P(ConvDesc), _P(Tensor), _P(NormOnLoad), _P(ConvEpilogue), _P(Tensor), C.c_int, C.c_void_p]),
     "mmtta_conv_cls8_lean_epilogue": (C.c_int, [_P(ConvDesc), _P(Tensor), _P(NormOnLoad), _P(ConvEpilogue), _P(Tensor), C.c_int, C.c_void_p]),
+    "mmtta_conv_s2_plane_loader": (C.c_int, [_P(ConvDesc), _P(Tensor), _P(NormOnLoad), _P(ConvEpilogue), _P(Tensor), C.c_int, C.c_void_p]),
     "mmtta_conv_thin_lean": (C.c_int, [_P(ConvDesc), _P(Tensor), _P(NormOnLoad), _P(ConvEpilogue), _P(Tensor), C.c_int, C.c_void_p]),
     "mmtta_conv_thin_kernel": (C.c_int, [_P(ConvDesc), _P(Tensor), _P(NormOnLoad), _P(ConvEpilogue), _P(Tensor), C.c_int, C.c_void_p]),
     "mmtta_conv_head_loss_eligible": (C.c_int, [_P(ConvDesc), _P(Tensor), _P(NormOnLoad), _P(ConvEpilogue), _P(Tensor), _P(Tensor),
@@ -345,6 +346,8 @@
         lib.mmtta_set_option(20, int(os.environ["MMTTA_CLS8PIPE"]))
     if "MMTTA_CLS8LEAN" in os.environ:
         lib.mmtta_set_option(21, int(os.environ["MMTTA_CLS8LEAN"]))
+    if "MMTTA_S2PLANE" in os.environ:
+        lib.mmtta_set_option(22, int(os.environ["MMTTA_S2PLANE"]))
     _lib = lib
     return lib
 
diff --git a/multimodal_tta_amd/csrc/api.hip b/multimodal_tta_amd/csrc/api.hip
--- a/multimodal_tta_amd/csrc/api.hip
+++ b/multimodal_tta_amd/csrc/api.hip
@@ -24,6 +24,7 @@
 int g_wgrad_epilogue_update = 1;
 int g_cls8_pipeline = 1;
 int g_cls8_lean_epilogue = 1;
+int g_s2_plane_loader = 1;
 int g_tune[4] = {96, 128, 128, 256};
 }
 
@@ -98,6 +99,11 @@
     mmtta::g_cls8_lean_epilogue = value & 1;
     return prev;
   }
+  if (key == MMTTA_OPT_S2_PLANE_LOADER) {
+    const int prev = mmtta::g_s2_plane_loader;
+    mmtta::g_s2_plane_loader = value ? 1 : 0;
+    return prev;
+  }
   if (key == MMTTA_OPT_IGEMM_PIPELINE) {
     const int prev = mmtta::g_igemm_pipeline;
     mmtta::g_igemm_pipeline = value ? 1 : 0;
diff --git a/multimodal_tta_amd/csrc/common.h b/multimodal_tta_amd/csrc/common.h
--- a/multimodal_tta_amd/csrc/common.h
+++ b/multimodal_tta_amd/csrc/common.h
@@ -44,6 +44,7 @@
 extern int g_wgrad_epilogue_update;
 extern int g_cls8_pipeline;
 extern int g_cls8_lean_epilogue;
+extern int g_s2_plane_loader;
 extern int g_tune[4];
 
 inline bool nl_leaky(const mmtta_norm_on_load* t) { return t != nullptr && t->relu == MMTTA_ACT_LEAKY_RELU; }
diff --git a/multimodal_tta_amd/csrc/conv_igemm.hip b/multimodal_tta_amd/csrc/conv_igemm.hip
--- a/multimodal_tta_amd/csrc/conv_igemm.hip
+++ b/multimodal_tta_amd/csrc/conv_igemm.hip
@@ -78,6 +78,34 @@
 }
 
 constexpr int LDS_PITCH_BF16 = 12;
+constexpr int LDS_PITCH_S2 = 18;
+__host__ __device__ constexpr int s2_xslot(int bx, int tx) { return (bx & 1) * (tx + 1) + (bx >> 1); }
+
+template <int TX, int KCI, int VS>
+__device__ __forceinline__ void s2_item(const GArgs& a, int idx, int cv, int iy0, int ix0, unsigned& off, int& ldsoff, bool& ok) {
+  constexpr int BX = 2 * TX + 1;
+  const int vox = idx / (KCI / 8), qy = vox / BX, qx = vox - qy * BX;
+  const int iy = iy0 + qy, ix = ix0 + qx;
+  ok = (unsigned)iy < (unsigned)a.Hi && (unsigned)ix < (unsigned)a.Wi;
+  off = __umul24((unsigned)min(max(iy, 0), a.Hi - 1), (unsigned)a.ish) + __umul24((unsigned)min(max(ix, 0), a.Wi - 1), (unsigned)a.isw) + cv * 8;
+  ldsoff = (qy * LDS_PITCH_S2 + s2_xslot(qx, TX)) * VS + cv * 8;
+}
+template <int PB, int PE, int NJ, int BZ, int KCI, int NA, int NBJ>
+__device__ __forceinline__ void s2_request(uint4 (&va)[NA], uint4 (&vb)[NBJ], const GArgs& a, int n, int ks, int iz0, int wave, int cv,
+                                           int cmax8, unsigned offA, unsigned offB) {
+  const unsigned over = (unsigned)max(ks * KCI + cv * 8 - cmax8, 0);
+  const unsigned short* sb = reinterpret_cast<const unsigned short*>(a.in) + ((long long)n * a.isn + (long long)ks * KCI);
+  auto plane = [&](int p) { return sb + (long long)min(max(iz0 + p, 0), a.Di - 1) * a.isd; };
+  static_for<PB, PE>([&](auto pc) {
+    constexpr int P = decltype(pc)::value;
+    va[P] = *reinterpret_cast<const uint4*>(plane(P) + (offA - over));
+  });
+  static_for<0, NJ>([&](auto jc) {
+    constexpr int J = decltype(jc)::value;
+    const int p = wave + 4 * J;
+    if (4 * J + 3 < BZ || p < BZ) vb[J] = *reinterpret_cast<const uint4*>(plane(p) + (offB - over));
+  });
+}
 
 __host__ __device__ constexpr int tap27_off(int t, int rby) { return ((t / 9) * rby + (t / 3) % 3) * LDS_PITCH_BF16 + t % 3; }
 
@@ -231,27 +259,34 @@
 
 template <int NB, int MB, int TZ, int TY, int TX, int KCI, bool BF, int OCC = 2, bool ABF = false>
 __global__ __launch_bounds__(256, OCC) void igemm_kernel(GArgs a) {
-  constexpr bool REUSE = false, RAW = false;
+  constexpr bool REUSE = false, RAW = false, S2P = false;
 #include "conv_igemm_body.h"
 }
 
 template <bool ABF>
 __global__ __launch_bounds__(256, 3) void igemm_reuse_kernel(GArgs a) {
   constexpr int NB = 1, MB = 2, TZ = 4, TY = 8, TX = 8, KCI = 16, OCC = 3;
-  constexpr bool BF = true, REUSE = true, RAW = false;
+  constexpr bool BF = true, REUSE = true, RAW = false, S2P = false;
 #include "conv_igemm_body.h"
 }
 
 template <int NB, int MB, int TZ, int TY, int TX, int KCI, int OCC>
 __global__ __launch_bounds__(256, OCC) void igemm_raw_kernel(GArgs a) {
-  constexpr bool BF = true, ABF = true, REUSE = false, RAW = true;
+  constexpr bool BF = true, ABF = true, REUSE = false, RAW = true, S2P = false;
 #include "conv_igemm_body.h"
 }
 
 template <bool ABF>
 __global__ __launch_bounds__(256, 3) void igemm_reuse_raw_kernel(GArgs a) {
   constexpr int NB = 1, MB = 2, TZ = 4, TY = 8, TX = 8, KCI = 16, OCC = 3;
-  constexpr bool BF = true, REUSE = true, RAW = true;
+  constexpr bool BF = true, REUSE = true, RAW = true, S2P = false;
+#include "conv_igemm_body.h"
+}
+
+template <int NB, int MB>
+__global__ __launch_bounds__(256, 2) void igemm_raw_s2_kernel(GArgs a) {
+  constexpr int TZ = 4, TY = 4, TX = 8, KCI = 16, OCC = 2;
+  constexpr bool BF = true, ABF = true, REUSE = false, RAW = true, S2P = true;
 #include "conv_igemm_body.h"
 }
 
@@ -1027,6 +1062,12 @@
          item_fits_31(x, x->c + 16);
 }
 
+static bool s2_plane_loader(int route, bool bf_tile, int si, bool classes, int ksize, const mmtta_tensor* x,
+                            const mmtta_norm_on_load* x_norm, const mmtta_tensor* y, const mmtta_tensor* add) {
+  return g_s2_plane_loader && (route == 11 || route == 12) && si == 2 && !classes && ksize == 3 && raw_staging(route, bf_tile, x, x_norm, y, add) &&
+         rowload_operand(x);
+}
+
 static bool igemm_reuse_applicable(const mmtta_conv_desc* d, const mmtta_tensor* x, const mmtta_tensor* y, const Geometry& g,
                                    const RunFacts& rt) {
   const mmtta_tensor* ad = rt.add;
@@ -1155,7 +1196,7 @@
   t.zext = zmx - zmn; t.yext = ymx - ymn; t.xext = xmx - xmn;
 }
 
-template <int NB, int MB, int TZ, int TY, int TX, int KCI, bool BF, int OCC, bool ABF, bool REUSE = false, bool RAW = false>
+template <int NB, int MB, int TZ, int TY, int TX, int KCI, bool BF, int OCC, bool ABF, bool REUSE = false, bool RAW = false, bool S2P = false>
 static int launch_cfg_t(const GArgs& a_in, const Taps* ht, int tiles, hipStream_t s) {
   GArgs a = a_in;
   size_t lds = 0;
@@ -1178,6 +1219,14 @@
     for (int t = 0; t < 27; ++t)
       if (a.toff[t] != tap27_off(t, TY + 2) || a.slab[t] != (a.flip27 ? 26 - t : t)) a.rowload = 0;
   }
+  if constexpr (S2P) {
+    bool same = a.si == 2 && a.ncls == 1 && a.cls[0].ntaps == 27 && ht[0].zext == 2 && ht[0].yext == 2 && ht[0].xext == 2;
+    for (int t = 0; same && t < 27; ++t)
+      same = a.toff[t] == ((t / 9) * (2 * TY + 1) + (t / 3) % 3) * (2 * TX + 1) + t % 3 && a.slab[t] == t;
+    if (!same) return launch_cfg_t<NB, MB, TZ, TY, TX, KCI, BF, OCC, ABF, REUSE, RAW, false>(a_in, ht, tiles, s);
+    for (int t = 0; t < 27; ++t) a.toff[t] = ((t / 9) * (2 * TY + 1) + (t / 3) % 3) * LDS_PITCH_S2 + s2_xslot(t % 3, TX);
+    lds = (size_t)(2 * TZ + 1) * (2 * TY + 1) * LDS_PITCH_S2 * (KCI + 8) * 2;
+  }
   constexpr size_t epi = (4 * (REUSE ? 2 : 1) * EPI_TILE_FLOATS + 4 * 2 * 32) * sizeof(float);
   if (lds < epi) lds = epi;
   if constexpr (REUSE) {
@@ -1193,6 +1242,7 @@
   if constexpr (RAW) {
     static_assert(BF && ABF, "raw staging copies bf16-stored items");
     if constexpr (REUSE) kern = igemm_reuse_raw_kernel<ABF>;
+    else if constexpr (S2P) kern = igemm_raw_s2_kernel<NB, MB>;
     else kern = igemm_raw_kernel<NB, MB, TZ, TY, TX, KCI, OCC>;
   } else if constexpr (REUSE) {
     kern = igemm_reuse_kernel<ABF>;
@@ -1217,13 +1267,16 @@
 }
 
 template <int NB, int MB, int TZ, int TY, int TX, int KCI, bool BF, int OCC = 2, bool REUSE = false>
-static int launch_cfg(const GArgs& a, const Taps* ht, int tiles, bool raw, hipStream_t s) {
+static int launch_cfg(const GArgs& a, const Taps* ht, int tiles, bool raw, bool s2p, hipStream_t s) {
   if constexpr (BF) {
     if (a.in_bf || a.out_bf || a.add_bf) {
       MMTTA_CHECK(a.in_bf && a.out_bf && (a.add == nullptr || a.add_bf), MMTTA_ERR_UNSUPPORTED,
                   "conv: input, output and fused add must share one storage type (in %d out %d add %d)", a.in_bf, a.out_bf,
                   a.add_bf);
       if constexpr (RAW_KERNELS) {
+        if constexpr (NB == MB && (NB == 2 || NB == 4) && TZ == 4 && TY == 4 && TX == 8 && KCI == 16 && OCC == 2 && !REUSE) {
+          if (raw && s2p) return launch_cfg_t<NB, MB, TZ, TY, TX, KCI, BF, OCC, true, REUSE, true, true>(a, ht, tiles, s);
+        }
         if (raw) return launch_cfg_t<NB, MB, TZ, TY, TX, KCI, BF, OCC, true, REUSE, true>(a, ht, tiles, s);
       }
       return launch_cfg_t<NB, MB, TZ, TY, TX, KCI, BF, OCC, true, REUSE>(a, ht, tiles, s);
@@ -1232,22 +1285,22 @@
   return launch_cfg_t<NB, MB, TZ, TY, TX, KCI, BF, OCC, false, REUSE>(a, ht, tiles, s);
 }
 
-static int launch_any(int route, const GArgs& a, const Taps* ht, int tiles, bool raw, hipStream_t s) {
+static int launch_any(int route, const GArgs& a, const Taps* ht, int tiles, bool raw, bool s2p, hipStream_t s) {
   switch (route) {
-    case 0: return launch_cfg<1, 4, 8, 8, 8, 8, false>(a, ht, tiles, raw, s);
-    case 1: return launch_cfg<2, 4, 4, 8, 8, 16, false>(a, ht, tiles, raw, s);
-    case 2: return launch_cfg<4, 4, 4, 4, 8, 32, false>(a, ht, tiles, raw, s);
-    case 3: return launch_cfg<1, 1, 4, 4, 8, 8, false>(a, ht, tiles, raw, s);
-    case 4: return launch_cfg<2, 2, 4, 4, 8, 8, false>(a, ht, tiles, raw, s);
-    case 5: return launch_cfg<4, 4, 4, 4, 8, 8, false>(a, ht, tiles, raw, s);
-    case 14: return launch_cfg<1, 2, 4, 8, 8, 16, true, 3>(a, ht, tiles, raw, s);
-    case C_IGEMM_REUSE: return launch_cfg<1, 2, 4, 8, 8, 16, true, 3, true>(a, ht, tiles, raw, s);
-    case 7: return launch_cfg<1, 4, 8, 8, 8, 16, true>(a, ht, tiles, raw, s);
-    case 8: return launch_cfg<2, 4, 4, 8, 8, 32, true>(a, ht, tiles, raw, s);
-    case 9: return launch_cfg<4, 4, 4, 4, 8, 32, true>(a, ht, tiles, raw, s);
-    case 10: return launch_cfg<1, 1, 4, 4, 8, 16, true>(a, ht, tiles, raw, s);
-    case 11: return launch_cfg<2, 2, 4, 4, 8, 16, true>(a, ht, tiles, raw, s);
-    default: return launch_cfg<4, 4, 4, 4, 8, 16, true>(a, ht, tiles, raw, s);
+    case 0: return launch_cfg<1, 4, 8, 8, 8, 8, false>(a, ht, tiles, raw, s2p, s);
+    case 1: return launch_cfg<2, 4, 4, 8, 8, 16, false>(a, ht, tiles, raw, s2p, s);
+    case 2: return launch_cfg<4, 4, 4, 4, 8, 32, false>(a, ht, tiles, raw, s2p, s);
+    case 3: return launch_cfg<1, 1, 4, 4, 8, 8, false>(a, ht, tiles, raw, s2p, s);
+    case 4: return launch_cfg<2, 2, 4, 4, 8, 8, false>(a, ht, tiles, raw, s2p, s);
+    case 5: return launch_cfg<4, 4, 4, 4, 8, 8, false>(a, ht, tiles, raw, s2p, s);
+    case 14: return launch_cfg<1, 2, 4, 8, 8, 16, true, 3>(a, ht, tiles, raw, s2p, s);
+    case C_IGEMM_REUSE: return launch_cfg<1, 2, 4, 8, 8, 16, true, 3, true>(a, ht, tiles, raw, s2p, s);
+    case 7: return launch_cfg<1, 4, 8, 8, 8, 16, true>(a, ht, tiles, raw, s2p, s);
+    case 8: return launch_cfg<2, 4, 4, 8, 8, 32, true>(a, ht, tiles, raw, s2p, s);
+    case 9: return launch_cfg<4, 4, 4, 4, 8, 32, true>(a, ht, tiles, raw, s2p, s);
+    case 10: return launch_cfg<1, 1, 4, 4, 8, 16, true>(a, ht, tiles, raw, s2p, s);
+    case 11: return launch_cfg<2, 2, 4, 4, 8, 16, true>(a, ht, tiles, raw, s2p, s);
+    default: return launch_cfg<4, 4, 4, 4, 8, 16, true>(a, ht, tiles, raw, s2p, s);
   }
 }
 
@@ -1305,8 +1358,10 @@
   GArgs a; Taps ht[8];
   const int st = fill_gargs(c, g, a, ht);
   if (st) return st;
-  const bool raw = raw_staging(g.route, g.cfg.bf, c.x, c.x_norm, c.y, (c.epi && c.epi->add) ? c.epi->add : nullptr);
-  return launch_any(g.route, a, ht, g.tiles, raw, c.stream);
+  const mmtta_tensor* ad = (c.epi && c.epi->add) ? c.epi->add : nullptr;
+  const bool raw = raw_staging(g.route, g.cfg.bf, c.x, c.x_norm, c.y, ad);
+  const bool s2p = s2_plane_loader(g.route, g.cfg.bf, g.si, g.classes, c.d->ksize, c.x, c.x_norm, c.y, ad);
+  return launch_any(g.route, a, ht, g.tiles, raw, s2p, c.stream);
 }
 
 static int cls_fused_run(const ConvCall& c, const Geometry& g) {
@@ -1502,6 +1557,15 @@
   return (raw_staging(g.route, g.cfg.bf, x, x_norm, y, add) && !(add && nl_leaky(&epi->add_norm))) ? 1 : 0;
 }
 
+extern "C" int mmtta_conv_s2_plane_loader(const mmtta_conv_desc* d, const mmtta_tensor* x, const mmtta_norm_on_load* x_norm,
+                                          const mmtta_conv_epilogue* epi, const mmtta_tensor* y, int accumulate, const float* stats) {
+  Geometry g;
+  const int st = plan_run(d, x, x_norm, epi, y, accumulate, stats, nullptr, g);
+  if (st) return st < 0 ? st : -st;
+  const mmtta_tensor* add = (epi && epi->add) ? epi->add : nullptr;
+  return (s2_plane_loader(g.route, g.cfg.bf, g.si, g.classes, d->ksize, x, x_norm, y, add) && !(add && nl_leaky(&epi->add_norm))) ? 1 : 0;
+}
+
 extern "C" int mmtta_conv_cls8_pipelined(const mmtta_conv_desc* d, const mmtta_tensor* x, const mmtta_norm_on_load* x_norm,
                                          const mmtta_conv_epilogue* epi, const mmtta_tensor* y, int accumulate, const float* stats) {
   Geometry g;
diff --git a/multimodal_tta_amd/csrc/conv_igemm_body.h b/multimodal_tta_amd/csrc/conv_igemm_body.h
--- a/multimodal_tta_amd/csrc/conv_igemm_body.h
+++ b/multimodal_tta_amd/csrc/conv_igemm_body.h
@@ -2,6 +2,7 @@
   static_assert(!REUSE || (NB == 1 && MB == 2 && TZ == 4 && TY == 8 && TX == 8 && KCI == 16 && BF && OCC > 2),
                 "fragment reuse is built for the lean tile");
   static_assert(!RAW || (BF && ABF), "raw staging copies bf16-stored items");
+  static_assert(!S2P || (RAW && !REUSE && KCI == 16 && OCC == 2), "the plane loader stages raw 16-channel stride-2 stages");
   constexpr int VS = BF ? (KCI + 8) : (KCI + 1);
   static_assert(!BF || KCI % 16 == 0, "bf16 stages are multiples of the MFMA K=16");
   constexpr int MT = TZ * TY * TX;
@@ -31,7 +32,7 @@
   const int BY = (TY - 1) * a.si + ci.yext + 1;
   const int BX = (TX - 1) * a.si + ci.xext + 1;
   const int boxvox = BZ * BY * BX;
-  const int LP = (BF && a.si == 1) ? LDS_PITCH_BF16 : BX;
+  const int LP = S2P ? LDS_PITCH_S2 : ((BF && a.si == 1) ? LDS_PITCH_BF16 : BX);
   const int iz0 = gz0 * a.si + ci.zmin, iy0 = gy0 * a.si + ci.ymin, ix0 = gx0 * a.si + ci.xmin;
 
   const int colbase = (lby * NB + cb) * 32;
@@ -43,6 +44,7 @@
     int zl, yl, xl;
     row_to_local<TZ, TY, TX, BF>((mg * MB + mb) * 32 + r, zl, yl, xl);
     rowaddr[mb] = (((zl * a.si) * BY + yl * a.si) * LP + xl * a.si) * VS + (BF ? 8 * h : h);
+    if constexpr (S2P) rowaddr[mb] = ((zl * 2 * BY + yl * 2) * LP + xl) * VS + 8 * h;
     if constexpr (REUSE) rowaddr[mb] = ((mg * (TY + 2) + (r >> 3) + 4 * ((r >> 2) & 1)) * LDS_PITCH_BF16 + (r & 3)) * VS + 8 * h;
   }
 
@@ -63,9 +65,11 @@
   constexpr int RRPP = 256 / RIPR;
   constexpr int RNROW = RBZ * RBY;
   constexpr int RGP = (RNROW + RRPP - 1) / RRPP;
-  constexpr int RPG = !BF ? 0 : (OCC > 2 ? 0 : (KCI == 16 ? (ABF ? 4 : 2) : 0));
+  constexpr int RPGW = !BF ? 0 : (OCC > 2 ? 0 : (KCI == 16 ? (ABF ? 4 : 2) : 0));
+  constexpr int RPG = RPGW < RGP ? RPGW : RGP;
   constexpr int RGPA = BF ? RGP : 1;
-  const bool fast = REUSE || (BF && a.rowload && ci.ntaps == 27 && a.si == 1);
+  static_assert(RPG <= RGPA, "a prefetched pass is a pass of the stage");
+  const bool fast = !S2P && (REUSE || (BF && a.rowload && ci.ntaps == 27 && a.si == 1));
   const bool pipe = fast && RPG > 0;
   Oct8<ABF> gv[RGPA];
   unsigned voff[RGPA];
@@ -122,6 +126,31 @@
     if constexpr (!RAW) __syncthreads();
   }
 
+  constexpr int S2BZ = 2 * TZ + 1, S2BY = 2 * TY + 1, S2BX = 2 * TX + 1;
+  constexpr int S2IPP = S2BY * S2BX * (KCI / 8);
+  constexpr int S2PLANE = S2BY * LDS_PITCH_S2 * VS;
+  static_assert(LDS_PITCH_S2 >= 2 * TX + 1 && LDS_PITCH_S2 % 4 == 2, "room for the box row; 12 * pitch * 3 slots = 8 modulo 16");
+  constexpr int S2NB = S2IPP - 256;
+  constexpr int S2JB = (S2BZ + 3) / 4;
+  constexpr bool S2EARLY = S2P && MB == 2;
+  constexpr int S2PF = !S2P ? 0 : (S2EARLY ? 2 * TZ + 1 : 3);
+  constexpr int S2NA = S2P ? S2BZ : 1, S2NJ = S2P ? S2JB : 1;
+  static_assert(!S2P || (S2NB > 0 && S2NB <= 64 && (S2BZ - 1) * S2PLANE * 2 < 65536),
+                "a plane is 256 items and less than a wave more; plane offsets are ds_write immediates");
+  uint4 s2a[S2NA], s2b[S2NJ];
+  unsigned s2offA = 0u, s2offB = 0u;
+  int s2ldsA = 0, s2ldsB = 0, s2wave = 0;
+  bool s2okA = false, s2okB = false;
+  const int s2cv = tid % (KCI / 8);
+  if constexpr (S2P) {
+    s2wave = __builtin_amdgcn_readfirstlane(wave);
+    s2_item<TX, KCI, VS>(a, tid, s2cv, iy0, ix0, s2offA, s2ldsA, s2okA);
+    s2_item<TX, KCI, VS>(a, min(256 + lane, S2IPP - 1), s2cv, iy0, ix0, s2offB, s2ldsB, s2okB);
+    s2okB = s2okB && lane < S2NB;
+    s2ldsB += s2wave * S2PLANE;
+    if (ks0 < ks1) s2_request<0, S2PF, S2EARLY ? S2JB : 0, S2BZ, KCI>(s2a, s2b, a, n, ks0, iz0, s2wave, s2cv, cmax8, s2offA, s2offB);
+  }
+
   constexpr bool CANON_CFG = BF && OCC > 2;
   const long long wslab16 = (long long)(a.Kp / 8) * a.Np * 16;
   const char* const wuni = reinterpret_cast<const char*>(wpn) + (a.flip27 ? 26 * wslab16 : 0);
@@ -159,6 +188,34 @@
     }
     if constexpr (BF) {
       unsigned short* lh = reinterpret_cast<unsigned short*>(lds);
+      if constexpr (S2P) {
+        if constexpr (!S2EARLY) s2_request<S2PF, S2BZ, S2JB, S2BZ, KCI>(s2a, s2b, a, n, ks, iz0, s2wave, s2cv, cmax8, s2offA, s2offB);
+        uint4 ca[S2NA], cb[S2NJ];
+        static_for<0, S2BZ>([&](auto pc) { ca[decltype(pc)::value] = s2a[decltype(pc)::value]; });
+        static_for<0, S2JB>([&](auto jc) { cb[decltype(jc)::value] = s2b[decltype(jc)::value]; });
+        if constexpr (S2EARLY) {
+          if (stage + 1 < ks1) s2_request<0, S2BZ, S2JB, S2BZ, KCI>(s2a, s2b, a, n, stage + 1, iz0, s2wave, s2cv, cmax8, s2offA, s2offB);
+        }
+        const bool cok = c0 + s2cv * 8 < a.Ci;
+        const bool mA = s2okA && cok, mB = s2okB && cok;
+        static_for<0, S2BZ>([&](auto pc) {
+          constexpr int P = decltype(pc)::value;
+          const unsigned okm = (mA && (unsigned)(iz0 + P) < (unsigned)a.Di) ? 0xffffffffu : 0u;
+          uint4 pk = ca[P];
+          pk.x &= okm; pk.y &= okm; pk.z &= okm; pk.w &= okm;
+          *reinterpret_cast<uint4*>(lh + s2ldsA + P * S2PLANE) = pk;
+        });
+        static_for<0, S2JB>([&](auto jc) {
+          constexpr int J = decltype(jc)::value;
+          const int p = s2wave + 4 * J;
+          if (4 * J + 3 < S2BZ || p < S2BZ) {
+            const unsigned okm = (mB && (unsigned)(iz0 + p) < (unsigned)a.Di) ? 0xffffffffu : 0u;
+            uint4 pk = cb[J];
+            pk.x &= okm; pk.y &= okm; pk.z &= okm; pk.w &= okm;
+            if (lane < S2NB) *reinterpret_cast<uint4*>(lh + s2ldsB + 4 * J * S2PLANE) = pk;
+          }
+        });
+      } else
       if (fast) {
         const float* sb = stage_base(ks);
         constexpr int RB = ABF ? 6 : 4;
@@ -409,6 +466,10 @@
                 }
               }
             }
+            if constexpr (S2P) {
+              if (!S2EARLY && g == NG - 2 && stage + 1 < ks1)
+                s2_request<0, S2PF, 0, S2BZ, KCI>(s2a, s2b, a, n, stage + 1, iz0, s2wave, s2cv, cmax8, s2offA, s2offB);
+            } else
             if (g == NG - 2 && pipe && stage + 1 < ks1) issue(stage + 1);
             __builtin_amdgcn_sched_barrier(0);
 #pragma unroll
@@ -499,8 +560,9 @@
             }
           }
         }
-      } else if (pipe && stage + 1 < ks1) {
-        issue(stage + 1);
+      } else if (S2P ? (!S2EARLY && stage + 1 < ks1) : (pipe && stage + 1 < ks1)) {
+        if constexpr (S2P) s2_request<0, S2PF, 0, S2BZ, KCI>(s2a, s2b, a, n, stage + 1, iz0, s2wave, s2cv, cmax8, s2offA, s2offB);
+        else issue(stage + 1);
       }
     } else {
     if (colact) {
```

Result: no change. 122.3 (median of 3 runs) (+0.3%).
